# ChenyangLEI/All-In-One-Deflicker

Hardware: AMD Instinct MI355X
Metric: atlas-fit sampled points/sec (stage1, 10k iters) @1/2/4/8 GPU; PSNR vs ref (higher is better)
Workload: dtype f32 (MLP chains f16x3: operands split into 2 fp16 of their value scaled per row, 3 partial products; weight-gradient GEMM bf16x6; fp32 accumulate)

## Files before the change

all-in-one-deflicker_amd/csrc/elem.h:

```cpp
#pragma once
#include "af_dev.h"

struct PackArgs {
  const float* frames;
  const float* flow_f;
  const float* flow_b;
  const float* mask_f;
  const float* mask_b;
  const float* mask_fg;
  float* table;
  int resx, resy, F;
  unsigned long long* nvalid;
};

struct ResizeArgs {
  const void* src; int src_u8;
  int sh, sw, ch;
  float* dst; int dh, dw;
  long long pix_stride, ch_stride, offset;
  double scale0, scale1;
};
enum { AREA_GENERAL = 0, AREA_BLOCK = 1, AREA_2X2 = 2 };
struct AreaArgs {
  const unsigned char* src; int sh, sw, ch;
  unsigned char* dst; int dh, dw;
  int mode;
  int isx, isy; float inv_area;
  const int* xofs; const int* yofs;
  const int* xidx; const int* yidx;
  const float* xa; const float* ya;
};
struct LumaArgs {
  const unsigned char* src; int n, h, w;
  int gh, gw;
  int strip_rows, strips;
  unsigned long long* part;
};
enum { YUV_AXIS_FULL = 0, YUV_AXIS_CENTRED = 1, YUV_AXIS_COSITED = 2 };
struct YuvArgs {
  const unsigned char* src; unsigned char* dst;
  int h, w, ch, cw;
  int hmode, vmode, mono;
  int y0;
  int cy, crv, cgu, cgv, cbu;
  int ky[3], ku[3], kv[3];
};
struct ConsistencyArgs {
  const float* f12; const float* f21; int h, w;
  float* out; long long pix_stride, offset;
  float thresh;
};

struct PrepArgs {
  const float* table;
  const int64_t* inds;
  uint64_t seed; uint32_t iter;
  int N, resx, resy, F;
  float half_main, half_grad, half_frames;
  int d_local, d_global, nseg;
  float* coords;
  float* x0_tile;
  float* samples;
  int* counts;
  float* coords2;
  float* x0_tile2;
  float* coordsA;
  int d_global2;
  int* flow_rank;
  unsigned long long* scan;
  uint32_t epoch;
  unsigned long long* ticket;
  unsigned long long ticket_base;
  int* live;
};

struct LossArgs {
  const float* samples; const float* out_map; const float* out_atlas;
  float* dout_map; float* dout_atlas;
  const int* counts;
  const int* flow_rank; const int* live;
  float* loss_part;
  int N, nseg;
  float L, uv_scale; int d_local, d_global;
  float c_rgb, c_grad, c_rig, c_grig, c_flow;
};

struct LossSegArgs {
  const float* samples;
  const float* out_m1; const float* out_m2; const float* out_alpha; const float* out_atlas;
  float* dout_m1; float* dout_m2; float* dout_alpha; float* dout_atlas;
  const int* counts; float* loss_part;
  const int* flow_rank; const int* live;
  int N, nseg;
  float L, uv_scale; int d_local, d_global_fg, d_global_bg;
  float c_rgb, c_grad, c_rig, c_grig_fg, c_grig_bg, c_flow, c_boot, c_aflow, c_sparse;
};

struct PrePrepArgs {
  const int64_t* ys; const int64_t* xs;
  uint64_t seed; uint32_t iter;
  int N, resx, resy;
  float half_main, t;
  float* coords; float* x0_tile;
};
struct PreLossArgs { const float* coords; const float* out_map; float* dout_map; float* loss_part; int N; float uv_scale; };

struct CoordsAtArgs {
  float* coords;
  int resx, resy;
  int oh, ow;
  float half_main, t;
  long long r0; int n, n_pad;
};
struct FinishAtArgs {
  const float* out_atlas; const float* out_alpha; size_t row2;
  int n;
  float* rgb_out;
  unsigned char* u8_out;
  const unsigned char* ref;
  double* sse_part;
};

struct AdamJob {
  uint32_t part_off, part_blk, nslots, pld;
  uint32_t out_real, in_real, out_real_pad;
  uint32_t p_off;
  uint32_t p_ld;
  uint32_t col0;
  int32_t  b_off;
  uint32_t f_off;
  uint32_t f_mpad;
  int32_t  b_img_off;
  uint32_t b_mpad;
  uint32_t bias_img_off;
  uint32_t pe_kind;
  uint32_t hid_cols;
  int32_t  sf_off; uint32_t sf_kind, sf_mpad, sf_k0;
  int32_t  sb_off; uint32_t sb_kind, sb_mpad;
  int32_t  hf_off, hb_off;
};
struct AdamHyper { float step_size, bc2_sqrt, one_minus_b1, beta2, one_minus_b2, eps; };
struct AdamBufs { float* params; float* m; float* v; float* img_f; float* img_b; float* bias_img; char* sf; char* sb; char* hf; char* hb; };
struct AdamArgs {
  const AdamJob* jobs; const float* partial;
  AdamBufs bufs; AdamHyper hy;
  float* grad_out;
  const float* loss_part; float* loss_out; int* counts; int loss_nblk;
  int* nan_flag;
  int check_counts;
};

struct EditArgs {
  const float* uv1; const float* uv2; const float* out_alpha;
  int npix, res;
  int active[2]; float minx[2], miny[2], pixel_size[2];
  const float* tex[2];
  float* edit; float* edit_layer[2]; float* use[2];
  unsigned char* edit_u8;
};

struct LossMapArgs {
  float* coords; const float* table; size_t rec0;
  int resx, resy, rows_pad, frame, d;
  int seg_c, seg_ym, seg_xm, seg_t;
  float half_main, half_frames, t_centre;
  const float* out_m1; const float* out_m2;
  const float* out_alpha;
  const float* out_atlas;
  int flow_map;
  float L, uv_scale;
  float* rigidity1; float* rigidity2; float* flow1; float* flow2; float* flow_alpha; float* rgb_err; float* residual;
};

struct WarpErrArgs {
  const float* img1; const float* img2; const float* flow12; const float* flow21;
  size_t img_pair_stride, flow_pair_stride;
  int h, w, align_corners;
  float* noc; float* warped;
  double* part;
};
```

all-in-one-deflicker_amd/csrc/elem.hip:

```cpp
#include "af_dev.h"
#include "elem.h"

AF_DEV void philox4x32(uint32_t c0, uint32_t c1, uint32_t c2, uint32_t c3, uint32_t k0, uint32_t k1, uint32_t (&o)[4]) {
#pragma unroll
  for (int r = 0; r < 10; ++r) {
    const uint64_t p0 = (uint64_t)0xD2511F53u * c0, p1 = (uint64_t)0xCD9E8D57u * c2;
    const uint32_t n0 = (uint32_t)(p1 >> 32) ^ c1 ^ k0, n1 = (uint32_t)p1;
    const uint32_t n2 = (uint32_t)(p0 >> 32) ^ c3 ^ k1, n3 = (uint32_t)p0;
    c0 = n0; c1 = n1; c2 = n2; c3 = n3;
    k0 += 0x9E3779B9u; k1 += 0xBB67AE85u;
  }
  o[0] = c0; o[1] = c1; o[2] = c2; o[3] = c3;
}
AF_DEV uint64_t af_rand_below(uint64_t seed, uint32_t iter, uint32_t n, uint32_t stream, uint64_t bound) {
  uint32_t o[4];
  philox4x32(n, iter, stream, 0x41544c53u, (uint32_t)seed, (uint32_t)(seed >> 32), o);
  const uint64_t r = ((uint64_t)o[1] << 32) | o[0];
  return __umul64hi(r, bound);
}

__global__ void k_pack_table(PackArgs a) {
  const size_t P2 = (size_t)a.resx * a.resy;
  const size_t idx = (size_t)blockIdx.x * blockDim.x + threadIdx.x;
  const bool in_range = idx < P2 * a.F;
  const unsigned long long vf = __ballot(in_range && a.mask_f[idx] != 0.f), vb = __ballot(in_range && a.mask_b[idx] != 0.f);
  if (a.nvalid && (threadIdx.x & 63) == 0) {
    unsigned long long* c = a.nvalid + 2 * ((blockIdx.x * (blockDim.x >> 6) + (threadIdx.x >> 6)) & 63);
    if (vf) atomicAdd(c + 0, (unsigned long long)__popcll(vf));
    if (vb) atomicAdd(c + 1, (unsigned long long)__popcll(vb));
  }
  if (!in_range) return;
  const int f = (int)(idx % a.F);
  const size_t pix = idx / a.F;
  const int x = (int)(pix % a.resx), y = (int)(pix / a.resx);
  const int F = a.F;
  float rec[AF_REC_F];
#pragma unroll
  for (int c = 0; c < 3; ++c) {
    const float v = a.frames[(pix * 3 + c) * F + f];
    rec[REC_RGB + c] = v;
    rec[REC_DX + c] = (x + 1 < a.resx) ? a.frames[((pix + 1) * 3 + c) * F + f] - v : 0.f;
    rec[REC_DY + c] = (y + 1 < a.resy) ? a.frames[((pix + a.resx) * 3 + c) * F + f] - v : 0.f;
  }
#pragma unroll
  for (int c = 0; c < 2; ++c) {
    rec[REC_FF + c] = a.flow_f[(pix * 2 + c) * F + f];
    rec[REC_FB + c] = a.flow_b[(pix * 2 + c) * F + f];
  }
  rec[REC_MF] = a.mask_f[pix * F + f];
  rec[REC_MB] = a.mask_b[pix * F + f];
  rec[REC_FG] = a.mask_fg ? a.mask_fg[pix * F + f] : 0.f;
  f32x4* dst = (f32x4*)(a.table + ((size_t)f * P2 + pix) * AF_REC_F);
#pragma unroll
  for (int q = 0; q < 4; ++q) { f32x4 v = {rec[q * 4], rec[q * 4 + 1], rec[q * 4 + 2], rec[q * 4 + 3]}; dst[q] = v; }
}

template <class WT>
AF_DEV float resize_tap(const ResizeArgs& a, int y0, int y1, int x0, int x1, float a0, float a1, float b0, float b1, int c) {
#pragma clang fp contract(off)
  auto tap = [&](int yy, int xx) -> WT {
    const size_t i = ((size_t)yy * a.sw + xx) * a.ch + c;
    return a.src_u8 ? (WT)((double)((const unsigned char*)a.src)[i] / 255.0) : (WT)((const float*)a.src)[i];
  };
  const WT t0 = tap(y0, x0) * (WT)a0 + tap(y0, x1) * (WT)a1;
  const WT t1 = tap(y1, x0) * (WT)a0 + tap(y1, x1) * (WT)a1;
  return (float)(t0 * (WT)b0 + t1 * (WT)b1);
}
AF_DEV void resize_coeff(int d, int src, int dst, int& s0, int& s1, float& c0, float& c1) {
#pragma clang fp contract(off)
  const double scale = (double)src / (double)dst;
  float f = (float)(((double)d + 0.5) * scale - 0.5);
  int s = (int)floorf(f);
  f -= (float)s;
  if (s < 0) { s = 0; f = 0.f; }
  if (s >= src - 1) { s = src - 1; f = 0.f; }
  s0 = s; s1 = min(s + 1, src - 1); c0 = 1.f - f; c1 = f;
}
__global__ void k_resize_bilinear(ResizeArgs a) {
#pragma clang fp contract(off)
  const long long idx = (long long)blockIdx.x * blockDim.x + threadIdx.x;
  if (idx >= (long long)a.dh * a.dw) return;
  const int y = (int)(idx / a.dw), x = (int)(idx - (long long)y * a.dw);
  const bool same = a.sh == a.dh && a.sw == a.dw;
  int x0, x1, y0, y1; float a0, a1, b0, b1;
  resize_coeff(x, a.sw, a.dw, x0, x1, a0, a1);
  resize_coeff(y, a.sh, a.dh, y0, y1, b0, b1);
  for (int c = 0; c < a.ch; ++c) {
    float o;
    if (same) {
      const size_t i = ((size_t)y * a.sw + x) * a.ch + c;
      o = a.src_u8 ? (float)((double)((const unsigned char*)a.src)[i] / 255.0) : ((const float*)a.src)[i];
    } else {
      o = a.src_u8 ? resize_tap<double>(a, y0, y1, x0, x1, a0, a1, b0, b1, c) : resize_tap<float>(a, y0, y1, x0, x1, a0, a1, b0, b1, c);
    }
    if (c == 0) o = o * (float)a.scale0; else if (c == 1) o = o * (float)a.scale1;
    a.dst[idx * a.pix_stride + (long long)c * a.ch_stride + a.offset] = o;
  }
}

AF_DEV unsigned char area_u8(float v) { return (unsigned char)(int)fminf(fmaxf(rintf(v), 0.f), 255.f); }
__global__ __launch_bounds__(256) void k_resize_area(AreaArgs a) {
#pragma clang fp contract(off)
  const long long idx = (long long)blockIdx.x * blockDim.x + threadIdx.x;
  if (idx >= (long long)a.dh * a.dw) return;
  const int dy = (int)(idx / a.dw), dx = (int)(idx - (long long)dy * a.dw);
  unsigned char* o = a.dst + (size_t)idx * a.ch;
  if (a.mode != AREA_GENERAL) {
    unsigned long long s[4] = {0ull, 0ull, 0ull, 0ull};
    for (int ky = 0; ky < a.isy; ++ky) {
      const unsigned char* p = a.src + (((size_t)dy * a.isy + ky) * a.sw + (size_t)dx * a.isx) * a.ch;
      for (int kx = 0; kx < a.isx; ++kx, p += a.ch) {
#pragma unroll
        for (int c = 0; c < 4; ++c) if (c < a.ch) s[c] += p[c];
      }
    }
#pragma unroll
    for (int c = 0; c < 4; ++c) if (c < a.ch) o[c] = a.mode == AREA_2X2 ? (unsigned char)((s[c] + 2ull) >> 2) : area_u8((float)s[c] * a.inv_area);
    return;
  }
  const int x0 = a.xofs[dx], x1 = a.xofs[dx + 1], y0 = a.yofs[dy], y1 = a.yofs[dy + 1];
  float sum[4] = {0.f, 0.f, 0.f, 0.f};
  for (int j = y0; j < y1; ++j) {
    const unsigned char* row = a.src + (size_t)a.yidx[j] * a.sw * a.ch;
    const float beta = a.ya[j];
    float buf[4] = {0.f, 0.f, 0.f, 0.f};
    for (int i = x0; i < x1; ++i) {
      const unsigned char* p = row + (size_t)a.xidx[i] * a.ch;
      const float alpha = a.xa[i];
#pragma unroll
      for (int c = 0; c < 4; ++c) if (c < a.ch) buf[c] = buf[c] + (float)p[c] * alpha;
    }
#pragma unroll
    for (int c = 0; c < 4; ++c) sum[c] = j == y0 ? beta * buf[c] : sum[c] + beta * buf[c];
  }
#pragma unroll
  for (int c = 0; c < 4; ++c) if (c < a.ch) o[c] = area_u8(sum[c]);
}

__global__ void k_flow_consistency(ConsistencyArgs a) {
#pragma clang fp contract(off)
  const long long idx = (long long)blockIdx.x * blockDim.x + threadIdx.x;
  if (idx >= (long long)a.h * a.w) return;
  const int y = (int)(idx / a.w), x = (int)(idx - (long long)y * a.w);
  const float u = a.f12[idx * 2], v = a.f12[idx * 2 + 1];
  const float mx = u + (float)x, my = v + (float)y;
  const long long qx = (long long)rintf(mx * 32.f), qy = (long long)rintf(my * 32.f);
  const long long x0 = qx >> 5, y0 = qy >> 5;
  const float fx = (float)(qx & 31) / 32.f, fy = (float)(qy & 31) / 32.f;
  const float w0 = (1.f - fy) * (1.f - fx), w1 = (1.f - fy) * fx, w2 = fy * (1.f - fx), w3 = fy * fx;
  float acc[2];
  for (int c = 0; c < 2; ++c) {
    auto tap = [&](long long yy, long long xx) -> float {
      return (xx >= 0 && xx < a.w && yy >= 0 && yy < a.h) ? a.f21[(yy * a.w + xx) * 2 + c] : 0.f;
    };
    acc[c] = ((tap(y0, x0) * w0 + tap(y0, x0 + 1) * w1) + tap(y0 + 1, x0) * w2) + tap(y0 + 1, x0 + 1) * w3;
  }
  const float du = u + acc[0], dv = v + acc[1];
  const float nrm = sqrtf(du * du + dv * dv);
  a.out[idx * a.pix_stride + a.offset] = a.thresh > 0.f ? (nrm < a.thresh ? 1.f : 0.f) : nrm;
}

AF_DEV void put_row_to(float* coords, float* x0_tile, size_t r, float x, float y, float t) {
  f32x4 v = {x, y, t, 0.f};
  *(f32x4*)(coords + r * 4) = v;
  if (x0_tile) {
    float* tl = x0_tile + (r >> 5) * 1024 + (r & 31);
    tl[0] = x; tl[32] = y; tl[64] = t;
  }
}
AF_DEV void put_row_at(const PrepArgs& a, size_t r, long long arow, float x, float y, float t) {
  put_row_to(a.coords, a.x0_tile, r, x, y, t);
  if (a.coords2) {
    put_row_to(a.coords2, a.x0_tile2, r, x, y, t);
    if (arow >= 0) put_row_to(a.coordsA, nullptr, (size_t)arow, x, y, t);
  }
}
AF_DEV void put_row(const PrepArgs& a, int seg, int aseg, int n, float x, float y, float t) {
  put_row_at(a, (size_t)seg * a.N + n, aseg >= 0 ? (long long)aseg * a.N + n : -1, x, y, t);
}

__global__ __launch_bounds__(256) void k_prep(PrepArgs a) {
  __shared__ int wsum[4];
  __shared__ int red_i[4];
  if (threadIdx.x == 0) red_i[0] = (int)(atomicAdd(a.ticket, 1ull) - a.ticket_base);
  __syncthreads();
  const int vblk = red_i[0];
  __syncthreads();
  const int n = vblk * blockDim.x + threadIdx.x;
  const int lane = threadIdx.x & 63, wave = threadIdx.x >> 6;
  int vf = 0, vb = 0;
  int x = 0, y = 0, f = 0;
  float ffu = 0.f, ffv = 0.f, fbu = 0.f, fbv = 0.f;
  const float hm = a.half_main, hg = a.half_grad, hf = a.half_frames;
  if (n < a.N) {
    const uint64_t P2 = (uint64_t)a.resx * a.resy;
    const uint64_t k = a.inds ? (uint64_t)a.inds[n] : af_rand_below(a.seed, a.iter, (uint32_t)n, 0u, P2 * a.F);
    f = (int)(k / P2);
    const uint64_t rem = k - (uint64_t)f * P2;
    y = (int)(rem / a.resx); x = (int)(rem - (uint64_t)y * a.resx);
    const f32x4* rp = (const f32x4*)(a.table + k * AF_REC_F);
    f32x4 r0 = rp[0], r1 = rp[1], r2 = rp[2], r3 = rp[3];
    f32x4* sp = (f32x4*)(a.samples + (size_t)n * AF_REC_F);
    sp[0] = r0; sp[1] = r1; sp[2] = r2; sp[3] = r3;
    ffu = r2[1]; ffv = r2[2]; fbu = r2[3]; fbv = r3[0];
    const float mf = r3[1], mb = r3[2];
    const float xc = (float)x / hm - 1.f, yc = (float)y / hm - 1.f, tc = (float)f / hf - 1.f;
    put_row(a, 0, 0, n, xc, yc, tc);
    put_row(a, 1, 1, n, (float)x / hg - 1.f, (float)(y + 1) / hg - 1.f, tc);
    put_row(a, 2, 2, n, (float)(x + 1) / hg - 1.f, (float)y / hg - 1.f, tc);
    put_row(a, 3, -1, n, xc, (float)(y - a.d_local) / hm - 1.f, tc);
    put_row(a, 4, -1, n, (float)(x - a.d_local) / hm - 1.f, yc, tc);
    vf = mf != 0.f; vb = mb != 0.f;
    if (a.nseg > 7) {
      put_row_to(a.coords, a.x0_tile, (size_t)5 * a.N + n, xc, (float)(y - a.d_global) / hm - 1.f, tc);
      put_row_to(a.coords, a.x0_tile, (size_t)6 * a.N + n, (float)(x - a.d_global) / hm - 1.f, yc, tc);
      if (a.coords2) {
        put_row_to(a.coords2, a.x0_tile2, (size_t)5 * a.N + n, xc, (float)(y - a.d_global2) / hm - 1.f, tc);
        put_row_to(a.coords2, a.x0_tile2, (size_t)6 * a.N + n, (float)(x - a.d_global2) / hm - 1.f, yc, tc);
      }
    }
  }
  const unsigned long long bf = __ballot(vf), bb = __ballot(vb);
  const unsigned long long lt = (1ull << lane) - 1ull;
  const int in_wave = __popcll(bf & lt) + __popcll(bb & lt);
  if (lane == 0) {
    wsum[wave] = __popcll(bf) + __popcll(bb);
    if (bf) atomicAdd(a.counts + 0, __popcll(bf));
    if (bb) atomicAdd(a.counts + 1, __popcll(bb));
  }
  __syncthreads();
  int in_block = in_wave;
  for (int w = 0; w < wave; ++w) in_block += wsum[w];
  const int btot = (wsum[0] + wsum[1]) + (wsum[2] + wsum[3]);
  if (threadIdx.x == 0)
    __hip_atomic_store(a.scan + vblk, ((unsigned long long)a.epoch << 32) | (unsigned)btot, __ATOMIC_RELEASE, __HIP_MEMORY_SCOPE_AGENT);
  int pre = 0;
  if (wave == 0) {
    for (int b = lane; b < vblk; b += 64) {
      unsigned long long v;
      do { v = __hip_atomic_load(a.scan + b, __ATOMIC_ACQUIRE, __HIP_MEMORY_SCOPE_AGENT); } while ((uint32_t)(v >> 32) != a.epoch);
      pre += (int)(uint32_t)v;
    }
#pragma unroll
    for (int o = 32; o > 0; o >>= 1) pre += __shfl_xor(pre, o);
    if (lane == 0) red_i[0] = pre;
  }
  __syncthreads();
  pre = red_i[0];
  if (vblk == (int)gridDim.x - 1 && threadIdx.x == 0) *a.live = pre + btot;
  if (n < a.N) {
    const int rank_f = pre + in_block, rank_b = rank_f + vf;
    const size_t base = (size_t)(a.nseg - 2) * a.N, abase = (size_t)3 * a.N;
    a.flow_rank[2 * n] = vf ? rank_f : -1;
    a.flow_rank[2 * n + 1] = vb ? rank_b : -1;
    if (vf) put_row_at(a, base + rank_f, (long long)(abase + rank_f), ((float)x + ffu) / hm - 1.f, ((float)y + ffv) / hm - 1.f, (float)(f + 1) / hf - 1.f);
    if (vb) put_row_at(a, base + rank_b, (long long)(abase + rank_b), ((float)x + fbu) / hm - 1.f, ((float)y + fbv) / hm - 1.f, (float)(f - 1) / hf - 1.f);
  }
}

AF_DEV float block_sum(float v, float* red ) {
#pragma unroll
  for (int o = 32; o > 0; o >>= 1) v += __shfl_xor(v, o);
  __syncthreads();
  if ((threadIdx.x & 63) == 0) red[threadIdx.x >> 6] = v;
  __syncthreads();
  return (red[0] + red[1]) + (red[2] + red[3]);
}

struct Rig { float loss, du, dv, du_xm, du_ym, dv_xm, dv_ym; };
AF_DEV Rig rigidity(float u, float v, float u_ym, float v_ym, float u_xm, float v_xm, float L, float s, float d, float w) {
  const float j00 = ((u - u_xm) * L / 2.f) / s / d, j01 = ((u - u_ym) * L / 2.f) / s / d;
  const float j10 = ((v - v_xm) * L / 2.f) / s / d, j11 = ((v - v_ym) * L / 2.f) / s / d;
  const float g00 = j00 * j00 + j10 * j10, g01 = j00 * j01 + j10 * j11, g11 = j01 * j01 + j11 * j11;
  const float A = g00 + 0.001f, D = g11 + 0.001f, B = g01;
  const float det = A * D - B * B;
  const float i00 = D / det, i01 = -B / det, i11 = A / det;
  const float ng = sqrtf(g00 * g00 + 2.f * g01 * g01 + g11 * g11);
  const float ni = sqrtf(i00 * i00 + 2.f * i01 * i01 + i11 * i11);
  Rig r; r.loss = ng + ni;
  const float b2_00 = i00 * i00 + i01 * i01, b2_01 = i00 * i01 + i01 * i11, b2_11 = i01 * i01 + i11 * i11;
  const float b3_00 = b2_00 * i00 + b2_01 * i01, b3_01 = b2_00 * i01 + b2_01 * i11, b3_11 = b2_01 * i01 + b2_11 * i11;
  const float rg = ng > 0.f ? 1.f / ng : 0.f, ri = ni > 0.f ? 1.f / ni : 0.f;
  const float s00 = g00 * rg - b3_00 * ri, s01 = g01 * rg - b3_01 * ri, s11 = g11 * rg - b3_11 * ri;
  const float k = (L / 2.f) / s / d * w * 2.f;
  const float d00 = k * (j00 * s00 + j01 * s01), d01 = k * (j00 * s01 + j01 * s11);
  const float d10 = k * (j10 * s00 + j11 * s01), d11 = k * (j10 * s01 + j11 * s11);
  r.du = d00 + d01; r.dv = d10 + d11; r.du_xm = -d00; r.du_ym = -d01; r.dv_xm = -d10; r.dv_ym = -d11;
  return r;
}

AF_DEV void put_d2(float* dout, size_t row, float a, float b) { f32x4 v = {a, b, 0.f, 0.f}; *(f32x4*)(dout + row * 4) = v; }

__global__ __launch_bounds__(256) void k_loss_single(LossArgs a) {
  __shared__ float red[4];
  const int n = blockIdx.x * blockDim.x + threadIdx.x;
  float l_rgb = 0.f, l_grad = 0.f, l_rig = 0.f, l_grig = 0.f, l_ff = 0.f, l_fb = 0.f;
  if (n < a.N) {
    const size_t N = a.N;
    const float invN = 1.f / (float)a.N;
    const float* sp = a.samples + (size_t)n * AF_REC_F;
    const f32x4 uvc = *(const f32x4*)(a.out_map + (size_t)n * 4);
    const f32x4 uvy1 = *(const f32x4*)(a.out_map + (N + n) * 4);       (void)uvy1;
    float du = 0.f, dv = 0.f;
    const f32x4 tc = *(const f32x4*)(a.out_atlas + (size_t)n * 4);
    const f32x4 ty = *(const f32x4*)(a.out_atlas + (N + n) * 4);
    const f32x4 tx = *(const f32x4*)(a.out_atlas + (2 * N + n) * 4);
    float dtc[3], dty[3], dtx[3];
#pragma unroll
    for (int c = 0; c < 3; ++c) {
      const float rgb = (tc[c] + 1.f) * 0.5f, rgby = (ty[c] + 1.f) * 0.5f, rgbx = (tx[c] + 1.f) * 0.5f;
      const float e = rgb - sp[REC_RGB + c];
      const float rx = sp[REC_DX + c] - (rgbx - rgb), ry = sp[REC_DY + c] - (rgby - rgb);
      l_rgb += e * e;
      l_grad += rx * rx + ry * ry;
      dtc[c] = 0.5f * (a.c_rgb * 2.f * e + a.c_grad * 2.f * (rx + ry)) * invN;
      dtx[c] = 0.5f * (-a.c_grad * 2.f * rx) * invN;
      dty[c] = 0.5f * (-a.c_grad * 2.f * ry) * invN;
    }
    { f32x4 v = {dtc[0], dtc[1], dtc[2], 0.f}; *(f32x4*)(a.dout_atlas + (size_t)n * 4) = v; }
    { f32x4 v = {dty[0], dty[1], dty[2], 0.f}; *(f32x4*)(a.dout_atlas + (N + n) * 4) = v; }
    { f32x4 v = {dtx[0], dtx[1], dtx[2], 0.f}; *(f32x4*)(a.dout_atlas + (2 * N + n) * 4) = v; }
    put_d2(a.dout_map, N + n, 0.f, 0.f);
    put_d2(a.dout_map, 2 * N + n, 0.f, 0.f);
    {
      const f32x4 pym = *(const f32x4*)(a.out_map + (3 * N + n) * 4);
      const f32x4 pxm = *(const f32x4*)(a.out_map + (4 * N + n) * 4);
      const Rig r = rigidity(uvc[0], uvc[1], pym[0], pym[1], pxm[0], pxm[1], a.L, a.uv_scale, (float)a.d_local, a.c_rig * invN);
      l_rig = r.loss; du += r.du; dv += r.dv;
      put_d2(a.dout_map, 3 * N + n, r.du_ym, r.dv_ym);
      put_d2(a.dout_map, 4 * N + n, r.du_xm, r.dv_xm);
    }
    if (a.nseg > 7) {
      const f32x4 pym = *(const f32x4*)(a.out_map + (5 * N + n) * 4);
      const f32x4 pxm = *(const f32x4*)(a.out_map + (6 * N + n) * 4);
      const Rig r = rigidity(uvc[0], uvc[1], pym[0], pym[1], pxm[0], pxm[1], a.L, a.uv_scale, (float)a.d_global, a.c_grig * invN);
      l_grig = r.loss; du += r.du; dv += r.dv;
      put_d2(a.dout_map, 5 * N + n, r.du_ym, r.dv_ym);
      put_d2(a.dout_map, 6 * N + n, r.du_xm, r.dv_xm);
    }
    const float fscale = a.L / (2.f * a.uv_scale);
    const size_t flow_base = (size_t)(a.nseg - 2) * N;
#pragma unroll
    for (int dir = 0; dir < 2; ++dir) {
      const int rank = a.flow_rank[2 * n + dir];
      if (rank >= 0) {
        const size_t row = flow_base + rank;
        float gu = 0.f, gv = 0.f;
        const f32x4 m = *(const f32x4*)(a.out_map + row * 4);
        const float eu = m[0] - uvc[0], ev = m[1] - uvc[1];
        const float nrm = sqrtf(eu * eu + ev * ev);
        const float l = nrm * a.L / (2.f * a.uv_scale);
        if (dir) l_fb = l; else l_ff = l;
        const float cnt = (float)a.counts[dir];
        const float w = nrm > 0.f ? a.c_flow * 0.5f * fscale / (nrm * cnt) : 0.f;
        gu = w * eu; gv = w * ev;
        du -= gu; dv -= gv;
        put_d2(a.dout_map, row, gu, gv);
      }
    }
    put_d2(a.dout_map, (size_t)n, du, dv);
  }
  if (blockIdx.x == 0 && threadIdx.x < 32) {
    const size_t live_rows = (size_t)(a.nseg - 2) * a.N + *a.live, r = live_rows + threadIdx.x;
    if (r < ((live_rows + 31) & ~(size_t)31)) put_d2(a.dout_map, r, 0.f, 0.f);
  }
  float s[6] = {l_rgb, l_grad, l_rig, l_grig, l_ff, l_fb};
#pragma unroll
  for (int i = 0; i < 6; ++i) s[i] = block_sum(s[i], red);
  if (threadIdx.x == 0) {
    float* o = a.loss_part + (size_t)blockIdx.x * AF_LOSS_W;
#pragma unroll
    for (int i = 0; i < 6; ++i) o[i] = s[i];
#pragma unroll
    for (int i = 6; i < AF_LOSS_W; ++i) o[i] = 0.f;
  }
}

AF_DEV float alpha_of(float t) { float a = 0.5f * (t + 1.f); a = a * 0.99f; return a + 0.001f; }
#define AF_DALPHA 0.495f

__global__ __launch_bounds__(256) void k_loss_seg(LossSegArgs a) {
  __shared__ float red[4];
  const int n = blockIdx.x * blockDim.x + threadIdx.x;
  float ls[14];
#pragma unroll
  for (int i = 0; i < 14; ++i) ls[i] = 0.f;
  if (n < a.N) {
    const size_t N = a.N;
    const float invN = 1.f / (float)a.N;
    const float* sp = a.samples + (size_t)n * AF_REC_F;
    const float al = alpha_of(a.out_alpha[(size_t)n * 4]);
    const float aly = alpha_of(a.out_alpha[(N + n) * 4]);
    const float alx = alpha_of(a.out_alpha[(2 * N + n) * 4]);
    float dA = 0.f, dAy = 0.f, dAx = 0.f, dAf = 0.f, dAb = 0.f;
    const f32x4 t1c = *(const f32x4*)(a.out_atlas + (size_t)n * 4);
    const f32x4 t1y = *(const f32x4*)(a.out_atlas + (N + n) * 4);
    const f32x4 t1x = *(const f32x4*)(a.out_atlas + (2 * N + n) * 4);
    const f32x4 t2c = *(const f32x4*)(a.out_atlas + (3 * N + n) * 4);
    const f32x4 t2y = *(const f32x4*)(a.out_atlas + (4 * N + n) * 4);
    const f32x4 t2x = *(const f32x4*)(a.out_atlas + (5 * N + n) * 4);
    float d1c[3], d1y[3], d1x[3], d2c[3], d2y[3], d2x[3];
    float sq1 = 0.f;
#pragma unroll
    for (int c = 0; c < 3; ++c) {
      const float r1 = (t1c[c] + 1.f) * 0.5f, r2 = (t2c[c] + 1.f) * 0.5f;
      const float r1y = (t1y[c] + 1.f) * 0.5f, r2y = (t2y[c] + 1.f) * 0.5f;
      const float r1x = (t1x[c] + 1.f) * 0.5f, r2x = (t2x[c] + 1.f) * 0.5f;
      const float rgb = r1 * al + r2 * (1.f - al);
      const float rgby = r1y * aly + r2y * (1.f - aly);
      const float rgbx = r1x * alx + r2x * (1.f - alx);
      const float e = rgb - sp[REC_RGB + c];
      const float rx = sp[REC_DX + c] - (rgbx - rgb), ry = sp[REC_DY + c] - (rgby - rgb);
      const float nf = r1 * (1.f - al);
      ls[0] += e * e;
      ls[1] += rx * rx + ry * ry;
      ls[13] += nf * nf;
      sq1 += r1 * r1;
      const float g = (a.c_rgb * 2.f * e + a.c_grad * 2.f * (rx + ry)) * invN;
      const float gx = -a.c_grad * 2.f * rx * invN, gy = -a.c_grad * 2.f * ry * invN;
      d1c[c] = 0.5f * (al * g + a.c_sparse * 2.f * r1 * (1.f - al) * (1.f - al) * invN);
      d2c[c] = 0.5f * (1.f - al) * g;
      d1x[c] = 0.5f * alx * gx; d2x[c] = 0.5f * (1.f - alx) * gx;
      d1y[c] = 0.5f * aly * gy; d2y[c] = 0.5f * (1.f - aly) * gy;
      dA += (r1 - r2) * g;
      dAx += (r1x - r2x) * gx;
      dAy += (r1y - r2y) * gy;
    }
    dA -= a.c_sparse * 2.f * (1.f - al) * sq1 * invN;
    { f32x4 v = {d1c[0], d1c[1], d1c[2], 0.f}; *(f32x4*)(a.dout_atlas + (size_t)n * 4) = v; }
    { f32x4 v = {d1y[0], d1y[1], d1y[2], 0.f}; *(f32x4*)(a.dout_atlas + (N + n) * 4) = v; }
    { f32x4 v = {d1x[0], d1x[1], d1x[2], 0.f}; *(f32x4*)(a.dout_atlas + (2 * N + n) * 4) = v; }
    { f32x4 v = {d2c[0], d2c[1], d2c[2], 0.f}; *(f32x4*)(a.dout_atlas + (3 * N + n) * 4) = v; }
    { f32x4 v = {d2y[0], d2y[1], d2y[2], 0.f}; *(f32x4*)(a.dout_atlas + (4 * N + n) * 4) = v; }
    { f32x4 v = {d2x[0], d2x[1], d2x[2], 0.f}; *(f32x4*)(a.dout_atlas + (5 * N + n) * 4) = v; }
    {
      const float m = sp[REC_FG];
      ls[12] = -m * logf(al) - (1.f - m) * logf(1.f - al);
      dA += a.c_boot * (-m / al + (1.f - m) / (1.f - al)) * invN;
    }
    const float cntf = (float)a.counts[0], cntb = (float)a.counts[1];
    const bool vf = sp[REC_MF] != 0.f, vb = sp[REC_MB] != 0.f;
    const int rank_f = a.flow_rank[2 * n], rank_b = a.flow_rank[2 * n + 1];
    if (vf) {
      const float d = al - alpha_of(a.out_alpha[(3 * N + rank_f) * 4]);
      ls[10] = fabsf(d);
      const float g = a.c_aflow * 0.5f * (d > 0.f ? 1.f : (d < 0.f ? -1.f : 0.f)) / cntf;
      dA += g; dAf = -g;
    }
    if (vb) {
      const float d = alpha_of(a.out_alpha[(3 * N + rank_b) * 4]) - al;
      ls[11] = fabsf(d);
      const float g = a.c_aflow * 0.5f * (d > 0.f ? 1.f : (d < 0.f ? -1.f : 0.f)) / cntb;
      dAb = g; dA -= g;
    }
    const float fscale = a.L / (2.f * a.uv_scale);
#pragma unroll
    for (int net = 0; net < 2; ++net) {
      const float* om = net ? a.out_m2 : a.out_m1;
      float* dm = net ? a.dout_m2 : a.dout_m1;
      const f32x4 uvc = *(const f32x4*)(om + (size_t)n * 4);
      float du = 0.f, dv = 0.f;
      put_d2(dm, N + n, 0.f, 0.f);
      put_d2(dm, 2 * N + n, 0.f, 0.f);
      {
        const f32x4 pym = *(const f32x4*)(om + (3 * N + n) * 4);
        const f32x4 pxm = *(const f32x4*)(om + (4 * N + n) * 4);
        const Rig r = rigidity(uvc[0], uvc[1], pym[0], pym[1], pxm[0], pxm[1], a.L, a.uv_scale, (float)a.d_local, a.c_rig * invN);
        ls[2 + net] = r.loss; du += r.du; dv += r.dv;
        put_d2(dm, 3 * N + n, r.du_ym, r.dv_ym);
        put_d2(dm, 4 * N + n, r.du_xm, r.dv_xm);
      }
      if (a.nseg > 7) {
        const f32x4 pym = *(const f32x4*)(om + (5 * N + n) * 4);
        const f32x4 pxm = *(const f32x4*)(om + (6 * N + n) * 4);
        const Rig r = rigidity(uvc[0], uvc[1], pym[0], pym[1], pxm[0], pxm[1], a.L, a.uv_scale,
                               (float)(net ? a.d_global_bg : a.d_global_fg), (net ? a.c_grig_bg : a.c_grig_fg) * invN);
        ls[4 + net] = r.loss; du += r.du; dv += r.dv;
        put_d2(dm, 5 * N + n, r.du_ym, r.dv_ym);
        put_d2(dm, 6 * N + n, r.du_xm, r.dv_xm);
      }
      const float wrow = net ? 1.f - al : al;
      const float wsign = net ? -1.f : 1.f;
#pragma unroll
      for (int dir = 0; dir < 2; ++dir) {
        const bool valid = dir ? vb : vf;
        if (valid) {
          const size_t row = (size_t)(a.nseg - 2) * N + (dir ? rank_b : rank_f);
          float gu = 0.f, gv = 0.f;
          const f32x4 m = *(const f32x4*)(om + row * 4);
          const float eu = m[0] - uvc[0], ev = m[1] - uvc[1];
          const float nrm = sqrtf(eu * eu + ev * ev);
          const float l = nrm * a.L / (2.f * a.uv_scale);
          const float cnt = dir ? cntb : cntf;
          ls[6 + 2 * net + dir] = l * wrow;
          const float w = nrm > 0.f ? a.c_flow * 0.5f * fscale * wrow / (nrm * cnt) : 0.f;
          gu = w * eu; gv = w * ev;
          du -= gu; dv -= gv;
          dA += wsign * a.c_flow * 0.5f * l / cnt;
          put_d2(dm, row, gu, gv);
        }
      }
      put_d2(dm, (size_t)n, du, dv);
    }
    { f32x4 v = {AF_DALPHA * dA, 0.f, 0.f, 0.f};  *(f32x4*)(a.dout_alpha + (size_t)n * 4) = v; }
    { f32x4 v = {AF_DALPHA * dAy, 0.f, 0.f, 0.f}; *(f32x4*)(a.dout_alpha + (N + n) * 4) = v; }
    { f32x4 v = {AF_DALPHA * dAx, 0.f, 0.f, 0.f}; *(f32x4*)(a.dout_alpha + (2 * N + n) * 4) = v; }
    if (vf) { f32x4 v = {AF_DALPHA * dAf, 0.f, 0.f, 0.f}; *(f32x4*)(a.dout_alpha + (3 * N + rank_f) * 4) = v; }
    if (vb) { f32x4 v = {AF_DALPHA * dAb, 0.f, 0.f, 0.f}; *(f32x4*)(a.dout_alpha + (3 * N + rank_b) * 4) = v; }
  }
  if (blockIdx.x == 0 && threadIdx.x < 32) {
    const size_t live = (size_t)*a.live;
    const size_t rm = (size_t)(a.nseg - 2) * a.N + live, ra = (size_t)3 * a.N + live;
    if (rm + threadIdx.x < ((rm + 31) & ~(size_t)31)) { put_d2(a.dout_m1, rm + threadIdx.x, 0.f, 0.f); put_d2(a.dout_m2, rm + threadIdx.x, 0.f, 0.f); }
    if (ra + threadIdx.x < ((ra + 31) & ~(size_t)31)) { f32x4 v = {0.f, 0.f, 0.f, 0.f}; *(f32x4*)(a.dout_alpha + (ra + threadIdx.x) * 4) = v; }
  }
#pragma unroll
  for (int i = 0; i < 14; ++i) ls[i] = block_sum(ls[i], red);
  if (threadIdx.x == 0) {
    float* o = a.loss_part + (size_t)blockIdx.x * AF_LOSS_W;
#pragma unroll
    for (int i = 0; i < 14; ++i) o[i] = ls[i];
    o[14] = 0.f; o[15] = 0.f;
  }
}

__global__ void k_pre_prep(PrePrepArgs a) {
  const int n = blockIdx.x * blockDim.x + threadIdx.x;
  if (n >= a.N) return;
  const int y = a.ys ? (int)a.ys[n] : (int)af_rand_below(a.seed, a.iter, (uint32_t)n, 1u, (uint64_t)a.resy);
  const int x = a.xs ? (int)a.xs[n] : (int)af_rand_below(a.seed, a.iter, (uint32_t)n, 2u, (uint64_t)a.resx);
  const float xc = (float)x / a.half_main - 1.f, yc = (float)y / a.half_main - 1.f;
  f32x4 v = {xc, yc, a.t, 0.f};
  *(f32x4*)(a.coords + (size_t)n * 4) = v;
  if (a.x0_tile) {
    float* tl = a.x0_tile + ((size_t)n >> 5) * 1024 + (n & 31);
    tl[0] = xc; tl[32] = yc; tl[64] = a.t;
  }
}

__global__ __launch_bounds__(256) void k_pre_loss(PreLossArgs a) {
  __shared__ float red[4];
  const int n = blockIdx.x * blockDim.x + threadIdx.x;
  float l = 0.f;
  if (n < a.N) {
    const f32x4 c = *(const f32x4*)(a.coords + (size_t)n * 4);
    const f32x4 o = *(const f32x4*)(a.out_map + (size_t)n * 4);
    const float eu = c[0] * a.uv_scale - o[0], ev = c[1] * a.uv_scale - o[1];
    l = sqrtf(eu * eu + ev * ev);
    const float w = l > 0.f ? -1.f / (l * (float)a.N) : 0.f;
    put_d2(a.dout_map, (size_t)n, w * eu, w * ev);
  }
  l = block_sum(l, red);
  if (threadIdx.x == 0) { float* o = a.loss_part + (size_t)blockIdx.x * AF_LOSS_W; o[0] = l; for (int i = 1; i < AF_LOSS_W; ++i) o[i] = 0.f; }
}

AF_DEV uint16_t bf16_rne(float x) {
  const uint32_t u = __builtin_bit_cast(uint32_t, x);
  return (uint16_t)((u + 0x7fffu + ((u >> 16) & 1u)) >> 16);
}
AF_DEV void emit_bf3(char* block, uint32_t m, uint32_t k, float p) {
  const uint32_t T = k >> 5, q = (k >> 3) & 3, hh = (k >> 2) & 1, pp = k & 3;
  const uint32_t s = 2 * T + (q >> 1), i = 4 * (q & 1) + pp;
  const uint16_t h = bf16_rne(p);
  const float r1 = p - __builtin_bit_cast(float, (uint32_t)h << 16);
  const uint16_t mi = bf16_rne(r1);
  const float r2 = r1 - __builtin_bit_cast(float, (uint32_t)mi << 16);
  const uint16_t lo = bf16_rne(r2);
  const size_t base = ((size_t)((s * 8 + (m >> 5)) * 3) * 2 + hh) * 32 * 16 + (size_t)(m & 31) * 16 + i * 2;
  *(uint16_t*)(block + base) = h;
  *(uint16_t*)(block + base + 1024) = mi;
  *(uint16_t*)(block + base + 2048) = lo;
}

AF_DEV void emit_hf2(char* block, uint32_t m, uint32_t k, float p) {
  const uint32_t T = k >> 5, q = (k >> 3) & 3, hh = (k >> 2) & 1, pp = k & 3;
  const uint32_t s = 2 * T + (q >> 1), i = 4 * (q & 1) + pp;
  const float ps = p * 4096.f;
  const _Float16 h = (_Float16)ps;
  const _Float16 l = (_Float16)(ps - (float)h);
  const size_t base = ((size_t)((s * 8 + (m >> 5)) * 2) * 2 + hh) * 32 * 16 + (size_t)(m & 31) * 16 + i * 2;
  *(_Float16*)(block + base) = h;
  *(_Float16*)(block + base + 1024) = l;
}

AF_DEV void emit_weight(const AdamJob& j, const AdamBufs& b, uint32_t o, uint32_t i, float p) {
  const uint32_t col = j.col0 + i;
  uint32_t k = col;
  if (col >= j.hid_cols) k = j.hid_cols + (uint32_t)af_pe_slot_of_feature((int)j.pe_kind, (int)(col - j.hid_cols));
  b.img_f[j.f_off + af_img_index(j.f_mpad, o, k)] = p;
  if (j.b_img_off >= 0 && col < (j.hid_cols ? j.hid_cols : j.p_ld)) {
    const uint32_t mrow = j.hid_cols ? col : (uint32_t)af_pe_slot_of_feature((int)j.pe_kind, (int)col);
    b.img_b[(uint32_t)j.b_img_off + af_img_index(j.b_mpad, mrow, o)] = p;
    if (b.sb && j.sb_off >= 0) {
      if (j.sb_kind == 0) ((float*)(b.sb + j.sb_off))[af_img_index(j.sb_mpad, mrow, o)] = p;
      else                emit_bf3(b.sb + j.sb_off, mrow, o, p);
    }
    if (b.hb && j.hb_off >= 0) {
      if (j.sb_kind == 0) ((float*)(b.hb + j.hb_off))[af_img_index(j.sb_mpad, mrow, o)] = p;
      else                emit_hf2(b.hb + j.hb_off, mrow, o, p);
    }
  }
  if (b.sf && j.sf_off >= 0) {
    if (j.sf_kind == 0) ((float*)(b.sf + j.sf_off))[af_img_index(j.sf_mpad, o, k - j.sf_k0)] = p;
    else                emit_bf3(b.sf + j.sf_off, o, k, p);
  }
  if (b.hf && j.hf_off >= 0) {
    if (j.sf_kind == 0) ((float*)(b.hf + j.hf_off))[af_img_index(j.sf_mpad, o, k - j.sf_k0)] = p;
    else                emit_hf2(b.hf + j.hf_off, o, k, p);
  }
}

template <bool UPDATE>
__global__ __launch_bounds__(256) void k_adam(AdamArgs a) {
  const AdamJob j = a.jobs[blockIdx.y];
  const uint32_t e = blockIdx.x * blockDim.x + threadIdx.x;
  const uint32_t nw = j.out_real * j.in_real;
  const uint32_t nb = j.b_off >= 0 ? j.out_real : 0u;
  if (e < nw + nb) {
    const bool is_bias = e >= nw;
    const uint32_t o = is_bias ? e - nw : e / j.in_real;
    const uint32_t i = is_bias ? 0u : e - o * j.in_real;
    const uint32_t pidx = is_bias ? (uint32_t)j.b_off + o : j.p_off + o * j.p_ld + i;
    float p = a.bufs.params[pidx];
    if (UPDATE) {
      const float* pp = a.partial + j.part_off + (is_bias ? j.out_real_pad * j.pld + o : o * j.pld + i);
      float g = 0.f;
      uint32_t s = 0;
      for (; s + 8 <= j.nslots; s += 8) {
        float t[8];
#pragma unroll
        for (int q = 0; q < 8; ++q) t[q] = pp[(size_t)(s + q) * j.part_blk];
#pragma unroll
        for (int q = 0; q < 8; ++q) g += t[q];
      }
      if (s + 4 <= j.nslots) {
        float t[4];
#pragma unroll
        for (int q = 0; q < 4; ++q) t[q] = pp[(size_t)(s + q) * j.part_blk];
#pragma unroll
        for (int q = 0; q < 4; ++q) g += t[q];
        s += 4;
      }
      if (s + 2 <= j.nslots) {
        const float t0 = pp[(size_t)s * j.part_blk], t1 = pp[(size_t)(s + 1) * j.part_blk];
        g += t0; g += t1; s += 2;
      }
      if (s < j.nslots) g += pp[(size_t)s * j.part_blk];
      float m = a.bufs.m[pidx], v = a.bufs.v[pidx];
      m = m + (g - m) * a.hy.one_minus_b1;
      v = v * a.hy.beta2 + (a.hy.one_minus_b2 * g) * g;
      const float denom = sqrtf(v) / a.hy.bc2_sqrt + a.hy.eps;
      p = p - a.hy.step_size * (m / denom);
      a.bufs.m[pidx] = m; a.bufs.v[pidx] = v; a.bufs.params[pidx] = p;
      if (a.grad_out) a.grad_out[pidx] = g;
    }
    if (a.nan_flag && !(fabsf(p) <= 3.4028235e38f)) atomicOr(a.nan_flag, 1);
    if (a.nan_flag && a.bufs.hf && !is_bias && j.sf_kind == 1 && fabsf(p) >= 8.f) atomicOr(a.nan_flag, 2);
    if (is_bias) a.bufs.bias_img[j.bias_img_off + o] = p;
    else emit_weight(j, a.bufs, o, i, p);
  }
  if (UPDATE && blockIdx.x == 0 && blockIdx.y == 0 && a.loss_out) {
    if (threadIdx.x < AF_LOSS_W - 2) {
      float s = 0.f;
      for (int b = 0; b < a.loss_nblk; ++b) s += a.loss_part[b * AF_LOSS_W + threadIdx.x];
      a.loss_out[threadIdx.x] = s;
      if (a.nan_flag && !(s == s)) atomicOr(a.nan_flag, 1);
    } else if (threadIdx.x < AF_LOSS_W) {
      a.loss_out[threadIdx.x] = (float)a.counts[threadIdx.x - (AF_LOSS_W - 2)];
      if (a.nan_flag && a.check_counts && a.counts[threadIdx.x - (AF_LOSS_W - 2)] == 0) atomicOr(a.nan_flag, 1);
      a.counts[threadIdx.x - (AF_LOSS_W - 2)] = 0;
    }
  }
}

__global__ void k_frame_coords(float* coords, int resx, int resy, float half_main, float t, int npix_pad) {
  const int r = blockIdx.x * blockDim.x + threadIdx.x;
  if (r >= npix_pad) return;
  const int npix = resx * resy;
  f32x4 v = {0.f, 0.f, 0.f, 0.f};
  if (r < npix) { const int y = r / resx, x = r - y * resx; v[0] = (float)x / half_main - 1.f; v[1] = (float)y / half_main - 1.f; v[2] = t; }
  *(f32x4*)(coords + (size_t)r * 4) = v;
}

__global__ __launch_bounds__(256) void k_frame_finish(const float* out_atlas, const float* table, float* rgb_out, double* sse_part,
                                                     int npix, size_t rec0) {
  __shared__ double red[4];
  const int r = blockIdx.x * blockDim.x + threadIdx.x;
  double sse = 0.0;
  if (r < npix) {
    const f32x4 t = *(const f32x4*)(out_atlas + (size_t)r * 4);
    const float* rec = table + (rec0 + r) * AF_REC_F;
#pragma unroll
    for (int c = 0; c < 3; ++c) {
      const float v = (t[c] + 1.f) * 0.5f;
      rgb_out[(size_t)r * 3 + c] = v;
      const double d = (double)rec[REC_RGB + c] - (double)v;
      sse += d * d;
    }
  }
#pragma unroll
  for (int o = 32; o > 0; o >>= 1) sse += __shfl_xor(sse, o);
  if ((threadIdx.x & 63) == 0) red[threadIdx.x >> 6] = sse;
  __syncthreads();
  if (threadIdx.x == 0) sse_part[blockIdx.x] = (red[0] + red[1]) + (red[2] + red[3]);
}

__global__ __launch_bounds__(256) void k_frame_finish_seg(const float* out_atlas, const float* out_alpha, size_t row2, const float* table,
                                                         float* rgb_out, double* sse_part, int npix, size_t rec0) {
  __shared__ double red[4];
  const int r = blockIdx.x * blockDim.x + threadIdx.x;
  double sse = 0.0;
  if (r < npix) {
    const f32x4 t1 = *(const f32x4*)(out_atlas + (size_t)r * 4);
    const f32x4 t2 = *(const f32x4*)(out_atlas + (row2 + r) * 4);
    const float al = alpha_of(out_alpha[(size_t)r * 4]);
    const float* rec = table + (rec0 + r) * AF_REC_F;
#pragma unroll
    for (int c = 0; c < 3; ++c) {
      const float v = ((t1[c] + 1.f) * 0.5f) * al + ((t2[c] + 1.f) * 0.5f) * (1.f - al);
      rgb_out[(size_t)r * 3 + c] = v;
      const double d = (double)rec[REC_RGB + c] - (double)v;
      sse += d * d;
    }
  }
#pragma unroll
  for (int o = 32; o > 0; o >>= 1) sse += __shfl_xor(sse, o);
  if ((threadIdx.x & 63) == 0) red[threadIdx.x >> 6] = sse;
  __syncthreads();
  if (threadIdx.x == 0) sse_part[blockIdx.x] = (red[0] + red[1]) + (red[2] + red[3]);
}

__global__ __launch_bounds__(256) void k_frame_u8(const float* rgb, unsigned char* out, int npix) {
  const int r = blockIdx.x * blockDim.x + threadIdx.x;
  if (r >= npix) return;
#pragma unroll
  for (int c = 0; c < 3; ++c) out[(size_t)r * 3 + c] = (unsigned char)(int)((double)rgb[(size_t)r * 3 + c] * 255.0);
}

AF_DEV float coord_at(int d, int src, int dst, float half_main) {
#pragma clang fp contract(off)
  const double scale = (double)src / (double)dst;
  double s = ((double)d + 0.5) * scale - 0.5;
  s = s < 0.0 ? 0.0 : s;
  s = s > (double)(src - 1) ? (double)(src - 1) : s;
  return (float)s / half_main - 1.f;
}
__global__ __launch_bounds__(256) void k_frame_coords_at(CoordsAtArgs a) {
  const int r = blockIdx.x * blockDim.x + threadIdx.x;
  if (r >= a.n_pad) return;
  f32x4 v = {0.f, 0.f, 0.f, 0.f};
  if (r < a.n) {
    const long long g = a.r0 + r;
    const int Y = (int)(g / a.ow), X = (int)(g - (long long)Y * a.ow);
    v[0] = coord_at(X, a.resx, a.ow, a.half_main); v[1] = coord_at(Y, a.resy, a.oh, a.half_main); v[2] = a.t;
  }
  *(f32x4*)(a.coords + (size_t)r * 4) = v;
}

template <bool SEG>
__global__ __launch_bounds__(256) void k_frame_finish_at(FinishAtArgs a) {
#pragma clang fp contract(off)
  __shared__ double red[4];
  const int r = blockIdx.x * blockDim.x + threadIdx.x;
  double sse = 0.0;
  if (r < a.n) {
    const f32x4 t1 = *(const f32x4*)(a.out_atlas + (size_t)r * 4);
    f32x4 t2 = {0.f, 0.f, 0.f, 0.f};
    float al = 1.f;
    if (SEG) {
      t2 = *(const f32x4*)(a.out_atlas + (a.row2 + r) * 4);
      const float h = 0.5f * (a.out_alpha[(size_t)r * 4] + 1.f), q = h * 0.99f;
      al = q + 0.001f;
    }
#pragma unroll
    for (int c = 0; c < 3; ++c) {
      float v = (t1[c] + 1.f) * 0.5f;
      if (SEG) {
        const float bg = ((t2[c] + 1.f) * 0.5f) * (1.f - al);
        if (c == 1) { const float fg = v * al; v = fg + bg; } else v = __builtin_fmaf(al, v, bg);
      }
      if (a.rgb_out) a.rgb_out[(size_t)r * 3 + c] = v;
      if (a.u8_out) a.u8_out[(size_t)r * 3 + c] = (unsigned char)(int)((double)v * 255.0);
      if (a.ref) { const double d = (double)a.ref[(size_t)r * 3 + c] / 255.0 - (double)v; sse += d * d; }
    }
  }
  if (!a.sse_part) return;
#pragma unroll
  for (int o = 32; o > 0; o >>= 1) sse += __shfl_xor(sse, o);
  if ((threadIdx.x & 63) == 0) red[threadIdx.x >> 6] = sse;
  __syncthreads();
  if (threadIdx.x == 0) a.sse_part[blockIdx.x] = (red[0] + red[1]) + (red[2] + red[3]);
}

extern "C" {
int af_launch_frame_coords_at(const CoordsAtArgs* a, hipStream_t s) {
  hipLaunchKernelGGL(k_frame_coords_at, dim3((a->n_pad + 255) / 256), dim3(256), 0, s, *a);
  return (int)hipGetLastError();
}
int af_launch_frame_finish_at(const FinishAtArgs* a, hipStream_t s) {
  if (a->out_alpha) hipLaunchKernelGGL(k_frame_finish_at<true>, dim3((a->n + 255) / 256), dim3(256), 0, s, *a);
  else              hipLaunchKernelGGL(k_frame_finish_at<false>, dim3((a->n + 255) / 256), dim3(256), 0, s, *a);
  return (int)hipGetLastError();
}
int af_launch_frame_u8(const float* rgb, unsigned char* out, int npix, hipStream_t s) {
  hipLaunchKernelGGL(k_frame_u8, dim3((npix + 255) / 256), dim3(256), 0, s, rgb, out, npix);
  return (int)hipGetLastError();
}
int af_launch_resize(const ResizeArgs* a, hipStream_t s) {
  const long long n = (long long)a->dh * a->dw;
  hipLaunchKernelGGL(k_resize_bilinear, dim3((unsigned)((n + 255) / 256)), dim3(256), 0, s, *a);
  return (int)hipGetLastError();
}
int af_launch_resize_area(const AreaArgs* a, hipStream_t s) {
  const long long n = (long long)a->dh * a->dw;
  hipLaunchKernelGGL(k_resize_area, dim3((unsigned)((n + 255) / 256)), dim3(256), 0, s, *a);
  return (int)hipGetLastError();
}
int af_launch_consistency(const ConsistencyArgs* a, hipStream_t s) {
  const long long n = (long long)a->h * a->w;
  hipLaunchKernelGGL(k_flow_consistency, dim3((unsigned)((n + 255) / 256)), dim3(256), 0, s, *a);
  return (int)hipGetLastError();
}
int af_launch_loss_seg(const LossSegArgs* a, hipStream_t s) {
  hipLaunchKernelGGL(k_loss_seg, dim3((a->N + 255) / 256), dim3(256), 0, s, *a);
  return (int)hipGetLastError();
}
int af_launch_frame_finish_seg(const float* out_atlas, const float* out_alpha, size_t row2, const float* table, float* rgb_out, double* sse_part,
                               int npix, size_t rec0, hipStream_t s) {
  hipLaunchKernelGGL(k_frame_finish_seg, dim3((npix + 255) / 256), dim3(256), 0, s, out_atlas, out_alpha, row2, table, rgb_out, sse_part, npix, rec0);
  return (int)hipGetLastError();
}
int af_launch_pack(const PackArgs* a, hipStream_t s) {
  const size_t n = (size_t)a->resx * a->resy * a->F;
  hipLaunchKernelGGL(k_pack_table, dim3((unsigned)((n + 255) / 256)), dim3(256), 0, s, *a);
  return (int)hipGetLastError();
}
int af_launch_prep(const PrepArgs* a, hipStream_t s) {
  hipLaunchKernelGGL(k_prep, dim3((a->N + 255) / 256), dim3(256), 0, s, *a);
  return (int)hipGetLastError();
}
int af_launch_loss_single(const LossArgs* a, hipStream_t s) {
  hipLaunchKernelGGL(k_loss_single, dim3((a->N + 255) / 256), dim3(256), 0, s, *a);
  return (int)hipGetLastError();
}
int af_launch_pre_prep(const PrePrepArgs* a, hipStream_t s) {
  hipLaunchKernelGGL(k_pre_prep, dim3((a->N + 255) / 256), dim3(256), 0, s, *a);
  return (int)hipGetLastError();
}
int af_launch_pre_loss(const PreLossArgs* a, hipStream_t s) {
  hipLaunchKernelGGL(k_pre_loss, dim3((a->N + 255) / 256), dim3(256), 0, s, *a);
  return (int)hipGetLastError();
}
int af_launch_adam(const AdamArgs* a, int njobs, int update, hipStream_t s) {
  const dim3 grid((AF_HID * 320 + AF_HID + 255) / 256, njobs);
  if (update) hipLaunchKernelGGL(k_adam<true>, grid, dim3(256), 0, s, *a);
  else        hipLaunchKernelGGL(k_adam<false>, grid, dim3(256), 0, s, *a);
  return (int)hipGetLastError();
}
int af_launch_frame_coords(float* coords, int resx, int resy, float half_main, float t, int npix_pad, hipStream_t s) {
  hipLaunchKernelGGL(k_frame_coords, dim3((npix_pad + 255) / 256), dim3(256), 0, s, coords, resx, resy, half_main, t, npix_pad);
  return (int)hipGetLastError();
}
int af_launch_frame_finish(const float* out_atlas, const float* table, float* rgb_out, double* sse_part, int npix, size_t rec0, hipStream_t s) {
  hipLaunchKernelGGL(k_frame_finish, dim3((npix + 255) / 256), dim3(256), 0, s, out_atlas, table, rgb_out, sse_part, npix, rec0);
  return (int)hipGetLastError();
}
}
```

all-in-one-deflicker_amd/csrc/host.hip:

```cpp
#include <hip/hip_runtime.h>
#include <float.h>
#include <math.h>
#include <cmath>
#include <stdio.h>
#include <string.h>
#include <algorithm>
#include <string>
#include <vector>

#include "../../include/atlasfit.h"
#include "af_dev.h"
#include "elem.h"

extern "C" {
int af_launch_fwd_multi(MultiFwd* m, int train, hipStream_t s);
int af_launch_bwd_multi(MultiBwd* m, hipStream_t s);
int af_mlp_init();
int af_mlp_chunk_bytes(int net, int which, int nl);
int af_launch_fwd_multi_bf(MultiFwd* m, int train, hipStream_t s);
int af_launch_bwd_multi_bf(MultiBwd* m, hipStream_t s);
int af_mlp_bf_init();
int af_mlp_chunk_bytes_bf(int net, int which, int nl);
int af_launch_fwd_multi_hf(MultiFwd* m, int train, hipStream_t s);
int af_launch_bwd_multi_hf(MultiBwd* m, hipStream_t s);
int af_mlp_hf_init();
int af_mlp_chunk_bytes_hf(int net, int which, int nl);
int af_launch_fwd16(int net, const FwdArgs* a, hipStream_t s);
int af_launch_bwd16(int net, const BwdArgs* a, hipStream_t s);
int af_mlp16_init();
int af_launch_dw(const DwArgs* a, int nwg, int mode, hipStream_t s);
int af_dw_init();
int af_launch_pack(const PackArgs* a, hipStream_t s);
int af_launch_prep(const PrepArgs* a, hipStream_t s);
int af_launch_loss_single(const LossArgs* a, hipStream_t s);
int af_launch_loss_seg(const LossSegArgs* a, hipStream_t s);
int af_launch_resize(const ResizeArgs* a, hipStream_t s);
int af_launch_resize_area(const AreaArgs* a, hipStream_t s);
int af_launch_consistency(const ConsistencyArgs* a, hipStream_t s);
int af_launch_luma_grid(const LumaArgs* a, hipStream_t s);
int af_launch_yuv_to_rgb(const YuvArgs* a, hipStream_t s);
int af_launch_rgb_to_yuv(const YuvArgs* a, hipStream_t s);
int af_launch_frame_finish_seg(const float* out_atlas, const float* out_alpha, size_t row2, const float* table, float* rgb_out, double* sse_part,
                               int npix, size_t rec0, hipStream_t s);
int af_launch_pre_prep(const PrePrepArgs* a, hipStream_t s);
int af_launch_pre_loss(const PreLossArgs* a, hipStream_t s);
int af_launch_adam(const AdamArgs* a, int njobs, int update, hipStream_t s);
int af_launch_frame_coords(float* coords, int resx, int resy, float half_main, float t, int npix_pad, hipStream_t s);
int af_launch_frame_finish(const float* out_atlas, const float* table, float* rgb_out, double* sse_part, int npix, size_t rec0, hipStream_t s);
int af_launch_frame_u8(const float* rgb, unsigned char* out, int npix, hipStream_t s);
int af_launch_frame_coords_at(const CoordsAtArgs* a, hipStream_t s);
int af_launch_frame_finish_at(const FinishAtArgs* a, hipStream_t s);
int af_launch_layer_finish(const float* uv1s, const float* uv2s, const float* out_atlas, size_t row2, const float* out_alpha, int npix,
                           float* uv1, float* uv2, float* alpha, float* rgb1, float* rgb2, hipStream_t s);
int af_launch_area_reduce(const float* uv, const float* out_alpha, const float* table, size_t rec0, int npix, int which, float* part, hipStream_t s);
int af_launch_tex_coords(float* coords, int res, int row0, int nrows, float sx, float ex, float sy, float ey, int rows_pad, hipStream_t s);
int af_launch_tex_finish(const float* out_atlas, int rows, float* out, hipStream_t s);
int af_launch_edit(const EditArgs* a, hipStream_t s);
int af_launch_layer_finish_at(const float* uv1s, const float* uv2s, const float* out_atlas, size_t row2, const float* out_alpha, int npix,
                              float* uv1, float* uv2, float* alpha, float* rgb1, float* rgb2, unsigned char* alpha_u8, hipStream_t s);
int af_launch_edit_at(const EditArgs* a, hipStream_t s);
int af_launch_lossmap_rows(const LossMapArgs* a, hipStream_t s);
int af_launch_lossmap_finish(const LossMapArgs* a, hipStream_t s);
int af_launch_warp_error(const WarpErrArgs* a, int kind, int npairs, hipStream_t s);
}

namespace {

thread_local std::string g_create_error;

struct StreamPlan {
  size_t f_base = 0, b_base = 0;
  long long f_hid[AF_MAX_LAYERS], f_fp[AF_MAX_LAYERS], b_hid[AF_MAX_LAYERS], b_fp[AF_MAX_LAYERS];
};

struct NetDesc {
  int kern = -1;
  int id = -1, NL = 0, in_kind = 0, in_feat0 = 0, out = 0, pe_feats = 0, pe_kind = 0;
  unsigned skip = 0; bool dx0 = false; bool used = false;
  int in_feat[AF_MAX_LAYERS], out_feat[AF_MAX_LAYERS];
  size_t w_off[AF_MAX_LAYERS], b_off[AF_MAX_LAYERS];
  size_t nparams = 0, p_base = 0;
  int hid = AF_HID; size_t nlogical = 0; std::vector<uint32_t> lmap;
  size_t f_off[AF_MAX_LAYERS]; int f_mpad[AF_MAX_LAYERS], f_groups[AF_MAX_LAYERS];
  long long b_off_img[AF_MAX_LAYERS]; int b_mpad[AF_MAX_LAYERS];
  size_t f_base = 0, b_base = 0, bias_base = 0;
  std::vector<AfChunk> fchunks, bchunks;
  StreamPlan bf, hf;
  int nt_cap = 0;
  float *coords = nullptr, *x0_tile = nullptr;
  float *acts = nullptr, *dz = nullptr, *dz_last = nullptr, *pe_tile = nullptr, *out_buf = nullptr, *dout = nullptr;
  uint32_t* masks = nullptr;
};

struct Sched {
  std::vector<DwJob> jobs; std::vector<AdamJob> ajobs; std::vector<DwSeg> segs;
  int nwg = 0; size_t partial_floats = 0;
  DwJob* d_jobs = nullptr; AdamJob* d_ajobs = nullptr; DwSeg* d_segs = nullptr;
};

struct TimedEv { int cls; hipEvent_t a, b; };

}

struct af_edit {
  af_handle* h = nullptr;
  int res = 0; bool track = false;
  bool have_win[2] = {false, false}; float win[2][3] = {{0, 0, 0}, {0, 0, 0}};
  float* tex[2] = {nullptr, nullptr};
  float* use[2] = {nullptr, nullptr};
};

struct af_handle {
  af_config cfg;
  bool seg = false;
  int device = 0; hipStream_t stream = nullptr; int ncu = 256;
  std::string err;
  NetDesc nets[AF_MAX_NETS];
  size_t total_params = 0, img_f_floats = 0, img_b_floats = 0, bias_floats = 0, sf_bytes = 0, sb_bytes = 0;
  char *img_sf = nullptr, *img_sb = nullptr;
  char *img_hf = nullptr, *img_hb = nullptr; size_t hf_bytes = 0, hb_bytes = 0;
  int mlp_mode = 3;
  float *params = nullptr, *adam_m = nullptr, *adam_v = nullptr, *pre_m = nullptr, *pre_v = nullptr, *grads = nullptr;
  float *img_f = nullptr, *img_b = nullptr, *bias_img = nullptr;
  long long adam_step = 0;
  float* table = nullptr; bool have_video = false;
  int N = 0;
  float *samples = nullptr, *loss_part = nullptr, *loss_log = nullptr;
  int* counts = nullptr; int loss_nblk_cap = 0; size_t loss_log_cap = 0;
  int* nan_flag = nullptr;
  int cur_nseg = 0;
  int* flow_rank = nullptr; unsigned long long* scan = nullptr; int* live = nullptr; uint32_t prep_epoch = 0; unsigned long long prep_tickets = 0;
  unsigned long long* nvalid = nullptr; double p_valid[2] = {1.0, 1.0};
  int plan_flow_rows = 0;
  Sched sched[4]; float* partial = nullptr; size_t partial_cap = 0;
  unsigned long long* dw_clock = nullptr;
  unsigned long long* step_stamp = nullptr;
  int render_rows_cap = 0; float *r_coords = nullptr, *r_uv = nullptr, *r_uv2 = nullptr, *r_al = nullptr, *r_t = nullptr, *r_rgb = nullptr; double* r_sse = nullptr;
  unsigned char* r_u8 = nullptr;
  unsigned char* r_at = nullptr;
  std::vector<double> frame_sse; std::vector<char> frame_sse_valid;
  float* l_buf = nullptr; size_t l_cap = 0;
  std::vector<af_edit*> sessions;
  bool debug = false; unsigned timing = 0, timing_every = 1; bool timing_live = true;
  double flop_fwd[AF_MAX_NETS] = {0}, flop_dx[AF_MAX_NETS] = {0};
  bool dw_cost_set = false; double dw_cost[5] = {0}, dw_seg_cost = 0;
  int dw_mode = 1;
  std::vector<TimedEv> evs; double t_ms[16] = {0}, t_flops[16] = {0}; long long t_cnt[16] = {0};

  int fail(int code, const char* what, hipError_t e = hipSuccess) {
    char buf[512];
    if (e != hipSuccess) snprintf(buf, sizeof buf, "%s: %s", what, hipGetErrorString(e));
    else snprintf(buf, sizeof buf, "%s", what);
    err = buf;
    return code;
  }
};

#define HCHK(x) do { hipError_t e_ = (x); if (e_ != hipSuccess) return h->fail(AF_EHIP, #x, e_); } while (0)
#define AF_TEX_MAX 16384
#define LCHK(x) do { int r_ = (x); if (r_ != 0) return h->fail(AF_EHIP, #x, (hipError_t)r_); } while (0)

namespace {

enum { T_PREP = 0, T_FWD_1 = 1, T_FWD_2 = 2, T_LOSS = 3, T_BWD_1 = 4, T_BWD_2 = 5, T_DW = 6, T_ADAM = 7 };

template <class T> hipError_t dalloc(T** p, size_t n) { return hipMalloc((void**)p, std::max<size_t>(n, 1) * sizeof(T)); }

void describe_net(NetDesc& n, int id, int NL, int in_kind, int pe_freqs, int out, unsigned skip, bool dx0, int hid = AF_HID) {
  n.id = id; n.kern = (in_kind == AF_IN_PE3 && out == 2) ? AF_KIND_MAP_PE : id; n.NL = NL; n.in_kind = in_kind; n.out = out; n.skip = skip; n.dx0 = dx0; n.used = true;
  const int in_dim = in_kind == AF_IN_PE2 ? 2 : 3;
  n.pe_feats = in_kind == AF_IN_XYT ? 0 : 2 * in_dim * pe_freqs;
  n.pe_kind = in_kind == AF_IN_PE3 ? 2 : (in_kind == AF_IN_PE2 ? 1 : 0);
  n.in_feat0 = in_kind == AF_IN_XYT ? 3 : n.pe_feats;
  size_t off = 0;
  for (int l = 0; l < NL; ++l) {
    n.in_feat[l] = l == 0 ? n.in_feat0 : (AF_HID + (((skip >> l) & 1) ? n.pe_feats : 0));
    n.out_feat[l] = l == NL - 1 ? out : AF_HID;
    n.w_off[l] = off; off += (size_t)n.in_feat[l] * n.out_feat[l];
    n.b_off[l] = off; off += n.out_feat[l];
  }
  n.nparams = off;
  n.hid = hid; n.nlogical = off; n.lmap.clear();
  if (hid != AF_HID) {
    for (int l = 0; l < NL; ++l) {
      const int pin = n.in_feat[l], pout = n.out_feat[l];
      const int lout = l == NL - 1 ? out : hid;
      const int extra = l == 0 ? n.in_feat0 : (pin - AF_HID);
      const int lhid = l == 0 ? 0 : hid;
      for (int r = 0; r < lout; ++r) {
        for (int c = 0; c < lhid; ++c) n.lmap.push_back((uint32_t)(n.w_off[l] + (size_t)r * pin + c));
        for (int c = 0; c < extra; ++c) n.lmap.push_back((uint32_t)(n.w_off[l] + (size_t)r * pin + (l == 0 ? 0 : AF_HID) + c));
      }
      (void)pout;
      for (int r = 0; r < lout; ++r) n.lmap.push_back((uint32_t)(n.b_off[l] + r));
    }
    n.nlogical = n.lmap.size();
  }
}

size_t round_up(size_t v, size_t a) { return (v + a - 1) / a * a; }

void plan_images(NetDesc& n, size_t& f_cursor, size_t& b_cursor, size_t& bias_cursor) {
  n.f_base = f_cursor; n.b_base = b_cursor; n.bias_base = bias_cursor;
  bias_cursor += (size_t)n.NL * AF_HID;
  const int peg = n.in_kind == AF_IN_PE3 ? 4 : (n.in_kind == AF_IN_PE2 ? 5 : 0);
  size_t foff = 0;
  for (int l = 0; l < n.NL; ++l) {
    const bool last = l == n.NL - 1;
    const int mpad = last ? 4 : AF_HID;
    const int groups = (l == 0) ? (n.in_kind == AF_IN_XYT ? 1 : peg) : (32 + (((n.skip >> l) & 1) ? peg : 0));
    n.f_mpad[l] = mpad; n.f_groups[l] = groups;
    n.f_off[l] = n.f_base + foff / 4;
    const size_t gbytes = (size_t)2 * mpad * 16;
    if (l == 0 || last) {
      const size_t bytes = round_up(groups * gbytes, 4096);
      n.fchunks.push_back({(uint32_t)foff, (uint32_t)bytes});
      foff += bytes;
    } else {
      for (int c = 0; c < 4; ++c) { n.fchunks.push_back({(uint32_t)foff, (uint32_t)(8 * gbytes)}); foff += 8 * gbytes; }
      if ((n.skip >> l) & 1) { const size_t bytes = round_up(peg * gbytes, 4096); n.fchunks.push_back({(uint32_t)foff, (uint32_t)bytes}); foff += bytes; }
    }
  }
  f_cursor += foff / 4;
  size_t boff = 0;
  for (int l = 0; l < n.NL; ++l) { n.b_off_img[l] = -1; n.b_mpad[l] = 0; }
  for (int l = n.NL - 1; l >= (n.dx0 ? 0 : 1); --l) {
    const int mpad = l == 0 ? 64 : AF_HID;
    const int groups = l == n.NL - 1 ? 1 : 32;
    n.b_mpad[l] = mpad; n.b_off_img[l] = (long long)(n.b_base + boff / 4);
    const size_t gbytes = (size_t)2 * mpad * 16;
    if (groups * gbytes <= AF_CHUNK_MAX) { n.bchunks.push_back({(uint32_t)boff, (uint32_t)(groups * gbytes)}); boff += groups * gbytes; }
    else for (int c = 0; c < 4; ++c) { n.bchunks.push_back({(uint32_t)boff, (uint32_t)(8 * gbytes)}); boff += 8 * gbytes; }
  }
  b_cursor += boff / 4;
}

struct ChainFamily {
  int cls;
  int (*fwd)(MultiFwd*, int, hipStream_t);
  int (*bwd)(MultiBwd*, hipStream_t);
  int (*chunk_bytes)(int net, int which, int nl);
  int hid_chunks, wbytes;
};
const ChainFamily k_fp32 = {0, af_launch_fwd_multi, af_launch_bwd_multi, af_mlp_chunk_bytes, 4, 4};
const ChainFamily k_bf16x6 = {1, af_launch_fwd_multi_bf, af_launch_bwd_multi_bf, af_mlp_chunk_bytes_bf, 8, 6};
const ChainFamily k_f16x3 = {2, af_launch_fwd_multi_hf, af_launch_bwd_multi_hf, af_mlp_chunk_bytes_hf, 4, 4};
const ChainFamily& chain_family(int mlp_mode) { return mlp_mode == 3 ? k_f16x3 : (mlp_mode ? k_bf16x6 : k_fp32); }

bool plan_stream(NetDesc& n, StreamPlan& sp, const ChainFamily& fam, size_t& f_cursor, size_t& b_cursor) {
  const auto chunk_bytes = fam.chunk_bytes; const int hid_chunks = fam.hid_chunks;
  const int peg = n.in_kind == AF_IN_PE3 ? 4 : (n.in_kind == AF_IN_PE2 ? 5 : 0);
  const int cb_l0 = chunk_bytes(n.kern, 0, n.NL), cb_hid = chunk_bytes(n.kern, 1, n.NL), cb_skip = chunk_bytes(n.kern, 2, n.NL);
  const int cb_last = chunk_bytes(n.kern, 3, n.NL), cb_blast = chunk_bytes(n.kern, 4, n.NL), cb_bl0h = chunk_bytes(n.kern, 5, n.NL);
  for (int l = 0; l < AF_MAX_LAYERS; ++l) sp.f_hid[l] = sp.f_fp[l] = sp.b_hid[l] = sp.b_fp[l] = -1;
  sp.f_base = f_cursor; sp.b_base = b_cursor;
  size_t off = 0;
  sp.f_fp[0] = (long long)off; off += cb_l0;
  if ((size_t)cb_l0 < round_up((size_t)(n.in_kind == AF_IN_XYT ? 1 : peg) * 2 * AF_HID * 16, 4096)) return false;
  for (int l = 1; l < n.NL - 1; ++l) {
    sp.f_hid[l] = (long long)off; off += (size_t)hid_chunks * cb_hid;
    if ((n.skip >> l) & 1) { sp.f_fp[l] = (long long)off; off += cb_skip; }
  }
  sp.f_fp[n.NL - 1] = (long long)off; off += cb_last;
  f_cursor += off;
  off = 0;
  sp.b_fp[n.NL - 1] = (long long)off; off += cb_blast;
  for (int l = n.NL - 2; l >= 1; --l) { sp.b_hid[l] = (long long)off; off += (size_t)hid_chunks * cb_hid; }
  if (n.dx0) { sp.b_fp[0] = (long long)off; off += (size_t)2 * cb_bl0h; }
  b_cursor += off;
  return hid_chunks * cb_hid == AF_HID * AF_HID * fam.wbytes && cb_blast == 2 * AF_HID * 16 && 2 * cb_bl0h == 32 * 2 * 64 * 16;
}

bool check_chunk_plan(const NetDesc& n) {
  std::vector<int> f, b;
  f.push_back(af_mlp_chunk_bytes(n.kern, 0, n.NL));
  for (int l = 1; l < n.NL - 1; ++l) { for (int c = 0; c < 4; ++c) f.push_back(af_mlp_chunk_bytes(n.kern, 1, n.NL)); if ((n.skip >> l) & 1) f.push_back(af_mlp_chunk_bytes(n.kern, 2, n.NL)); }
  f.push_back(af_mlp_chunk_bytes(n.kern, 3, n.NL));
  b.push_back(af_mlp_chunk_bytes(n.kern, 4, n.NL));
  for (int l = n.NL - 2; l >= 1; --l) for (int c = 0; c < 4; ++c) b.push_back(af_mlp_chunk_bytes(n.kern, 1, n.NL));
  if (n.dx0) b.push_back(af_mlp_chunk_bytes(n.kern, 5, n.NL));
  auto same = [](const std::vector<AfChunk>& plan, const std::vector<int>& want) {
    if (plan.size() != want.size()) return false;
    uint32_t off = 0;
    for (size_t i = 0; i < plan.size(); ++i) { if (plan[i].off != off || (int)plan[i].bytes != want[i]) return false; off += plan[i].bytes; }
    return true;
  };
  return same(n.fchunks, f) && same(n.bchunks, b);
}

int shape_tiles(int shape, int& To, int& Ti) {
  switch (shape) {
    case DW_8x8: To = 8; Ti = 8; return 256;
    case DW_8x2: To = 8; Ti = 2; return 64;
    case DW_8x1: To = 8; Ti = 1; return 32;
    case DW_1x8: To = 1; Ti = 8; return 32;
    default:     To = 1; Ti = 2; return 16;
  }
}

struct NetUse { NetDesc* n; int NT; int live_base = -1; int NT_plan = -1; };

bool build_sched(af_handle* h, Sched& sc, const std::vector<NetUse>& uses) {
  sc.jobs.clear(); sc.ajobs.clear(); sc.segs.clear();
  std::vector<int> job_nt, job_cap;
  int cur_live_base = -1, cur_cap = 0;
  auto add = [&](NetDesc& n, int NT, int l, int shape, const float* A, uint32_t as, const float* B, uint32_t bs,
                 int col0, int in_real, bool owns_bias) {
    int To, Ti; shape_tiles(shape, To, Ti);
    DwJob j{}; j.A = A; j.B = B; j.a_stride = as; j.b_stride = bs; j.shape = shape;
    if (cur_live_base >= 0) { j.live_base = cur_live_base; j.live_rows = h->live; }
    j.part_blk = (uint32_t)(To * 32 * Ti * 32 + To * 32);
    sc.jobs.push_back(j); job_nt.push_back(NT); job_cap.push_back(cur_cap);
    AdamJob a{};
    a.part_blk = j.part_blk; a.pld = Ti * 32; a.out_real = n.out_feat[l]; a.in_real = in_real; a.out_real_pad = To * 32;
    a.p_off = (uint32_t)(n.p_base + n.w_off[l] + col0); a.p_ld = n.in_feat[l]; a.col0 = col0;
    a.b_off = owns_bias ? (int32_t)(n.p_base + n.b_off[l]) : -1;
    a.f_off = (uint32_t)n.f_off[l]; a.f_mpad = n.f_mpad[l];
    a.b_img_off = (int32_t)n.b_off_img[l]; a.b_mpad = n.b_mpad[l];
    a.bias_img_off = (uint32_t)(n.bias_base + (size_t)l * AF_HID);
    a.pe_kind = n.pe_kind;
    a.hid_cols = l == 0 ? (n.in_kind == AF_IN_XYT ? n.in_feat[l] : 0) : AF_HID;
    const bool last_l = l == n.NL - 1;
    a.sf_k0 = 0; a.sf_mpad = last_l ? 4 : AF_HID; a.sb_mpad = l == 0 ? 64 : AF_HID;
    if (l == 0 || last_l)  { a.sf_kind = 0; a.sf_off = (int32_t)(n.bf.f_base + n.bf.f_fp[l]); }
    else if (col0 == 0)    { a.sf_kind = 1; a.sf_off = (int32_t)(n.bf.f_base + n.bf.f_hid[l]); }
    else                   { a.sf_kind = 0; a.sf_off = (int32_t)(n.bf.f_base + n.bf.f_fp[l]); a.sf_k0 = AF_HID; }
    if (n.b_off_img[l] < 0)      { a.sb_kind = 0; a.sb_off = -1; }
    else if (last_l || l == 0)   { a.sb_kind = 0; a.sb_off = (int32_t)(n.bf.b_base + n.bf.b_fp[l]); }
    else                         { a.sb_kind = 1; a.sb_off = (int32_t)(n.bf.b_base + n.bf.b_hid[l]); }
    a.hf_off = (int32_t)(n.hf.f_base + (a.sf_kind == 1 ? n.hf.f_hid[l] : n.hf.f_fp[l]));
    a.hb_off = a.sb_off < 0 ? -1 : (int32_t)(n.hf.b_base + (a.sb_kind == 1 ? n.hf.b_hid[l] : n.hf.b_fp[l]));
    sc.ajobs.push_back(a);
  };
  for (const NetUse& u : uses) {
    NetDesc& n = *u.n;
    const int NT = u.NT_plan >= 0 ? std::min(u.NT_plan, u.NT) : u.NT;
    cur_live_base = u.live_base; cur_cap = u.NT;
    const size_t ts = (size_t)u.NT * AF_TILE_F;
    for (int l = 0; l < n.NL; ++l) {
      const bool last = l == n.NL - 1, sk = (n.skip >> l) & 1;
      if (l == 0) {
        if (n.in_kind == AF_IN_XYT) add(n, NT, 0, DW_8x1, n.dz, AF_TILE_F, n.x0_tile, 1024, 0, 3, true);
        else                        add(n, NT, 0, DW_8x2, n.dz, AF_TILE_F, n.pe_tile, 2048, 0, n.pe_feats, true);
      } else if (!last) {
        add(n, NT, l, DW_8x8, n.dz + l * ts, AF_TILE_F, n.acts + (l - 1) * ts, AF_TILE_F, 0, AF_HID, true);
        if (sk) add(n, NT, l, DW_8x2, n.dz + l * ts, AF_TILE_F, n.pe_tile, 2048, AF_HID, n.pe_feats, false);
      } else {
        add(n, NT, l, DW_1x8, n.dz_last, 1024, n.acts + (l - 1) * ts, AF_TILE_F, 0, AF_HID, true);
        if (sk) add(n, NT, l, DW_1x2, n.dz_last, 1024, n.pe_tile, 2048, AF_HID, n.pe_feats, false);
      }
    }
  }
  const int nj = (int)sc.jobs.size();
  static const double kTileCost[3][5] = {{306.0, 94.0, 62.0, 62.0, 46.0}, {306.0, 166.0, 140.0, 143.0, 97.0}, {306.0, 168.0, 157.0, 150.0, 95.0}};
  double seg_cost = 60.0;
  double cost_row[5];
  for (int i = 0; i < 5; ++i) cost_row[i] = kTileCost[h->dw_mode][i];
  if (h->dw_cost_set) {
    for (int i = 0; i < 5; ++i) cost_row[i] = h->dw_cost[i];
    if (h->dw_seg_cost > 0) seg_cost = h->dw_seg_cost;
  }
  auto tile_cost = [&](int j) { return cost_row[sc.jobs[j].shape]; };
  double work = 0;
  for (int j = 0; j < nj; ++j) work += tile_cost(j) * job_nt[j];
  int nwg = (int)std::min<double>(h->ncu, std::max(1.0, work / (4.0 * 276.0)));
  std::vector<int> order(nj);
  for (int j = 0; j < nj; ++j) order[j] = j;
  std::stable_sort(order.begin(), order.end(), [&](int a, int b) { return tile_cost(a) * job_nt[a] > tile_cost(b) * job_nt[b]; });
  std::vector<int> nslots(nj, 0);
  std::vector<std::vector<DwSeg>> wg(nwg);
  const double total = work + seg_cost * (nj + nwg);
  const double target = total / nwg;
  int w = 0; double cum = 0;
  for (int oi = 0; oi < nj; ++oi) {
    const int j = order[oi]; int t = 0; const double tc = tile_cost(j);
    while (t < job_nt[j]) {
      const double bound = (w + 1) * target;
      int take;
      if (w == nwg - 1) take = job_nt[j] - t;
      else {
        take = (int)floor((bound - cum - seg_cost) / tc + 0.5);
        if (take <= 0 || (int)wg[w].size() >= DW_MAXSEG) { ++w; continue; }
        take = std::min(take, job_nt[j] - t);
      }
      wg[w].push_back({j, t, t + take, nslots[j]++});
      cum += seg_cost + tc * take; t += take;
      if (t == job_nt[j]) wg[w].back().t1 = job_cap[j];
      if (w < nwg - 1 && cum >= bound - 0.5 * tc) ++w;
    }
  }
  sc.nwg = nwg;
  for (int i = 0; i < nwg; ++i) if (wg[i].size() > DW_MAXSEG) return false;
  sc.segs.assign((size_t)nwg * DW_MAXSEG, DwSeg{-1, 0, 0, 0});
  for (int i = 0; i < nwg; ++i)
    for (size_t s = 0; s < wg[i].size() && s < DW_MAXSEG; ++s) sc.segs[(size_t)i * DW_MAXSEG + s] = wg[i][s];
  size_t off = 0;
  for (int j = 0; j < nj; ++j) {
    sc.jobs[j].part_off = (uint32_t)off; sc.ajobs[j].part_off = (uint32_t)off; sc.ajobs[j].nslots = nslots[j];
    off += (size_t)nslots[j] * sc.jobs[j].part_blk;
  }
  sc.partial_floats = off;
  return true;
}

hipError_t upload_sched(Sched& sc) {
  hipError_t e;
  if (sc.d_jobs) { (void)hipFree(sc.d_jobs); (void)hipFree(sc.d_ajobs); (void)hipFree(sc.d_segs); sc.d_jobs = nullptr; }
  if ((e = dalloc(&sc.d_jobs, sc.jobs.size())) != hipSuccess) return e;
  if ((e = dalloc(&sc.d_ajobs, sc.ajobs.size())) != hipSuccess) return e;
  if ((e = dalloc(&sc.d_segs, sc.segs.size())) != hipSuccess) return e;
  if ((e = hipMemcpy(sc.d_jobs, sc.jobs.data(), sc.jobs.size() * sizeof(DwJob), hipMemcpyHostToDevice)) != hipSuccess) return e;
  if ((e = hipMemcpy(sc.d_ajobs, sc.ajobs.data(), sc.ajobs.size() * sizeof(AdamJob), hipMemcpyHostToDevice)) != hipSuccess) return e;
  return hipMemcpy(sc.d_segs, sc.segs.data(), sc.segs.size() * sizeof(DwSeg), hipMemcpyHostToDevice);
}

int tiles_of(int rows) { return (rows + 31) / 32; }

int planned_flow_rows(const af_handle* h) {
  const double N = h->N, pf = h->p_valid[0], pb = h->p_valid[1];
  const double e = N * (pf + pb), sd = sqrt(std::max(0.0, N * (pf * (1.0 - pf) + pb * (1.0 - pb))));
  return (int)std::min(2.0 * N, ceil(e + 4.0 * sd) + 32.0);
}

bool build_main_scheds(af_handle* h) {
  NetDesc& M = h->nets[AF_NET_MAP1]; NetDesc& A = h->nets[AF_NET_ATLAS]; NetDesc& M2 = h->nets[AF_NET_MAP2]; NetDesc& AL = h->nets[AF_NET_ALPHA];
  const int N = h->N; const bool seg = h->seg;
  h->plan_flow_rows = planned_flow_rows(h);
  for (int v = 0; v < 2; ++v) {
    const int nseg = v == 0 ? 9 : 7, fb = (nseg - 2) * N;
    std::vector<NetUse> uses = {{&M, tiles_of(nseg * N), fb, tiles_of(fb + h->plan_flow_rows)}};
    if (seg) { uses.push_back({&M2, tiles_of(nseg * N), fb, tiles_of(fb + h->plan_flow_rows)}); uses.push_back({&AL, tiles_of(5 * N), 3 * N, tiles_of(3 * N + h->plan_flow_rows)}); }
    uses.push_back({&A, tiles_of((seg ? 6 : 3) * N)});
    if (!build_sched(h, h->sched[v], uses)) return false;
  }
  return true;
}

hipError_t alloc_net_buffers(NetDesc& n, int rows_cap, bool own_coords) {
  n.nt_cap = tiles_of(rows_cap);
  const size_t nt = n.nt_cap, rp = nt * 32;
  hipError_t e;
  if ((e = dalloc(&n.acts, (size_t)(n.NL - 1) * nt * AF_TILE_F)) != hipSuccess) return e;
  if ((e = dalloc(&n.dz, (size_t)(n.NL - 1) * nt * AF_TILE_F)) != hipSuccess) return e;
  if ((e = dalloc(&n.masks, (size_t)(n.NL - 1) * nt * 64 * 4)) != hipSuccess) return e;
  if ((e = dalloc(&n.dz_last, nt * 1024)) != hipSuccess) return e;
  if ((e = dalloc(&n.pe_tile, n.pe_feats ? nt * 2048 : 1)) != hipSuccess) return e;
  if ((e = dalloc(&n.out_buf, rp * 4)) != hipSuccess) return e;
  if ((e = dalloc(&n.dout, rp * 4)) != hipSuccess) return e;
  if ((e = hipMemset(n.dz_last, 0, nt * 1024 * 4)) != hipSuccess) return e;
  if (n.pe_feats && (e = hipMemset(n.pe_tile, 0, nt * 2048 * 4)) != hipSuccess) return e;
  if ((e = hipMemset(n.out_buf, 0, rp * 16)) != hipSuccess) return e;
  if ((e = hipMemset(n.dout, 0, rp * 16)) != hipSuccess) return e;
  if (own_coords) {
    if ((e = dalloc(&n.coords, rp * 4)) != hipSuccess) return e;
    if ((e = hipMemset(n.coords, 0, rp * 16)) != hipSuccess) return e;
    if (n.in_kind == AF_IN_XYT) {
      if ((e = dalloc(&n.x0_tile, nt * 1024)) != hipSuccess) return e;
      if ((e = hipMemset(n.x0_tile, 0, nt * 4096)) != hipSuccess) return e;
    }
  }
  return hipSuccess;
}

void free_net(NetDesc& n) {
  (void)hipFree(n.acts); (void)hipFree(n.dz); (void)hipFree(n.masks); (void)hipFree(n.dz_last); (void)hipFree(n.pe_tile); (void)hipFree(n.out_buf); (void)hipFree(n.dout);
  (void)hipFree(n.coords); (void)hipFree(n.x0_tile);
}

const float* chain_wimg(const af_handle* h, const NetDesc& n, bool fwd) {
  switch (chain_family(h->mlp_mode).cls) {
    case 0:  return fwd ? h->img_f + n.f_base : h->img_b + n.b_base;
    case 1:  return (const float*)(fwd ? h->img_sf + n.bf.f_base : h->img_sb + n.bf.b_base);
    default: return (const float*)(fwd ? h->img_hf + n.hf.f_base : h->img_hb + n.hf.b_base);
  }
}

FwdArgs fwd_args(af_handle* h, NetDesc& n, const float* in, float* out, int NT, bool train) {
  FwdArgs a{};
  a.wimg = chain_wimg(h, n, true); a.bias = h->bias_img + n.bias_base;
  a.in = in; a.in1 = nullptr; a.out = out; a.acts = train ? n.acts : nullptr; a.masks = train ? n.masks : nullptr; a.pe_tile = train ? n.pe_tile : nullptr;
  a.in_scale = 0.5f; a.in_shift0 = 0.5f; a.in_shift1 = -0.5f; a.split_row = 0x7fffffff;
  a.NT = NT; a.nt_stride = NT; a.nl = n.NL;
  return a;
}

BwdArgs bwd_args(af_handle* h, NetDesc& n, int NT) {
  BwdArgs a{};
  a.wimg = chain_wimg(h, n, false); a.out = n.out_buf; a.dout = n.dout; a.masks = n.masks;
  a.dz = n.dz; a.dz_last = n.dz_last; a.pe_tile = n.pe_tile; a.din0 = nullptr; a.din1 = nullptr; a.din_scale = 0.5f;
  a.split_row = 0x7fffffff; a.nrows = 0; a.NT = NT; a.nt_stride = NT; a.nl = n.NL;
  return a;
}
FwdArgs fp32_images(FwdArgs a, const af_handle* h, const NetDesc& n) { a.wimg = h->img_f + n.f_base; return a; }
BwdArgs fp32_images(BwdArgs a, const af_handle* h, const NetDesc& n) { a.wimg = h->img_b + n.b_base; return a; }

struct Timer {
  af_handle* h; int cls; hipEvent_t a = nullptr, b = nullptr;
  Timer(af_handle* h_, int c, double flops = 0.0) : h(h_), cls(c) {
    if (on()) { (void)hipEventCreate(&a); (void)hipEventCreate(&b); (void)hipEventRecord(a, h->stream); h->t_flops[cls] += flops; }
  }
  ~Timer() { if (on()) { (void)hipEventRecord(b, h->stream); h->evs.push_back({cls, a, b}); } }
  bool on() const { return h->timing_live && ((h->timing >> cls) & 1u); }
};

void drain_timers(af_handle* h) {
  for (TimedEv& e : h->evs) {
    float ms = 0; (void)hipEventSynchronize(e.b); (void)hipEventElapsedTime(&ms, e.a, e.b);
    h->t_ms[e.cls] += ms; h->t_cnt[e.cls] += 1;
    (void)hipEventDestroy(e.a); (void)hipEventDestroy(e.b);
  }
  h->evs.clear();
}

AdamHyper adam_hyper(double lr, long long step) {
  const double b1 = 0.9, b2 = 0.999, eps = 1e-8;
  const double bc1 = 1.0 - pow(b1, (double)step), bc2 = 1.0 - pow(b2, (double)step);
  AdamHyper hy;
  hy.step_size = (float)(lr / bc1); hy.bc2_sqrt = (float)sqrt(bc2);
  hy.one_minus_b1 = (float)(1.0 - b1); hy.beta2 = (float)b2; hy.one_minus_b2 = (float)(1.0 - b2); hy.eps = (float)eps;
  return hy;
}

AdamBufs adam_bufs(af_handle* h, float* m, float* v) {
  const int cls = chain_family(h->mlp_mode).cls;
  const bool bf = cls == 1, hf = cls == 2;
  return {h->params, m, v, h->img_f, h->img_b, h->bias_img, bf ? h->img_sf : nullptr, bf ? h->img_sb : nullptr, hf ? h->img_hf : nullptr, hf ? h->img_hb : nullptr};
}

int repack(af_handle* h, Sched& sc) {
  AdamArgs a{};
  a.jobs = sc.d_ajobs; a.partial = h->partial;
  a.bufs = adam_bufs(h, h->adam_m, h->adam_v);
  a.nan_flag = h->nan_flag;
  LCHK(af_launch_adam(&a, (int)sc.ajobs.size(), 0, h->stream));
  return 0;
}

bool glob_on(const af_config& c, int iter) { return c.include_global_rigidity_loss && iter <= c.stop_global_rigidity; }

double part_rows(int tile0, int NT, int rows_total) { return (double)std::max(0, std::min(NT * 32, rows_total) - tile0 * 32); }

struct FwdPart { int net; FwdArgs a; int rows_total; };
struct BwdPart { int net; BwdArgs a; int rows_total; };

int launch_fwd(af_handle* h, int cls, std::initializer_list<FwdPart> parts, bool train) {
  MultiFwd m{}; double fl = 0;
  for (const FwdPart& p : parts) {
    if (p.a.NT <= p.a.tile0) continue;
    m.net[m.n] = h->nets[p.net].kern; m.a[m.n] = p.a; ++m.n;
    fl += part_rows(p.a.tile0, p.a.NT, p.rows_total) * h->flop_fwd[p.net];
  }
  if (m.n == 0) return 0;
  if (h->step_stamp && train && (cls == T_FWD_1 || cls == T_FWD_2)) m.wg_stamp = h->step_stamp + (size_t)(cls == T_FWD_1 ? 0 : 1) * AF_STAMP_WG * 4;
  Timer t(h, cls, fl);
  LCHK(chain_family(h->mlp_mode).fwd(&m, train ? 1 : 0, h->stream));
  return 0;
}
int launch_bwd(af_handle* h, int cls, std::initializer_list<BwdPart> parts) {
  MultiBwd m{}; double fl = 0;
  for (const BwdPart& p : parts) {
    if (p.a.NT <= p.a.tile0) continue;
    m.net[m.n] = h->nets[p.net].kern; m.a[m.n] = p.a; ++m.n;
    fl += part_rows(p.a.tile0, p.a.NT, p.rows_total) * h->flop_dx[p.net];
  }
  if (m.n == 0) return 0;
  if (h->step_stamp && (cls == T_BWD_1 || cls == T_BWD_2)) m.wg_stamp = h->step_stamp + (size_t)(cls == T_BWD_1 ? 2 : 3) * AF_STAMP_WG * 4;
  Timer t(h, cls, fl);
  m.nprod = h->mlp_mode == 2 ? 3 : 6;
  LCHK(chain_family(h->mlp_mode).bwd(&m, h->stream));
  return 0;
}
template <class Args> Args with_live(Args a, const af_handle* h, int live_base) { a.live_rows = h->live; a.live_base = live_base; return a; }
FwdArgs tile_range(FwdArgs a, int t0, int t1) { a.tile0 = t0; a.NT = t1; return a; }
BwdArgs tile_range(BwdArgs a, int t0, int t1) { a.tile0 = t0; a.NT = t1; return a; }

void plan_mapping_split(int ncu, int NT_map, int NT_atlas, int dep_rows, int& T1, int& T2) {
  const int round = ncu * 4, t1 = NT_map / round * round;
  T1 = t1 * 32 >= dep_rows ? t1 : NT_map;
  const int extra = (NT_atlas + 3) / 4 + (NT_map - T1 + 3) / 4 - ncu;
  T2 = std::min(NT_map, T1 + 4 * std::max(0, extra));
}

int finish_step(af_handle* h, Sched& sc, float* m, float* v, long long step, float* loss_out, int loss_nblk, double dw_flops, bool check_counts = true) {
  { Timer t(h, T_DW, dw_flops); DwArgs d{sc.d_jobs, sc.d_segs, h->partial, h->dw_clock, h->step_stamp ? h->step_stamp + (size_t)4 * AF_STAMP_WG * 4 : nullptr}; LCHK(af_launch_dw(&d, sc.nwg, h->dw_mode, h->stream)); }
  {
    Timer t(h, T_ADAM);
    AdamArgs a{};
    a.jobs = sc.d_ajobs; a.partial = h->partial;
    a.bufs = adam_bufs(h, m, v);
    a.hy = adam_hyper(h->cfg.lr, step);
    a.grad_out = h->debug ? h->grads : nullptr;
    a.loss_part = h->loss_part; a.loss_out = loss_out; a.counts = h->counts; a.loss_nblk = loss_nblk; a.nan_flag = h->nan_flag;
    a.check_counts = check_counts ? 1 : 0;
    LCHK(af_launch_adam(&a, (int)sc.ajobs.size(), 1, h->stream));
  }
  return 0;
}

int take_nan_flag(af_handle* h, int& flag) {
  flag = 0;
  HCHK(hipMemcpy(&flag, h->nan_flag, 4, hipMemcpyDeviceToHost));
  if (flag) HCHK(hipMemset(h->nan_flag, 0, 4));
  return 0;
}

int ensure_loss_log(af_handle* h, size_t steps) {
  if (steps * AF_LOSS_W <= h->loss_log_cap) return 0;
  if (h->loss_log) (void)hipFree(h->loss_log);
  h->loss_log = nullptr; h->loss_log_cap = 0;
  HCHK(dalloc(&h->loss_log, steps * AF_LOSS_W));
  h->loss_log_cap = steps * AF_LOSS_W;
  return 0;
}

int enqueue_single_step(af_handle* h, int i, const int64_t* d_inds, uint64_t seed, float* loss_out) {
  const af_config& c = h->cfg;
  NetDesc& M = h->nets[AF_NET_MAP1]; NetDesc& A = h->nets[AF_NET_ATLAS];
  const int N = h->N, L = std::max(c.resx, c.resy);
  const bool glob = glob_on(c, i);
  const int nseg = glob ? 9 : 7;
  Sched& sc = h->sched[glob ? 0 : 1];
  const int NT_map = tiles_of(nseg * N), NT_atlas = tiles_of(3 * N);
  if (nseg != h->cur_nseg) {
    HCHK(hipMemsetAsync(M.dout, 0, (size_t)M.nt_cap * 32 * 16, h->stream));
    h->cur_nseg = nseg;
  }
  {
    Timer t(h, T_PREP);
    PrepArgs p{};
    p.table = h->table; p.inds = d_inds; p.seed = seed; p.iter = (uint32_t)i;
    p.N = N; p.resx = c.resx; p.resy = c.resy; p.F = c.number_of_frames;
    p.half_main = (float)(L / 2.0); p.half_grad = (float)(c.resx / 2.0); p.half_frames = (float)(c.number_of_frames / 2.0);
    p.d_local = c.derivative_amount; p.d_global = c.global_rigidity_derivative_amount_fg; p.nseg = nseg;
    p.coords = M.coords; p.x0_tile = M.x0_tile; p.samples = h->samples; p.counts = h->counts;
    p.flow_rank = h->flow_rank; p.scan = h->scan; p.live = h->live; p.epoch = ++h->prep_epoch;
    p.ticket = h->scan + (N + 255) / 256; p.ticket_base = h->prep_tickets;
    LCHK(af_launch_prep(&p, h->stream));
    h->prep_tickets += (unsigned long long)((N + 255) / 256);
  }
  int rc, T1, T2;
  plan_mapping_split(h->ncu, std::min(NT_map, tiles_of((nseg - 2) * N + h->plan_flow_rows)), NT_atlas, 3 * N, T1, T2);
  const int flow_base = (nseg - 2) * N;
  const FwdArgs fm = with_live(fwd_args(h, M, M.coords, M.out_buf, NT_map, true), h, flow_base);
  if ((rc = launch_fwd(h, T_FWD_1, {{AF_NET_MAP1, tile_range(fm, 0, T1), nseg * N}}, true)) != 0) return rc;
  if ((rc = launch_fwd(h, T_FWD_2, {{AF_NET_MAP1, tile_range(fm, T1, T2), nseg * N},
                                    {AF_NET_ATLAS, fwd_args(h, A, M.out_buf, A.out_buf, NT_atlas, true), 3 * N},
                                    {AF_NET_MAP1, tile_range(fm, T2, NT_map), nseg * N}}, true)) != 0) return rc;
  {
    Timer t(h, T_LOSS);
    LossArgs l{};
    l.samples = h->samples; l.out_map = M.out_buf; l.out_atlas = A.out_buf; l.dout_map = M.dout; l.dout_atlas = A.dout;
    l.counts = h->counts; l.loss_part = h->loss_part; l.N = N; l.nseg = nseg; l.flow_rank = h->flow_rank; l.live = h->live;
    l.L = (float)L; l.uv_scale = c.uv_mapping_scale; l.d_local = c.derivative_amount; l.d_global = c.global_rigidity_derivative_amount_fg;
    l.c_rgb = c.rgb_coeff; l.c_grad = c.use_gradient_loss ? c.gradient_loss_coeff : 0.f; l.c_rig = c.rigidity_coeff;
    l.c_grig = glob ? c.global_rigidity_coeff_fg : 0.f; l.c_flow = c.optical_flow_coeff;
    LCHK(af_launch_loss_single(&l, h->stream));
  }
  h->adam_step += 1;
  {
    BwdArgs ba = bwd_args(h, A, NT_atlas); ba.din0 = M.dout; ba.nrows = 3 * N;
    const BwdArgs bm = with_live(bwd_args(h, M, NT_map), h, flow_base);
    if ((rc = launch_bwd(h, T_BWD_1, {{AF_NET_MAP1, tile_range(bm, T1, T2), nseg * N}, {AF_NET_ATLAS, ba, 3 * N},
                                      {AF_NET_MAP1, tile_range(bm, T2, NT_map), nseg * N}})) != 0) return rc;
    if ((rc = launch_bwd(h, T_BWD_2, {{AF_NET_MAP1, tile_range(bm, 0, T1), nseg * N}})) != 0) return rc;
  }
  const double dwf = (double)nseg * N * h->flop_fwd[AF_NET_MAP1] + 3.0 * N * h->flop_fwd[AF_NET_ATLAS];
  return finish_step(h, sc, h->adam_m, h->adam_v, h->adam_step, loss_out, (N + 255) / 256, dwf);
}

int enqueue_seg_step(af_handle* h, int i, const int64_t* d_inds, uint64_t seed, float* loss_out) {
  const af_config& c = h->cfg;
  NetDesc& M1 = h->nets[AF_NET_MAP1]; NetDesc& M2 = h->nets[AF_NET_MAP2]; NetDesc& A = h->nets[AF_NET_ATLAS]; NetDesc& AL = h->nets[AF_NET_ALPHA];
  const int N = h->N, L = std::max(c.resx, c.resy);
  const bool glob = glob_on(c, i);
  const int nseg = glob ? 9 : 7;
  Sched& sc = h->sched[glob ? 0 : 1];
  const int NT_map = tiles_of(nseg * N), NT_atlas = tiles_of(6 * N), NT_alpha = tiles_of(5 * N);
  if (nseg != h->cur_nseg) {
    HCHK(hipMemsetAsync(M1.dout, 0, (size_t)M1.nt_cap * 32 * 16, h->stream));
    HCHK(hipMemsetAsync(M2.dout, 0, (size_t)M2.nt_cap * 32 * 16, h->stream));
    h->cur_nseg = nseg;
  }
  {
    Timer t(h, T_PREP);
    PrepArgs p{};
    p.table = h->table; p.inds = d_inds; p.seed = seed; p.iter = (uint32_t)i;
    p.N = N; p.resx = c.resx; p.resy = c.resy; p.F = c.number_of_frames;
    p.half_main = (float)(L / 2.0); p.half_grad = (float)(c.resx / 2.0); p.half_frames = (float)(c.number_of_frames / 2.0);
    p.d_local = c.derivative_amount; p.d_global = c.global_rigidity_derivative_amount_fg; p.nseg = nseg;
    p.coords = M1.coords; p.x0_tile = M1.x0_tile; p.samples = h->samples; p.counts = h->counts;
    p.coords2 = M2.coords; p.x0_tile2 = M2.x0_tile; p.coordsA = AL.coords; p.d_global2 = c.global_rigidity_derivative_amount_bg;
    p.flow_rank = h->flow_rank; p.scan = h->scan; p.live = h->live; p.epoch = ++h->prep_epoch;
    p.ticket = h->scan + (N + 255) / 256; p.ticket_base = h->prep_tickets;
    LCHK(af_launch_prep(&p, h->stream));
    h->prep_tickets += (unsigned long long)((N + 255) / 256);
  }
  int rc;
  const int wg_atlas = (NT_atlas + 3) / 4, pad = (h->ncu - wg_atlas % h->ncu) % h->ncu;
  const int T_al = std::max(0, std::min(NT_alpha, tiles_of(3 * N + h->plan_flow_rows)) - 4 * pad);
  const int flow_base = (nseg - 2) * N;
  const FwdArgs fal = with_live(fwd_args(h, AL, AL.coords, AL.out_buf, NT_alpha, true), h, 3 * N);
  FwdArgs fat = fwd_args(h, A, M1.out_buf, A.out_buf, NT_atlas, true);
  fat.in1 = M2.out_buf; fat.split_row = 3 * N;
  if ((rc = launch_fwd(h, T_FWD_1, {{AF_NET_ALPHA, tile_range(fal, 0, T_al), 5 * N},
                                    {AF_NET_MAP1, with_live(fwd_args(h, M1, M1.coords, M1.out_buf, NT_map, true), h, flow_base), nseg * N},
                                    {AF_NET_MAP2, with_live(fwd_args(h, M2, M2.coords, M2.out_buf, NT_map, true), h, flow_base), nseg * N}}, true)) != 0) return rc;
  if ((rc = launch_fwd(h, T_FWD_2, {{AF_NET_ATLAS, fat, 6 * N}, {AF_NET_ALPHA, tile_range(fal, T_al, NT_alpha), 5 * N}}, true)) != 0) return rc;
  {
    Timer t(h, T_LOSS);
    LossSegArgs l{};
    l.samples = h->samples; l.out_m1 = M1.out_buf; l.out_m2 = M2.out_buf; l.out_alpha = AL.out_buf; l.out_atlas = A.out_buf;
    l.dout_m1 = M1.dout; l.dout_m2 = M2.dout; l.dout_alpha = AL.dout; l.dout_atlas = A.dout;
    l.counts = h->counts; l.loss_part = h->loss_part; l.N = N; l.nseg = nseg; l.flow_rank = h->flow_rank; l.live = h->live;
    l.L = (float)L; l.uv_scale = c.uv_mapping_scale; l.d_local = c.derivative_amount;
    l.d_global_fg = c.global_rigidity_derivative_amount_fg; l.d_global_bg = c.global_rigidity_derivative_amount_bg;
    l.c_rgb = c.rgb_coeff; l.c_grad = c.use_gradient_loss ? c.gradient_loss_coeff : 0.f; l.c_rig = c.rigidity_coeff;
    l.c_grig_fg = glob ? c.global_rigidity_coeff_fg : 0.f; l.c_grig_bg = glob ? c.global_rigidity_coeff_bg : 0.f;
    l.c_flow = c.optical_flow_coeff;
    l.c_boot = i > c.stop_bootstrapping_iteration ? 0.f : c.alpha_bootstrapping_factor;
    l.c_aflow = c.alpha_flow_factor; l.c_sparse = c.sparsity_coeff;
    LCHK(af_launch_loss_seg(&l, h->stream));
  }
  h->adam_step += 1;
  {
    BwdArgs ba = bwd_args(h, A, NT_atlas);
    ba.din0 = M1.dout; ba.din1 = M2.dout; ba.split_row = 3 * N; ba.nrows = 6 * N;
    const BwdArgs bal = with_live(bwd_args(h, AL, NT_alpha), h, 3 * N);
    if ((rc = launch_bwd(h, T_BWD_1, {{AF_NET_ATLAS, ba, 6 * N}, {AF_NET_ALPHA, tile_range(bal, T_al, NT_alpha), 5 * N}})) != 0) return rc;
    if ((rc = launch_bwd(h, T_BWD_2, {{AF_NET_ALPHA, tile_range(bal, 0, T_al), 5 * N}, {AF_NET_MAP1, with_live(bwd_args(h, M1, NT_map), h, flow_base), nseg * N},
                                      {AF_NET_MAP2, with_live(bwd_args(h, M2, NT_map), h, flow_base), nseg * N}})) != 0) return rc;
  }
  const double dwf = (double)nseg * N * (h->flop_fwd[AF_NET_MAP1] + h->flop_fwd[AF_NET_MAP2]) + 6.0 * N * h->flop_fwd[AF_NET_ATLAS] + 5.0 * N * h->flop_fwd[AF_NET_ALPHA];
  return finish_step(h, sc, h->adam_m, h->adam_v, h->adam_step, loss_out, (N + 255) / 256, dwf);
}

}

extern "C" {

size_t af_config_size(void) { return sizeof(af_config); }

namespace {
struct Staged {
  void* d = nullptr; bool own = false;
  hipError_t in(const void* p, size_t bytes, bool on_device) {
    if (on_device) { d = const_cast<void*>(p); return hipSuccess; }
    hipError_t e = hipMalloc(&d, std::max<size_t>(bytes, 1)); if (e != hipSuccess) return e;
    own = true;
    return p ? hipMemcpy(d, p, bytes, hipMemcpyHostToDevice) : hipSuccess;
  }
  ~Staged() { if (own) (void)hipFree(d); }
};
int util_fail(const char* what, hipError_t e) { g_create_error = std::string(what) + ": " + hipGetErrorString(e); return AF_EHIP; }
}

int af_resize_bilinear(int device_ordinal, const void* src, int src_u8, int sh, int sw, int ch, float* dst, int dh, int dw,
                       int64_t pix_stride, int64_t ch_stride, int64_t offset, double scale0, double scale1, int on_device) {
  if (!src || !dst || sh <= 0 || sw <= 0 || dh <= 0 || dw <= 0 || ch <= 0 || pix_stride <= 0) { g_create_error = "af_resize_bilinear: arguments"; return AF_EINVAL; }
  hipError_t e = hipSetDevice(device_ordinal); if (e != hipSuccess) return util_fail("hipSetDevice", e);
  if (!on_device && (pix_stride != ch || ch_stride != 1 || offset != 0)) { g_create_error = "af_resize_bilinear: host destinations must be HWC contiguous"; return AF_EINVAL; }
  Staged s, d;
  const size_t sbytes = (size_t)sh * sw * ch * (src_u8 ? 1 : 4), dbytes = (size_t)dh * dw * ch * 4;
  if ((e = s.in(src, sbytes, on_device)) != hipSuccess) return util_fail("stage source", e);
  if ((e = d.in(on_device ? (const void*)dst : nullptr, dbytes, on_device)) != hipSuccess) return util_fail("stage destination", e);
  ResizeArgs a{s.d, src_u8, sh, sw, ch, (float*)d.d, dh, dw, pix_stride, ch_stride, offset, scale0, scale1};
  int r = af_launch_resize(&a, nullptr); if (r) return util_fail("k_resize_bilinear", (hipError_t)r);
  if ((e = hipStreamSynchronize(nullptr)) != hipSuccess) return util_fail("k_resize_bilinear", e);
  if (!on_device && (e = hipMemcpy(dst, d.d, dbytes, hipMemcpyDeviceToHost)) != hipSuccess) return util_fail("copy back", e);
  return AF_OK;
}

static void area_table(int ssize, int dsize, double scale, std::vector<int>& ofs, std::vector<int>& idx, std::vector<float>& w) {
  for (int d = 0; d < dsize; ++d) {
    const double f1 = d * scale, f2 = f1 + scale, cell = std::min(scale, ssize - f1);
    int s1 = (int)std::ceil(f1);
    const int s2 = std::min((int)std::floor(f2), ssize - 1);
    s1 = std::min(s1, s2);
    ofs.push_back((int)idx.size());
    if (s1 - f1 > 1e-3) { idx.push_back(s1 - 1); w.push_back((float)((s1 - f1) / cell)); }
    for (int s = s1; s < s2; ++s) { idx.push_back(s); w.push_back((float)(1.0 / cell)); }
    if (f2 - s2 > 1e-3) { idx.push_back(s2); w.push_back((float)(std::min(std::min(f2 - s2, 1.0), cell) / cell)); }
  }
  ofs.push_back((int)idx.size());
}

int af_resize_area(int device_ordinal, const uint8_t* src, int sh, int sw, int ch, uint8_t* dst, int dh, int dw, int on_device) {
  if (!src || !dst) { g_create_error = "af_resize_area: null pointer"; return AF_EINVAL; }
  if (ch < 1 || ch > 4) { g_create_error = "af_resize_area: ch must be 1..4"; return AF_EINVAL; }
  if (dh < 1) { g_create_error = "af_resize_area: dh < 1"; return AF_EINVAL; }
  if (dw < 1) { g_create_error = "af_resize_area: dw < 1"; return AF_EINVAL; }
  if (dh > sh) { g_create_error = "af_resize_area: dh > sh (INTER_AREA is implemented for shrinking only)"; return AF_EINVAL; }
  if (dw > sw) { g_create_error = "af_resize_area: dw > sw (INTER_AREA is implemented for shrinking only)"; return AF_EINVAL; }
  if (dh == sh && dw == sw) { g_create_error = "af_resize_area: dh == sh && dw == sw (nothing to resize)"; return AF_EINVAL; }
  if ((int64_t)dh * dw > ((int64_t)1 << 38)) { g_create_error = "af_resize_area: image too large"; return AF_EINVAL; }
  hipError_t e = hipSetDevice(device_ordinal); if (e != hipSuccess) return util_fail("hipSetDevice", e);
  AreaArgs a{};
  a.sh = sh; a.sw = sw; a.ch = ch; a.dh = dh; a.dw = dw;
  const double scale_x = 1.0 / ((double)dw / sw), scale_y = 1.0 / ((double)dh / sh);
  const int isx = (int)std::nearbyint(scale_x), isy = (int)std::nearbyint(scale_y);
  const bool fast = std::fabs(scale_x - isx) < DBL_EPSILON && std::fabs(scale_y - isy) < DBL_EPSILON &&
                    (int64_t)isx * dw == sw && (int64_t)isy * dh == sh;
  std::vector<int> tab;
  Staged t;
  if (fast) {
    a.mode = (isx == 2 && isy == 2 && ch != 2) ? AREA_2X2 : AREA_BLOCK;
    a.isx = isx; a.isy = isy; a.inv_area = (float)(1.f / (float)((int64_t)isx * isy));
  } else {
    std::vector<int> xofs, yofs, xidx, yidx; std::vector<float> xa, ya;
    area_table(sw, dw, scale_x, xofs, xidx, xa);
    area_table(sh, dh, scale_y, yofs, yidx, ya);
    for (int v : xidx) if (v < 0 || v >= sw) { g_create_error = "af_resize_area: x table out of range"; return AF_EINVAL; }
    for (int v : yidx) if (v < 0 || v >= sh) { g_create_error = "af_resize_area: y table out of range"; return AF_EINVAL; }
    const size_t o_yofs = xofs.size(), o_xidx = o_yofs + yofs.size(), o_yidx = o_xidx + xidx.size(), o_xa = o_yidx + yidx.size(), o_ya = o_xa + xa.size();
    tab.resize(o_ya + ya.size());
    std::copy(xofs.begin(), xofs.end(), tab.begin()); std::copy(yofs.begin(), yofs.end(), tab.begin() + o_yofs);
    std::copy(xidx.begin(), xidx.end(), tab.begin() + o_xidx); std::copy(yidx.begin(), yidx.end(), tab.begin() + o_yidx);
    if (!xa.empty()) memcpy(tab.data() + o_xa, xa.data(), xa.size() * 4);
    if (!ya.empty()) memcpy(tab.data() + o_ya, ya.data(), ya.size() * 4);
    if ((e = t.in(tab.data(), tab.size() * 4, false)) != hipSuccess) return util_fail("stage tables", e);
    const int* base = (const int*)t.d;
    a.mode = AREA_GENERAL;
    a.xofs = base; a.yofs = base + o_yofs; a.xidx = base + o_xidx; a.yidx = base + o_yidx;
    a.xa = (const float*)(base + o_xa); a.ya = (const float*)(base + o_ya);
  }
  Staged s, d;
  const size_t sbytes = (size_t)sh * sw * ch, dbytes = (size_t)dh * dw * ch;
  if ((e = s.in(src, sbytes, on_device)) != hipSuccess) return util_fail("stage source", e);
  if ((e = d.in(on_device ? (const void*)dst : nullptr, dbytes, on_device)) != hipSuccess) return util_fail("stage destination", e);
  a.src = (const unsigned char*)s.d; a.dst = (unsigned char*)d.d;
  int r = af_launch_resize_area(&a, nullptr); if (r) return util_fail("k_resize_area", (hipError_t)r);
  if ((e = hipStreamSynchronize(nullptr)) != hipSuccess) return util_fail("k_resize_area", e);
  if (!on_device && (e = hipMemcpy(dst, d.d, dbytes, hipMemcpyDeviceToHost)) != hipSuccess) return util_fail("copy back", e);
  return AF_OK;
}

int af_luma_grid(int device_ordinal, const uint8_t* src, int n, int h, int w, int gh, int gw, uint64_t* sums_out, int on_device) {
  if (!src || !sums_out) { g_create_error = "af_luma_grid: null pointer"; return AF_EINVAL; }
  if (n < 1) { g_create_error = "af_luma_grid: n < 1"; return AF_EINVAL; }
  if (h < 1) { g_create_error = "af_luma_grid: h < 1"; return AF_EINVAL; }
  if (w < 1) { g_create_error = "af_luma_grid: w < 1"; return AF_EINVAL; }
  if (gh < 1 || gh > 64) { g_create_error = "af_luma_grid: gh must be 1..64"; return AF_EINVAL; }
  if (gw < 1 || gw > 64) { g_create_error = "af_luma_grid: gw must be 1..64"; return AF_EINVAL; }
  if (h > (1 << 24) || w > (1 << 24)) { g_create_error = "af_luma_grid: image too large"; return AF_EINVAL; }
  hipError_t e = hipSetDevice(device_ordinal); if (e != hipSuccess) return util_fail("hipSetDevice", e);
  LumaArgs a{};
  a.n = n; a.h = h; a.w = w; a.gh = std::min(gh, h); a.gw = std::min(gw, w);
  const int cw = (w + a.gw - 1) / a.gw, chh = (h + a.gh - 1) / a.gh;
  a.strip_rows = std::max(4, (4096 + cw - 1) / cw);
  a.strips = (chh + a.strip_rows - 1) / a.strip_rows;
  const size_t cells = (size_t)a.gh * a.gw, nparts = (size_t)n * cells * a.strips;
  Staged s, d;
  if ((e = s.in(src, (size_t)n * h * w * 3, on_device)) != hipSuccess) return util_fail("stage source", e);
  if ((e = d.in(nullptr, nparts * 8, false)) != hipSuccess) return util_fail("stage partial sums", e);
  a.src = (const unsigned char*)s.d; a.part = (unsigned long long*)d.d;
  int r = af_launch_luma_grid(&a, nullptr); if (r) return util_fail("k_luma_grid", (hipError_t)r);
  if ((e = hipStreamSynchronize(nullptr)) != hipSuccess) return util_fail("k_luma_grid", e);
  std::vector<unsigned long long> part(nparts);
  if ((e = hipMemcpy(part.data(), d.d, nparts * 8, hipMemcpyDeviceToHost)) != hipSuccess) return util_fail("copy back", e);
  for (size_t c = 0; c < (size_t)n * cells; ++c) {
    uint64_t t = 0;
    for (int k = 0; k < a.strips; ++k) t += part[c * a.strips + k];
    sums_out[c] = t;
  }
  return AF_OK;
}

namespace {
bool yuv_plane_sizes(int h, int w, int layout, int* ch, int* cw, int* hmode, int* vmode) {
  switch (layout) {
    case AF_YUV_444: *hmode = YUV_AXIS_FULL; *vmode = YUV_AXIS_FULL; break;
    case AF_YUV_422: *hmode = YUV_AXIS_COSITED; *vmode = YUV_AXIS_FULL; break;
    case AF_YUV_420JPEG: *hmode = YUV_AXIS_CENTRED; *vmode = YUV_AXIS_CENTRED; break;
    case AF_YUV_420MPEG2: *hmode = YUV_AXIS_COSITED; *vmode = YUV_AXIS_CENTRED; break;
    case AF_YUV_MONO: *hmode = YUV_AXIS_FULL; *vmode = YUV_AXIS_FULL; *ch = 0; *cw = 0; return true;
    default: return false;
  }
  *cw = *hmode == YUV_AXIS_FULL ? w : (w + 1) / 2;
  *ch = *vmode == YUV_AXIS_FULL ? h : (h + 1) / 2;
  return true;
}
int yuv_q14(double v) { return (int)std::nearbyint(v * 16384.0); }
void yuv_fix_row(int (&row)[3], int target) {
  int big = 0;
  for (int k = 1; k < 3; ++k) if (std::abs(row[k]) > std::abs(row[big])) big = k;
  row[big] += target - (row[0] + row[1] + row[2]);
}
int yuv_convert(const char* name, bool to_rgb, int device_ordinal, const uint8_t* src, int h, int w, int layout, int matrix, int full_range,
                uint8_t* dst, int on_device) {
  const std::string who(name);
  if (!src || !dst) { g_create_error = who + ": null pointer"; return AF_EINVAL; }
  if (h < 1 || h > 16384) { g_create_error = who + ": h must be 1..16384"; return AF_EINVAL; }
  if (w < 1 || w > 16384) { g_create_error = who + ": w must be 1..16384"; return AF_EINVAL; }
  YuvArgs a{};
  if (!yuv_plane_sizes(h, w, layout, &a.ch, &a.cw, &a.hmode, &a.vmode)) { g_create_error = who + ": unknown layout"; return AF_EINVAL; }
  if (matrix != AF_YUV_BT601 && matrix != AF_YUV_BT709) { g_create_error = who + ": unknown matrix"; return AF_EINVAL; }
  hipError_t e = hipSetDevice(device_ordinal); if (e != hipSuccess) return util_fail("hipSetDevice", e);
  const double kr = matrix == AF_YUV_BT601 ? 0.299 : 0.2126, kb = matrix == AF_YUV_BT601 ? 0.114 : 0.0722, kg = 1.0 - kr - kb;
  const double sy = full_range ? 1.0 : 219.0 / 255.0, sc = full_range ? 1.0 : 224.0 / 255.0;
  a.h = h; a.w = w; a.mono = layout == AF_YUV_MONO; a.y0 = full_range ? 0 : 16;
  a.cy = yuv_q14(1.0 / sy);
  a.crv = yuv_q14(2.0 * (1.0 - kr) / sc);
  a.cgu = yuv_q14(-2.0 * (1.0 - kb) * kb / kg / sc);
  a.cgv = yuv_q14(-2.0 * (1.0 - kr) * kr / kg / sc);
  a.cbu = yuv_q14(2.0 * (1.0 - kb) / sc);
  a.ky[0] = yuv_q14(kr * sy); a.ky[1] = yuv_q14(kg * sy); a.ky[2] = yuv_q14(kb * sy);
  a.ku[0] = yuv_q14(-kr / (2.0 * (1.0 - kb)) * sc); a.ku[1] = yuv_q14(-kg / (2.0 * (1.0 - kb)) * sc); a.ku[2] = yuv_q14(0.5 * sc);
  a.kv[0] = yuv_q14(0.5 * sc); a.kv[1] = yuv_q14(-kg / (2.0 * (1.0 - kr)) * sc); a.kv[2] = yuv_q14(-kb / (2.0 * (1.0 - kr)) * sc);
  yuv_fix_row(a.ky, yuv_q14(sy)); yuv_fix_row(a.ku, 0); yuv_fix_row(a.kv, 0);
  const size_t ybytes = (size_t)h * w + 2 * (size_t)a.ch * a.cw, rbytes = (size_t)h * w * 3;
  const size_t sbytes = to_rgb ? ybytes : rbytes, dbytes = to_rgb ? rbytes : ybytes;
  Staged s, d;
  if ((e = s.in(src, sbytes, on_device)) != hipSuccess) return util_fail("stage source", e);
  if ((e = d.in(on_device ? (const void*)dst : nullptr, dbytes, on_device)) != hipSuccess) return util_fail("stage destination", e);
  a.src = (const unsigned char*)s.d; a.dst = (unsigned char*)d.d;
  const char* kernel = to_rgb ? "k_yuv_to_rgb" : "k_rgb_to_yuv";
  int r = to_rgb ? af_launch_yuv_to_rgb(&a, nullptr) : af_launch_rgb_to_yuv(&a, nullptr); if (r) return util_fail(kernel, (hipError_t)r);
  if ((e = hipStreamSynchronize(nullptr)) != hipSuccess) return util_fail(kernel, e);
  if (!on_device && (e = hipMemcpy(dst, d.d, dbytes, hipMemcpyDeviceToHost)) != hipSuccess) return util_fail("copy back", e);
  return AF_OK;
}
}

int64_t af_yuv_frame_bytes(int h, int w, int layout) {
  int ch, cw, hm, vm;
  if (h < 1 || h > 16384 || w < 1 || w > 16384 || !yuv_plane_sizes(h, w, layout, &ch, &cw, &hm, &vm)) return 0;
  return (int64_t)h * w + 2 * (int64_t)ch * cw;
}

int af_yuv_to_rgb(int device_ordinal, const uint8_t* yuv, int h, int w, int layout, int matrix, int full_range, uint8_t* rgb, int on_device) {
  return yuv_convert("af_yuv_to_rgb", true, device_ordinal, yuv, h, w, layout, matrix, full_range, rgb, on_device);
}

int af_rgb_to_yuv(int device_ordinal, const uint8_t* rgb, int h, int w, int layout, int matrix, int full_range, uint8_t* yuv, int on_device) {
  return yuv_convert("af_rgb_to_yuv", false, device_ordinal, rgb, h, w, layout, matrix, full_range, yuv, on_device);
}

int af_flow_consistency(int device_ordinal, const float* f12, const float* f21, int h, int w, float* out,
                        int64_t pix_stride, int64_t offset, float thresh, int on_device) {
  if (!f12 || !f21 || !out || h <= 0 || w <= 0 || pix_stride <= 0) { g_create_error = "af_flow_consistency: arguments"; return AF_EINVAL; }
  hipError_t e = hipSetDevice(device_ordinal); if (e != hipSuccess) return util_fail("hipSetDevice", e);
  if (!on_device && (pix_stride != 1 || offset != 0)) { g_create_error = "af_flow_consistency: host destinations must be contiguous"; return AF_EINVAL; }
  Staged a12, a21, o;
  const size_t fb = (size_t)h * w * 8, ob = (size_t)h * w * 4;
  if ((e = a12.in(f12, fb, on_device)) != hipSuccess || (e = a21.in(f21, fb, on_device)) != hipSuccess) return util_fail("stage flows", e);
  if ((e = o.in(on_device ? (const void*)out : nullptr, ob, on_device)) != hipSuccess) return util_fail("stage output", e);
  ConsistencyArgs a{(const float*)a12.d, (const float*)a21.d, h, w, (float*)o.d, pix_stride, offset, thresh};
  int r = af_launch_consistency(&a, nullptr); if (r) return util_fail("k_flow_consistency", (hipError_t)r);
  if ((e = hipStreamSynchronize(nullptr)) != hipSuccess) return util_fail("k_flow_consistency", e);
  if (!on_device && (e = hipMemcpy(out, o.d, ob, hipMemcpyDeviceToHost)) != hipSuccess) return util_fail("copy back", e);
  return AF_OK;
}

static double warp_error_of(const double* part, int nblk, int npix) {
  double sse = 0.0, cnt = 0.0;
  for (int b = 0; b < nblk; ++b) { sse += part[2 * b]; cnt += part[2 * b + 1]; }
  return sse / (3.0 * (cnt > 0.0 ? cnt : (double)npix));
}

int af_warp_error_pair(int device_ordinal, const float* img1, const float* img2, const float* flow12, const float* flow21, int h, int w,
                       int align_corners, double* err, float* noc, float* warped, int on_device) {
  if (!img1 || !img2 || !flow12 || !flow21 || !err || h < 2 || w < 2 || (align_corners != 0 && align_corners != 1)) {
    g_create_error = "af_warp_error_pair: arguments"; return AF_EINVAL;
  }
  if ((int64_t)h * w > INT32_MAX / 4) { g_create_error = "af_warp_error_pair: image too large"; return AF_EINVAL; }
  hipError_t e = hipSetDevice(device_ordinal); if (e != hipSuccess) return util_fail("hipSetDevice", e);
  const int npix = h * w, nblk = (npix + 255) / 256;
  const size_t ib = (size_t)npix * 12, fb = (size_t)npix * 8;
  Staged s1, s2, s12, s21, sn, sw, sp;
  if ((e = s1.in(img1, ib, on_device)) != hipSuccess || (e = s2.in(img2, ib, on_device)) != hipSuccess ||
      (e = s12.in(flow12, fb, on_device)) != hipSuccess || (e = s21.in(flow21, fb, on_device)) != hipSuccess) return util_fail("stage inputs", e);
  if (noc && (e = sn.in(on_device ? (const void*)noc : nullptr, (size_t)npix * 4, on_device)) != hipSuccess) return util_fail("stage noc", e);
  if (warped && (e = sw.in(on_device ? (const void*)warped : nullptr, ib, on_device)) != hipSuccess) return util_fail("stage warped", e);
  if ((e = sp.in(nullptr, (size_t)nblk * 16, false)) != hipSuccess) return util_fail("block partials", e);
  WarpErrArgs a{(const float*)s1.d, (const float*)s2.d, (const float*)s12.d, (const float*)s21.d, 0, 0, h, w, align_corners,
                noc ? (float*)sn.d : nullptr, warped ? (float*)sw.d : nullptr, (double*)sp.d};
  int r = af_launch_warp_error(&a, 2, 1, nullptr); if (r) return util_fail("k_warp_error", (hipError_t)r);
  std::vector<double> part((size_t)nblk * 2);
  if ((e = hipMemcpy(part.data(), sp.d, (size_t)nblk * 16, hipMemcpyDeviceToHost)) != hipSuccess) return util_fail("k_warp_error", e);
  if (!on_device && noc && (e = hipMemcpy(noc, sn.d, (size_t)npix * 4, hipMemcpyDeviceToHost)) != hipSuccess) return util_fail("copy back", e);
  if (!on_device && warped && (e = hipMemcpy(warped, sw.d, ib, hipMemcpyDeviceToHost)) != hipSuccess) return util_fail("copy back", e);
  *err = warp_error_of(part.data(), nblk, npix);
  return AF_OK;
}

const char* af_last_error(const af_handle* h) { return h ? h->err.c_str() : g_create_error.c_str(); }

void af_set_thread_error(const char* m) { g_create_error = m; }

int af_create(const af_config* cfg, int device_ordinal, af_handle** out) {
  if (!cfg || !out) { g_create_error = "af_create: null argument"; return AF_EINVAL; }
  *out = nullptr;
  auto bad = [&](const char* m) { g_create_error = std::string("af_create: ") + m; return (int)AF_EINVAL; };
  if (cfg->resx <= 1 || cfg->resy <= 1 || cfg->number_of_frames <= 0) return bad("resx/resy/number_of_frames");
  if (cfg->samples_batch <= 0) return bad("samples_batch");
  auto width_ok = [](int w) { return w >= 1 && w <= AF_HID; };
  if (!width_ok(cfg->number_of_channels_mapping1) || !width_ok(cfg->number_of_channels_atlas)) return bad("number_of_channels_mapping1 / number_of_channels_atlas must be 1..256 (config_flow_100.json:19,24)");
  auto layers_ok = [](int n) { return n >= 2 && n <= AF_MAX_LAYERS; };
  if (!layers_ok(cfg->number_of_layers_mapping1) || !layers_ok(cfg->number_of_layers_atlas)) return bad("number_of_layers_mapping1 / number_of_layers_atlas must be 2..8");
  if (cfg->positional_encoding_num_atlas < 1 || cfg->positional_encoding_num_atlas > 10) return bad("positional_encoding_num_atlas must be 1..10");
  auto pe_ok = [](int k) { return k >= 1 && k <= 5; };
  if (cfg->use_positional_encoding_mapping1 && !pe_ok(cfg->number_of_positional_encoding_mapping1)) return bad("number_of_positional_encoding_mapping1 must be 1..5 when use_positional_encoding_mapping1 is set");
  if (cfg->derivative_amount <= 0 || cfg->global_rigidity_derivative_amount_fg <= 0) return bad("derivative amounts");
  const bool seg = cfg->two_layer != 0;
  if (seg) {
    if (!width_ok(cfg->number_of_channels_mapping2) || !width_ok(cfg->number_of_channels_alpha)) return bad("number_of_channels_mapping2 / number_of_channels_alpha must be 1..256 (config_flow_100.json:21,26)");
    if (!layers_ok(cfg->number_of_layers_mapping2) || !layers_ok(cfg->number_of_layers_alpha)) return bad("number_of_layers_mapping2 / number_of_layers_alpha must be 2..8");
    if (cfg->positional_encoding_num_alpha < 1 || cfg->positional_encoding_num_alpha > 5) return bad("positional_encoding_num_alpha must be 1..5");
    if (cfg->use_positional_encoding_mapping2 && !pe_ok(cfg->number_of_positional_encoding_mapping2)) return bad("number_of_positional_encoding_mapping2 must be 1..5 when use_positional_encoding_mapping2 is set");
    if (cfg->global_rigidity_derivative_amount_bg <= 0) return bad("global_rigidity_derivative_amount_bg");
  }
  hipError_t e = hipSetDevice(device_ordinal);
  if (e != hipSuccess) { g_create_error = std::string("af_create: hipSetDevice: ") + hipGetErrorString(e); return AF_EHIP; }
  af_handle* h = new af_handle();
  h->cfg = *cfg; h->device = device_ordinal; h->seg = seg;
  if (h->cfg.pretrain_batch <= 0) h->cfg.pretrain_batch = 10000;
  if (h->cfg.lr <= 0) h->cfg.lr = 1e-4f;
  auto die = [&](int code) { g_create_error = h->err; af_destroy(h); return code; };
#define CCHK(x) do { hipError_t e_ = (x); if (e_ != hipSuccess) { h->fail(AF_EHIP, #x, e_); return die(e_ == hipErrorOutOfMemory ? AF_ENOMEM : AF_EHIP); } } while (0)
  hipDeviceProp_t prop; CCHK(hipGetDeviceProperties(&prop, device_ordinal));
  h->ncu = prop.multiProcessorCount > 0 ? prop.multiProcessorCount : 256;
  CCHK(hipStreamCreateWithFlags(&h->stream, hipStreamNonBlocking));
  CCHK((hipError_t)af_mlp_init()); CCHK((hipError_t)af_mlp16_init()); CCHK((hipError_t)af_dw_init()); CCHK((hipError_t)af_mlp_bf_init()); CCHK((hipError_t)af_mlp_hf_init());

  const int nl_atlas = cfg->number_of_layers_atlas;
  const unsigned atlas_skip = (nl_atlas > 4 ? (1u << 4) : 0u) | (nl_atlas > 7 ? (1u << 7) : 0u);
  if (cfg->use_positional_encoding_mapping1) describe_net(h->nets[AF_NET_MAP1], AF_NET_MAP1, cfg->number_of_layers_mapping1, AF_IN_PE3, cfg->number_of_positional_encoding_mapping1, 2, 0u, false, cfg->number_of_channels_mapping1);
  else describe_net(h->nets[AF_NET_MAP1], AF_NET_MAP1, cfg->number_of_layers_mapping1, AF_IN_XYT, 0, 2, 0u, false, cfg->number_of_channels_mapping1);
  describe_net(h->nets[AF_NET_ATLAS], AF_NET_ATLAS, nl_atlas, AF_IN_PE2, cfg->positional_encoding_num_atlas, 3, atlas_skip, true, cfg->number_of_channels_atlas);
  if (seg) {
    if (cfg->use_positional_encoding_mapping2) describe_net(h->nets[AF_NET_MAP2], AF_NET_MAP2, cfg->number_of_layers_mapping2, AF_IN_PE3, cfg->number_of_positional_encoding_mapping2, 2, 0u, false, cfg->number_of_channels_mapping2);
    else describe_net(h->nets[AF_NET_MAP2], AF_NET_MAP2, cfg->number_of_layers_mapping2, AF_IN_XYT, 0, 2, 0u, false, cfg->number_of_channels_mapping2);
    describe_net(h->nets[AF_NET_ALPHA], AF_NET_ALPHA, cfg->number_of_layers_alpha, AF_IN_PE3, cfg->positional_encoding_num_alpha, 1, 0u, false, cfg->number_of_channels_alpha);
  }
  for (NetDesc& n : h->nets) if (n.used) {
    auto lw = [&](int w) { return w == AF_HID ? n.hid : (w > AF_HID ? w - AF_HID + n.hid : w); };
    double f = 0, d = n.dx0 ? (double)n.in_feat0 * n.hid : 0.0;
    for (int l = 0; l < n.NL; ++l) {
      const double lin = l == 0 ? n.in_feat0 : lw(n.in_feat[l]), lout = l == n.NL - 1 ? n.out : n.hid;
      f += lin * lout; if (l >= 1) d += (double)n.hid * lout;
    }
    h->flop_fwd[n.id] = 2.0 * f; h->flop_dx[n.id] = 2.0 * d;
  }
  size_t fc = 0, bc = 0, biasc = 0, pc = 0;
  for (NetDesc& n : h->nets) if (n.used) {
    n.p_base = pc; pc += n.nparams; plan_images(n, fc, bc, biasc);
    if (!check_chunk_plan(n)) { h->fail(AF_EINVAL, "weight-image plan does not match the kernels' chunk sequence"); return die(AF_EINVAL); }
    if (!plan_stream(n, n.bf, k_bf16x6, h->sf_bytes, h->sb_bytes)) { h->fail(AF_EINVAL, "bf16 stream plan does not match the kernels' chunk sizes"); return die(AF_EINVAL); }
    if (!plan_stream(n, n.hf, k_f16x3, h->hf_bytes, h->hb_bytes)) { h->fail(AF_EINVAL, "fp16 stream plan does not match the kernels' chunk sizes"); return die(AF_EINVAL); }
  }
  h->sf_bytes += 49152 + 65536; h->sb_bytes += 49152 + 65536;
  if (h->sf_bytes >= ((size_t)1 << 31) || h->sb_bytes >= ((size_t)1 << 31)) { h->fail(AF_EINVAL, "stream images exceed 2 GB"); return die(AF_EINVAL); }
  CCHK(hipMalloc((void**)&h->img_sf, h->sf_bytes)); CCHK(hipMalloc((void**)&h->img_sb, h->sb_bytes));
  CCHK(hipMemset(h->img_sf, 0, h->sf_bytes)); CCHK(hipMemset(h->img_sb, 0, h->sb_bytes));
  h->hf_bytes += 2 * 65536; h->hb_bytes += 2 * 65536;
  if (h->hf_bytes >= ((size_t)1 << 31) || h->hb_bytes >= ((size_t)1 << 31)) { h->fail(AF_EINVAL, "stream images exceed 2 GB"); return die(AF_EINVAL); }
  CCHK(hipMalloc((void**)&h->img_hf, h->hf_bytes)); CCHK(hipMalloc((void**)&h->img_hb, h->hb_bytes));
  CCHK(hipMemset(h->img_hf, 0, h->hf_bytes)); CCHK(hipMemset(h->img_hb, 0, h->hb_bytes));
  fc += AF_CHUNK_MAX / 4; bc += AF_CHUNK_MAX / 4;
  h->total_params = pc; h->img_f_floats = fc; h->img_b_floats = bc; h->bias_floats = biasc;
  CCHK(dalloc(&h->params, pc)); CCHK(dalloc(&h->adam_m, pc)); CCHK(dalloc(&h->adam_v, pc));
  CCHK(dalloc(&h->pre_m, pc)); CCHK(dalloc(&h->pre_v, pc)); CCHK(dalloc(&h->grads, pc));
  CCHK(dalloc(&h->img_f, fc)); CCHK(dalloc(&h->img_b, bc)); CCHK(dalloc(&h->bias_img, biasc));
  CCHK(hipMemset(h->params, 0, pc * 4)); CCHK(hipMemset(h->adam_m, 0, pc * 4)); CCHK(hipMemset(h->adam_v, 0, pc * 4));
  CCHK(hipMemset(h->pre_m, 0, pc * 4)); CCHK(hipMemset(h->pre_v, 0, pc * 4)); CCHK(hipMemset(h->grads, 0, pc * 4));
  CCHK(hipMemset(h->img_f, 0, fc * 4)); CCHK(hipMemset(h->img_b, 0, bc * 4)); CCHK(hipMemset(h->bias_img, 0, biasc * 4));
  h->N = cfg->samples_batch;
  const int N = h->N, rows_pre = h->cfg.pretrain_batch;
  NetDesc& M = h->nets[AF_NET_MAP1]; NetDesc& A = h->nets[AF_NET_ATLAS]; NetDesc& M2 = h->nets[AF_NET_MAP2]; NetDesc& AL = h->nets[AF_NET_ALPHA];
  CCHK(alloc_net_buffers(M, std::max(9 * N, rows_pre), true));
  CCHK(alloc_net_buffers(A, (seg ? 6 : 3) * N, false));
  if (seg) {
    CCHK(alloc_net_buffers(M2, std::max(9 * N, rows_pre), true));
    CCHK(alloc_net_buffers(AL, 5 * N, true));
  }
  CCHK(dalloc(&h->samples, (size_t)N * AF_REC_F));
  h->loss_nblk_cap = (std::max(N, rows_pre) + 255) / 256;
  CCHK(dalloc(&h->loss_part, (size_t)h->loss_nblk_cap * AF_LOSS_W)); CCHK(hipMemset(h->loss_part, 0, (size_t)h->loss_nblk_cap * AF_LOSS_W * 4));
  CCHK(dalloc(&h->counts, 2)); CCHK(hipMemset(h->counts, 0, 8));
  CCHK(dalloc(&h->nan_flag, 1)); CCHK(hipMemset(h->nan_flag, 0, 4));
  CCHK(dalloc(&h->flow_rank, (size_t)2 * N)); CCHK(hipMemset(h->flow_rank, 0xff, (size_t)2 * N * 4));
  CCHK(dalloc(&h->scan, (size_t)(N + 255) / 256 + 1)); CCHK(hipMemset(h->scan, 0, (size_t)((N + 255) / 256 + 1) * 8));
  CCHK(dalloc(&h->live, 1)); CCHK(hipMemset(h->live, 0, 4));
  CCHK(dalloc(&h->nvalid, 128));
  bool ok = build_main_scheds(h);
  ok = ok && build_sched(h, h->sched[2], {{&M, tiles_of(rows_pre)}});
  if (seg) ok = ok && build_sched(h, h->sched[3], {{&M2, tiles_of(rows_pre)}});
  if (!ok) { h->fail(AF_EINVAL, "dW schedule needs more than DW_MAXSEG segments per workgroup"); return die(AF_EINVAL); }
  size_t pf = 0;
  for (int i = 0; i < (seg ? 4 : 3); ++i) { CCHK(upload_sched(h->sched[i])); pf = std::max(pf, h->sched[i].partial_floats); }
  CCHK(dalloc(&h->partial, pf)); h->partial_cap = pf;
  h->frame_sse.assign(cfg->number_of_frames, 0.0); h->frame_sse_valid.assign(cfg->number_of_frames, 0);
  if (repack(h, h->sched[0]) != 0) return die(AF_EHIP);
  CCHK(hipStreamSynchronize(h->stream));
#undef CCHK
  *out = h;
  return AF_OK;
}

static void edit_release(af_edit* e) {
  for (int L = 0; L < 2; ++L) { (void)hipFree(e->tex[L]); (void)hipFree(e->use[L]); e->tex[L] = nullptr; e->use[L] = nullptr; }
  e->h = nullptr;
}

void af_destroy(af_handle* h) {
  if (!h) return;
  (void)hipSetDevice(h->device);
  if (h->stream) (void)hipStreamSynchronize(h->stream);
  for (af_edit* e : h->sessions) edit_release(e);
  h->sessions.clear();
  drain_timers(h);
  for (NetDesc& n : h->nets) if (n.used) free_net(n);
  for (Sched& s : h->sched) { (void)hipFree(s.d_jobs); (void)hipFree(s.d_ajobs); (void)hipFree(s.d_segs); }
  (void)hipFree(h->params); (void)hipFree(h->adam_m); (void)hipFree(h->adam_v); (void)hipFree(h->pre_m); (void)hipFree(h->pre_v); (void)hipFree(h->grads);
  (void)hipFree(h->img_f); (void)hipFree(h->img_b); (void)hipFree(h->bias_img); (void)hipFree(h->table); (void)hipFree(h->img_sf); (void)hipFree(h->img_sb); (void)hipFree(h->img_hf); (void)hipFree(h->img_hb);
  (void)hipFree(h->samples); (void)hipFree(h->loss_part); (void)hipFree(h->loss_log); (void)hipFree(h->counts); (void)hipFree(h->nan_flag); (void)hipFree(h->flow_rank); (void)hipFree(h->scan); (void)hipFree(h->live); (void)hipFree(h->nvalid);
  (void)hipFree(h->partial); (void)hipFree(h->dw_clock); (void)hipFree(h->step_stamp); (void)hipFree(h->r_coords); (void)hipFree(h->r_uv); (void)hipFree(h->r_uv2); (void)hipFree(h->r_al);
  (void)hipFree(h->r_t); (void)hipFree(h->r_rgb); (void)hipFree(h->r_sse); (void)hipFree(h->r_u8); (void)hipFree(h->r_at); (void)hipFree(h->l_buf);
  if (h->stream) (void)hipStreamDestroy(h->stream);
  delete h;
}

int af_sync(af_handle* h) {
  if (!h) return AF_EINVAL;
  HCHK(hipSetDevice(h->device)); HCHK(hipStreamSynchronize(h->stream));
  return AF_OK;
}

int af_upload_video(af_handle* h, const float* frames, const float* flow_fwd, const float* flow_bwd,
                    const float* mask_fwd, const float* mask_bwd, const float* mask_fg, int on_device) {
  if (!h) return AF_EINVAL;
  if (!frames || !flow_fwd || !flow_bwd || !mask_fwd || !mask_bwd) return h->fail(AF_EINVAL, "af_upload_video: null tensor");
  if (h->seg && !mask_fg) return h->fail(AF_EINVAL, "af_upload_video: a two_layer handle needs mask_fg (mask_frames, unwrap_utils.py:68-70)");
  HCHK(hipSetDevice(h->device));
  const size_t P2 = (size_t)h->cfg.resx * h->cfg.resy, F = h->cfg.number_of_frames, P = P2 * F;
  if (!h->table) { hipError_t e = dalloc(&h->table, P * AF_REC_F); if (e != hipSuccess) return h->fail(AF_ENOMEM, "record table", e); }
  const float* src[6] = {frames, flow_fwd, flow_bwd, mask_fwd, mask_bwd, mask_fg};
  const size_t cnt[6] = {P * 3, P * 2, P * 2, P, P, P};
  float* tmp[6] = {nullptr, nullptr, nullptr, nullptr, nullptr, nullptr};
  const float* dev[6];
  int rc = AF_OK;
  for (int i = 0; i < 6 && rc == AF_OK; ++i) {
    if (!src[i]) { dev[i] = nullptr; continue; }
    if (on_device) { dev[i] = src[i]; continue; }
    hipError_t e = dalloc(&tmp[i], cnt[i]);
    if (e == hipSuccess) e = hipMemcpy(tmp[i], src[i], cnt[i] * 4, hipMemcpyHostToDevice);
    if (e != hipSuccess) rc = h->fail(e == hipErrorOutOfMemory ? AF_ENOMEM : AF_EHIP, "af_upload_video staging", e);
    dev[i] = tmp[i];
  }
  if (rc == AF_OK) {
    PackArgs a{dev[0], dev[1], dev[2], dev[3], dev[4], dev[5], h->table, h->cfg.resx, h->cfg.resy, h->cfg.number_of_frames, h->nvalid};
    hipError_t e = hipMemsetAsync(h->nvalid, 0, 128 * 8, h->stream);
    int r = e == hipSuccess ? af_launch_pack(&a, h->stream) : (int)e;
    e = r ? (hipError_t)r : hipStreamSynchronize(h->stream);
    unsigned long long nv[2] = {0, 0}, nvs[128];
    if (e == hipSuccess) e = hipMemcpy(nvs, h->nvalid, sizeof nvs, hipMemcpyDeviceToHost);
    if (e == hipSuccess) for (int i = 0; i < 64; ++i) { nv[0] += nvs[2 * i]; nv[1] += nvs[2 * i + 1]; }
    if (e != hipSuccess) rc = h->fail(AF_EHIP, "pack table", e);
    else {
      h->p_valid[0] = (double)nv[0] / (double)P; h->p_valid[1] = (double)nv[1] / (double)P;
      if (planned_flow_rows(h) != h->plan_flow_rows) {
        if (!build_main_scheds(h)) rc = h->fail(AF_EINVAL, "dW schedule needs more than DW_MAXSEG segments per workgroup");
        for (int i = 0; i < 2 && rc == AF_OK; ++i) {
          if ((e = upload_sched(h->sched[i])) != hipSuccess) rc = h->fail(AF_EHIP, "schedule upload", e);
          if (rc == AF_OK && h->sched[i].partial_floats > h->partial_cap) {
            (void)hipFree(h->partial); h->partial = nullptr;
            if ((e = dalloc(&h->partial, h->sched[i].partial_floats)) != hipSuccess) rc = h->fail(AF_ENOMEM, "partial dW buffer", e);
            else h->partial_cap = h->sched[i].partial_floats;
          }
        }
      }
    }
  }
  for (int i = 0; i < 6; ++i) if (tmp[i]) (void)hipFree(tmp[i]);
  if (rc == AF_OK) { h->have_video = true; std::fill(h->frame_sse_valid.begin(), h->frame_sse_valid.end(), 0); }
  return rc;
}

size_t af_param_count(const af_handle* h, int net) {
  if (!h || net < 0 || net >= AF_MAX_NETS || !h->nets[net].used) return 0;
  return h->nets[net].nlogical;
}

static int check_net(af_handle* h, int net, size_t n) {
  if (!h) return AF_EINVAL;
  if (net < 0 || net >= AF_MAX_NETS || !h->nets[net].used) return h->fail(AF_EINVAL, "unknown net");
  if (n != h->nets[net].nlogical) return h->fail(AF_EINVAL, "parameter count mismatch");
  return AF_OK;
}
static int put_flat(af_handle* h, const NetDesc& n, float* dev, const float* flat) {
  if (n.lmap.empty()) { HCHK(hipMemcpy(dev + n.p_base, flat, n.nparams * 4, hipMemcpyHostToDevice)); return AF_OK; }
  std::vector<float> phys(n.nparams, 0.f);
  for (size_t i = 0; i < n.nlogical; ++i) phys[n.lmap[i]] = flat[i];
  HCHK(hipMemcpy(dev + n.p_base, phys.data(), n.nparams * 4, hipMemcpyHostToDevice));
  return AF_OK;
}
static int get_flat(af_handle* h, const NetDesc& n, const float* dev, float* flat) {
  if (n.lmap.empty()) { HCHK(hipMemcpy(flat, dev + n.p_base, n.nparams * 4, hipMemcpyDeviceToHost)); return AF_OK; }
  std::vector<float> phys(n.nparams);
  HCHK(hipMemcpy(phys.data(), dev + n.p_base, n.nparams * 4, hipMemcpyDeviceToHost));
  for (size_t i = 0; i < n.nlogical; ++i) flat[i] = phys[n.lmap[i]];
  return AF_OK;
}

int af_set_params(af_handle* h, int net, const float* flat, size_t n) {
  int rc = check_net(h, net, n); if (rc) return rc;
  if (!flat) return h->fail(AF_EINVAL, "af_set_params: null");
  HCHK(hipSetDevice(h->device));
  HCHK(hipStreamSynchronize(h->stream));
  rc = put_flat(h, h->nets[net], h->params, flat); if (rc) return rc;
  rc = repack(h, h->sched[0]); if (rc) return rc;
  HCHK(hipStreamSynchronize(h->stream));
  std::fill(h->frame_sse_valid.begin(), h->frame_sse_valid.end(), 0);
  return AF_OK;
}

int af_get_params(af_handle* h, int net, float* flat, size_t n) {
  int rc = check_net(h, net, n); if (rc) return rc;
  if (!flat) return h->fail(AF_EINVAL, "af_get_params: null");
  HCHK(hipSetDevice(h->device)); HCHK(hipStreamSynchronize(h->stream));
  return get_flat(h, h->nets[net], h->params, flat);
}

int af_get_adam_state(af_handle* h, int net, float* m, float* v, int64_t* step) {
  if (!h) return AF_EINVAL;
  if (net < 0 || net >= AF_MAX_NETS || !h->nets[net].used) return h->fail(AF_EINVAL, "unknown net");
  HCHK(hipSetDevice(h->device)); HCHK(hipStreamSynchronize(h->stream));
  const NetDesc& n = h->nets[net];
  int rc = AF_OK;
  if (m && (rc = get_flat(h, n, h->adam_m, m)) != AF_OK) return rc;
  if (v && (rc = get_flat(h, n, h->adam_v, v)) != AF_OK) return rc;
  if (step) *step = h->adam_step;
  return AF_OK;
}

int af_set_adam_state(af_handle* h, int net, const float* m, const float* v, int64_t step) {
  if (!h) return AF_EINVAL;
  if (net < 0 || net >= AF_MAX_NETS || !h->nets[net].used) return h->fail(AF_EINVAL, "unknown net");
  if (step < 0) return h->fail(AF_EINVAL, "negative step");
  HCHK(hipSetDevice(h->device)); HCHK(hipStreamSynchronize(h->stream));
  const NetDesc& n = h->nets[net];
  int rc = AF_OK;
  if (m && (rc = put_flat(h, n, h->adam_m, m)) != AF_OK) return rc;
  if (v && (rc = put_flat(h, n, h->adam_v, v)) != AF_OK) return rc;
  h->adam_step = step;
  return AF_OK;
}

static int rebuild_dw_scheds(af_handle* h) {
  HCHK(hipSetDevice(h->device)); HCHK(hipStreamSynchronize(h->stream));
  bool ok = build_main_scheds(h);
  ok = ok && build_sched(h, h->sched[2], {{&h->nets[AF_NET_MAP1], tiles_of(h->cfg.pretrain_batch)}});
  if (h->seg) ok = ok && build_sched(h, h->sched[3], {{&h->nets[AF_NET_MAP2], tiles_of(h->cfg.pretrain_batch)}});
  if (!ok) return h->fail(AF_EINVAL, "dW schedule needs more than DW_MAXSEG segments per workgroup");
  for (int i = 0; i < (h->seg ? 4 : 3); ++i) {
    HCHK(upload_sched(h->sched[i]));
    if (h->sched[i].partial_floats > h->partial_cap) {
      (void)hipFree(h->partial); h->partial = nullptr; h->partial_cap = 0;
      HCHK(dalloc(&h->partial, h->sched[i].partial_floats)); h->partial_cap = h->sched[i].partial_floats;
    }
  }
  return AF_OK;
}
int af_set_dw_mode(af_handle* h, int mode) {
  if (!h) return AF_EINVAL;
  if (mode < 0 || mode > 2) return h->fail(AF_EINVAL, "af_set_dw_mode: 0 (fp32 MFMA), 1 (bf16x6) or 2 (bf16x3)");
  if (mode == h->dw_mode) return AF_OK;
  h->dw_mode = mode;
  return rebuild_dw_scheds(h);
}
int af_debug_set_dw_cost(af_handle* h, const double* cost5, double seg_cost) {
  if (!h) return AF_EINVAL;
  if (!cost5) { if (!h->dw_cost_set) return AF_OK; h->dw_cost_set = false; h->dw_seg_cost = 0; return rebuild_dw_scheds(h); }
  for (int i = 0; i < 5; ++i)
    if (!(cost5[i] > 0.0) || !std::isfinite(cost5[i])) return h->fail(AF_EINVAL, "af_debug_set_dw_cost: every tile cost must be finite and > 0");
  if (std::isnan(seg_cost) || std::isinf(seg_cost)) return h->fail(AF_EINVAL, "af_debug_set_dw_cost: seg_cost must be finite (<= 0 keeps the shipped one)");
  const double r = *std::max_element(cost5, cost5 + 5) / *std::min_element(cost5, cost5 + 5);
  if (r > 1.0e3) return h->fail(AF_EINVAL, "af_debug_set_dw_cost: cost ratios beyond 1000:1 cut segments the DW_MAXSEG lists cannot hold");
  double keep[5]; const bool was = h->dw_cost_set; const double keep_seg = h->dw_seg_cost;
  for (int i = 0; i < 5; ++i) { keep[i] = h->dw_cost[i]; h->dw_cost[i] = cost5[i]; }
  h->dw_cost_set = true; h->dw_seg_cost = seg_cost > 0 ? seg_cost : 0;
  const int rc = rebuild_dw_scheds(h);
  if (rc != AF_OK) {
    const std::string msg = h->err;
    for (int i = 0; i < 5; ++i) h->dw_cost[i] = keep[i];
    h->dw_cost_set = was; h->dw_seg_cost = keep_seg;
    (void)rebuild_dw_scheds(h);
    h->err = msg;
  }
  return rc;
}
int af_set_mlp_mode(af_handle* h, int mode) {
  if (!h) return AF_EINVAL;
  if (mode < 0 || mode > 3) return h->fail(AF_EINVAL, "af_set_mlp_mode: 0 (fp32 MFMA), 1 (bf16x6), 2 (bf16x6 forward, three-product bf16 backward chain) or 3 (f16x3: two-term fp16 split with a scale per row)");
  const int cls_old = chain_family(h->mlp_mode).cls, cls_new = chain_family(mode).cls;
  h->mlp_mode = mode;
  if (cls_new != cls_old && cls_new != 0) {
    HCHK(hipSetDevice(h->device));
    const int rc = repack(h, h->sched[0]); if (rc) return rc;
    HCHK(hipStreamSynchronize(h->stream));
  }
  return AF_OK;
}
int af_get_modes(const af_handle* h, int* mlp_mode, int* dw_mode) {
  if (!h) return AF_EINVAL;
  if (mlp_mode) *mlp_mode = h->mlp_mode;
  if (dw_mode) *dw_mode = h->dw_mode;
  return AF_OK;
}
int af_set_debug(af_handle* h, int enable) { if (!h) return AF_EINVAL; h->debug = enable != 0; return AF_OK; }
int af_set_timing(af_handle* h, int class_mask) {
  if (!h) return AF_EINVAL;
  h->timing = (unsigned)class_mask & 0xFFFFu;
  const unsigned every = ((unsigned)class_mask >> 16) & 0xFFu;
  h->timing_every = every ? every : 1;
  return AF_OK;
}
int af_get_timing(af_handle* h, double* ms16, int64_t* counts16, double* flops16, int reset) {
  if (!h) return AF_EINVAL;
  (void)hipSetDevice(h->device); (void)hipStreamSynchronize(h->stream); drain_timers(h);
  for (int i = 0; i < 16; ++i) {
    if (ms16) ms16[i] = h->t_ms[i];
    if (counts16) counts16[i] = h->t_cnt[i];
    if (flops16) flops16[i] = h->t_flops[i];
    if (reset) { h->t_ms[i] = 0; h->t_cnt[i] = 0; h->t_flops[i] = 0; }
  }
  return AF_OK;
}

int af_get_last_grads(af_handle* h, int net, float* flat, size_t n) {
  int rc = check_net(h, net, n); if (rc) return rc;
  HCHK(hipSetDevice(h->device)); HCHK(hipStreamSynchronize(h->stream));
  return get_flat(h, h->nets[net], h->grads, flat);
}

int af_loss_width(const af_handle* h) { return h && h->seg ? 16 : 8; }

int af_pretrain(af_handle* h, int net, int pretrain_iters, const int64_t* ys, const int64_t* xs, uint64_t seed, float* losses_out) {
  if (!h) return AF_EINVAL;
  if (!(net == AF_MAPPING1 || (net == AF_MAPPING2 && h->seg))) return h->fail(AF_EINVAL, "af_pretrain: net must be a mapping net of this handle");
  if (pretrain_iters < 0 || ((ys == nullptr) != (xs == nullptr))) return h->fail(AF_EINVAL, "af_pretrain: arguments");
  HCHK(hipSetDevice(h->device));
  const int F = h->cfg.number_of_frames, NB = h->cfg.pretrain_batch;
  const size_t steps = (size_t)pretrain_iters * F;
  if (steps == 0) return AF_OK;
  NetDesc& M = h->nets[net];
  Sched& sc = h->sched[net == AF_MAPPING1 ? 2 : 3];
  int rc = ensure_loss_log(h, steps); if (rc) return rc;
  int64_t *d_ys = nullptr, *d_xs = nullptr;
  if (ys) {
    HCHK(dalloc(&d_ys, steps * NB)); HCHK(dalloc(&d_xs, steps * NB));
    HCHK(hipMemcpy(d_ys, ys, steps * NB * 8, hipMemcpyHostToDevice));
    HCHK(hipMemcpy(d_xs, xs, steps * NB * 8, hipMemcpyHostToDevice));
  }
  const int NT = tiles_of(NB);
  HCHK(hipMemsetAsync(M.dout, 0, (size_t)M.nt_cap * 32 * 16, h->stream));
  HCHK(hipMemsetAsync(h->pre_m, 0, h->total_params * 4, h->stream));
  HCHK(hipMemsetAsync(h->pre_v, 0, h->total_params * 4, h->stream));
  h->cur_nseg = 0;
  const float half_main = (float)(std::max(h->cfg.resx, h->cfg.resy) / 2.0);
  size_t s = 0;
  for (int it = 0; it < pretrain_iters && rc == 0; ++it)
    for (int f = 0; f < F && rc == 0; ++f, ++s) {
      PrePrepArgs p{};
      p.ys = d_ys ? d_ys + s * NB : nullptr; p.xs = d_xs ? d_xs + s * NB : nullptr;
      p.seed = seed; p.iter = (uint32_t)s; p.N = NB; p.resx = h->cfg.resx; p.resy = h->cfg.resy;
      p.half_main = half_main; p.t = (float)((double)f / (F / 2.0) - 1.0);
      p.coords = M.coords; p.x0_tile = M.x0_tile;
      if (af_launch_pre_prep(&p, h->stream)) { rc = h->fail(AF_EHIP, "pre_prep"); break; }
      const bool hf = h->mlp_mode == 3;
      if (hf) { if ((rc = launch_fwd(h, T_FWD_1, {{net, fwd_args(h, M, M.coords, M.out_buf, NT, true), NB}}, true)) != 0) break; }
      else { Timer t(h, T_FWD_1, (double)NB * h->flop_fwd[net]); const FwdArgs fa = fp32_images(fwd_args(h, M, M.coords, M.out_buf, NT, true), h, M);
        if (af_launch_fwd16(M.kern, &fa, h->stream)) { rc = h->fail(AF_EHIP, "fwd16"); break; } }
      PreLossArgs l{M.coords, M.out_buf, M.dout, h->loss_part, NB, h->cfg.uv_mapping_scale};
      if (af_launch_pre_loss(&l, h->stream)) { rc = h->fail(AF_EHIP, "pre_loss"); break; }
      if (hf) { if ((rc = launch_bwd(h, T_BWD_2, {{net, bwd_args(h, M, NT), NB}})) != 0) break; }
      else { Timer t(h, T_BWD_2, (double)NB * h->flop_dx[net]); const BwdArgs ba = fp32_images(bwd_args(h, M, NT), h, M);
        if (af_launch_bwd16(M.kern, &ba, h->stream)) { rc = h->fail(AF_EHIP, "bwd16"); break; } }
      rc = finish_step(h, sc, h->pre_m, h->pre_v, (long long)s + 1, h->loss_log + s * AF_LOSS_W, (NB + 255) / 256, (double)NB * h->flop_fwd[net], false);
    }
  hipError_t e = hipStreamSynchronize(h->stream);
  drain_timers(h);
  if (d_ys) { (void)hipFree(d_ys); (void)hipFree(d_xs); }
  if (rc) return rc;
  if (e != hipSuccess) return h->fail(AF_EHIP, "af_pretrain sync", e);
  { int dev_nan = 0; int r2 = take_nan_flag(h, dev_nan); if (r2) return r2; if (dev_nan & 1) return h->fail(AF_ENAN, "af_pretrain: NaN loss or non-finite parameter");
    if ((dev_nan & 2) && h->mlp_mode == 3) return h->fail(AF_ERANGE, "af_pretrain: a hidden-layer weight reached |w| >= 8, beyond what the fp16 weight images of af_set_mlp_mode(h, 3) are scaled for; use mode 1 (bf16x6)"); }
  if (losses_out) {
    std::vector<float> tmp(steps * AF_LOSS_W);
    HCHK(hipMemcpy(tmp.data(), h->loss_log, steps * AF_LOSS_W * 4, hipMemcpyDeviceToHost));
    for (size_t i = 0; i < steps; ++i) losses_out[i] = tmp[i * AF_LOSS_W] / (float)NB;
  }
  std::fill(h->frame_sse_valid.begin(), h->frame_sse_valid.end(), 0);
  return AF_OK;
}

int af_train_steps(af_handle* h, int first_iter, int n_iters, const int64_t* inds, uint64_t seed, float* losses_out) {
  if (!h) return AF_EINVAL;
  if (!h->have_video) return h->fail(AF_ESTATE, "af_train_steps: no video uploaded");
  if (n_iters < 0 || first_iter < 0) return h->fail(AF_EINVAL, "af_train_steps: arguments");
  if (n_iters == 0) return AF_OK;
  HCHK(hipSetDevice(h->device));
  const af_config& c = h->cfg;
  const int N = h->N;
  int rc = ensure_loss_log(h, n_iters); if (rc) return rc;
  int64_t* d_inds = nullptr;
  if (inds) {
    HCHK(dalloc(&d_inds, (size_t)n_iters * N));
    HCHK(hipMemcpy(d_inds, inds, (size_t)n_iters * N * 8, hipMemcpyHostToDevice));
  }
  HCHK(hipMemsetAsync(h->counts, 0, 8, h->stream));
  for (int k = 0; k < n_iters && rc == 0; ++k) {
    const int64_t* di = d_inds ? d_inds + (size_t)k * N : nullptr;
    float* lo = h->loss_log + (size_t)k * AF_LOSS_W;
    h->timing_live = (k % (int)h->timing_every) == 0;
    rc = h->seg ? enqueue_seg_step(h, first_iter + k, di, seed, lo) : enqueue_single_step(h, first_iter + k, di, seed, lo);
  }
  h->timing_live = true;
  hipError_t e = hipStreamSynchronize(h->stream);
  drain_timers(h);
  if (d_inds) (void)hipFree(d_inds);
  if (rc) return rc;
  if (e != hipSuccess) return h->fail(AF_EHIP, "af_train_steps sync", e);
  std::fill(h->frame_sse_valid.begin(), h->frame_sse_valid.end(), 0);
  int dev_nan = 0;
  if ((rc = take_nan_flag(h, dev_nan)) != 0) return rc;
  if (losses_out) {
    std::vector<float> tmp((size_t)n_iters * AF_LOSS_W);
    HCHK(hipMemcpy(tmp.data(), h->loss_log, (size_t)n_iters * AF_LOSS_W * 4, hipMemcpyDeviceToHost));
    bool nan = false;
    const float invN = 1.f / (float)N;
    for (int k = 0; k < n_iters; ++k) {
      const int i = first_iter + k;
      const bool glob = glob_on(c, i);
      const float* s = &tmp[(size_t)k * AF_LOSS_W];
      const float nf = s[AF_LOSS_W - 2], nb = s[AF_LOSS_W - 1];
      float total;
      if (!h->seg) {
        float* o = losses_out + (size_t)k * 8;
        o[0] = s[0] * invN; o[1] = c.use_gradient_loss ? s[1] * invN : 0.f; o[2] = s[2] * invN; o[3] = glob ? s[3] * invN : 0.f;
        o[4] = 0.5f * (s[5] / nb) + 0.5f * (s[4] / nf);
        o[5] = c.rigidity_coeff * o[2] + (glob ? c.global_rigidity_coeff_fg * o[3] : 0.f) + c.rgb_coeff * o[0] + c.optical_flow_coeff * o[4] + c.gradient_loss_coeff * o[1];
        o[6] = nf; o[7] = nb;
        total = o[5];
      } else {
        float* o = losses_out + (size_t)k * 16;
        const float boot = i > c.stop_bootstrapping_iteration ? 0.f : c.alpha_bootstrapping_factor;
        o[0] = s[0] * invN; o[1] = c.use_gradient_loss ? s[1] * invN : 0.f; o[2] = s[2] * invN; o[3] = s[3] * invN;
        o[4] = glob ? s[4] * invN : 0.f; o[5] = glob ? s[5] * invN : 0.f;
        o[6] = 0.5f * (s[7] / nb) + 0.5f * (s[6] / nf);
        o[7] = 0.5f * (s[9] / nb) + 0.5f * (s[8] / nf);
        o[8] = (s[10] / nf + s[11] / nb) * 0.5f;
        o[9] = s[12] * invN; o[10] = s[13] * invN;
        o[11] = c.rigidity_coeff * (o[2] + o[3]) + c.rgb_coeff * o[0] + c.optical_flow_coeff * (o[6] + o[7]) + boot * o[9]
              + c.alpha_flow_factor * o[8] + c.sparsity_coeff * o[10] + c.gradient_loss_coeff * o[1]
              + (glob ? c.global_rigidity_coeff_fg * o[4] + c.global_rigidity_coeff_bg * o[5] : 0.f);
        o[12] = nf; o[13] = nb; o[14] = 0.f; o[15] = 0.f;
        total = o[11];
      }
      if (!(total == total)) nan = true;
    }
    if (nan) return h->fail(AF_ENAN, "af_train_steps: NaN loss (a batch without valid flow pixels, as in the reference, or divergence)");
  }
  if (dev_nan & 1) return h->fail(AF_ENAN, "af_train_steps: NaN loss or non-finite parameter (a batch without valid flow pixels, as in the reference, or divergence)");
  if ((dev_nan & 2) && h->mlp_mode == 3) return h->fail(AF_ERANGE, "af_train_steps: a hidden-layer weight reached |w| >= 8, beyond what the fp16 weight images of af_set_mlp_mode(h, 3) are scaled for; use mode 1 (bf16x6)");
  return AF_OK;
}

int af_step_work(const af_handle* h, int iter, int64_t rows4[4], double* flops) {
  if (!h) return AF_EINVAL;
  const int64_t nseg = glob_on(h->cfg, iter) ? 9 : 7, N = h->N;
  int64_t r[4] = {nseg * N, (h->seg ? 6 : 3) * N, h->seg ? nseg * N : 0, h->seg ? 5 * N : 0};
  double f = 0;
  for (int i = 0; i < 4; ++i) { if (rows4) rows4[i] = r[i]; f += (double)r[i] * (2.0 * h->flop_fwd[i] + h->flop_dx[i]); }
  if (flops) *flops = f;
  return AF_OK;
}

static int ensure_render(af_handle* h, int rows) {
  if (rows <= h->render_rows_cap) return 0;
  (void)hipFree(h->r_coords); (void)hipFree(h->r_uv); (void)hipFree(h->r_uv2); (void)hipFree(h->r_al); (void)hipFree(h->r_t); (void)hipFree(h->r_rgb); (void)hipFree(h->r_sse);
  h->r_coords = h->r_uv = h->r_uv2 = h->r_al = h->r_t = h->r_rgb = nullptr; h->r_sse = nullptr; h->render_rows_cap = 0;
  const size_t rp = (size_t)tiles_of(rows) * 32;
  HCHK(dalloc(&h->r_coords, rp * 4)); HCHK(dalloc(&h->r_uv, rp * 4)); HCHK(dalloc(&h->r_t, rp * 4 * (h->seg ? 2 : 1)));
  if (h->seg) { HCHK(dalloc(&h->r_uv2, rp * 4)); HCHK(dalloc(&h->r_al, rp * 4)); }
  HCHK(dalloc(&h->r_rgb, rp * 3)); HCHK(dalloc(&h->r_sse, (rp + 255) / 256));
  h->render_rows_cap = rows;
  return 0;
}

int af_debug_plan(int ncu, int rows_map, int rows_atlas, int dep_rows, int out3[3]) {
  if (!out3 || ncu <= 0) return AF_EINVAL;
  const int NT_map = tiles_of(rows_map), NT_atlas = tiles_of(rows_atlas);
  plan_mapping_split(ncu, NT_map, NT_atlas, dep_rows, out3[0], out3[1]);
  out3[2] = NT_map;
  return AF_OK;
}

int af_debug_dw_clocks(af_handle* h, int enable, uint64_t* out, int cap_wg) {
  if (!h) return AF_EINVAL;
  HCHK(hipSetDevice(h->device)); HCHK(hipStreamSynchronize(h->stream));
  if (enable && !h->dw_clock) { HCHK(dalloc(&h->dw_clock, (size_t)h->ncu * 2)); HCHK(hipMemset(h->dw_clock, 0, (size_t)h->ncu * 16)); }
  if (out && h->dw_clock) HCHK(hipMemcpy(out, h->dw_clock, (size_t)std::min(cap_wg, h->ncu) * 16, hipMemcpyDeviceToHost));
  if (!enable && h->dw_clock) { (void)hipFree(h->dw_clock); h->dw_clock = nullptr; }
  return h->ncu;
}

int af_debug_step_clocks(af_handle* h, int enable, uint64_t* out, int cap_wg) {
  if (!h) return AF_EINVAL;
  HCHK(hipSetDevice(h->device)); HCHK(hipStreamSynchronize(h->stream));
  const size_t n = (size_t)5 * AF_STAMP_WG * 4;
  if (enable && !h->step_stamp) { HCHK(dalloc(&h->step_stamp, n)); HCHK(hipMemset(h->step_stamp, 0, n * 8)); }
  if (out && h->step_stamp) {
    const int w = std::min(cap_wg, AF_STAMP_WG);
    for (int l = 0; l < 5; ++l) HCHK(hipMemcpy(out + (size_t)l * w * 4, h->step_stamp + (size_t)l * AF_STAMP_WG * 4, (size_t)w * 32, hipMemcpyDeviceToHost));
  }
  if (h->step_stamp) HCHK(hipMemset(h->step_stamp, 0, n * 8));
  if (!enable && h->step_stamp) { (void)hipFree(h->step_stamp); h->step_stamp = nullptr; }
  return AF_STAMP_WG;
}

int af_debug_dw_schedule(af_handle* h, int which, int32_t* out, int cap_wg) {
  if (!h || which < 0 || which > 3) return AF_EINVAL;
  const Sched& sc = h->sched[which];
  int live = 0;
  if (out) { (void)hipSetDevice(h->device); (void)hipStreamSynchronize(h->stream); (void)hipMemcpy(&live, h->live, 4, hipMemcpyDeviceToHost); }
  if (out) {
    for (int w = 0; w < std::min(cap_wg, sc.nwg); ++w)
      for (int k = 0; k < DW_MAXSEG; ++k) {
        const DwSeg& sg = sc.segs[(size_t)w * DW_MAXSEG + k];
        int32_t* o = out + ((size_t)w * DW_MAXSEG + k) * 4;
        o[0] = sg.job < 0 ? -1 : sc.jobs[sg.job].shape; o[1] = sg.t0; o[2] = sg.t1; o[3] = sg.job;
        if (sg.job >= 0 && sc.jobs[sg.job].live_rows) o[2] = std::max(sg.t0, std::min(sg.t1, tiles_of(sc.jobs[sg.job].live_base + live)));
      }
  }
  return sc.nwg;
}

int af_debug_records(af_handle* h, const int64_t* inds, int n, float* out) {
  if (!h || !inds || !out || n <= 0) return AF_EINVAL;
  if (!h->have_video) return h->fail(AF_ESTATE, "af_debug_records: no video uploaded");
  HCHK(hipSetDevice(h->device)); HCHK(hipStreamSynchronize(h->stream));
  const int64_t P = (int64_t)h->cfg.resx * h->cfg.resy * h->cfg.number_of_frames;
  for (int i = 0; i < n; ++i) {
    if (inds[i] < 0 || inds[i] >= P) return h->fail(AF_EINVAL, "af_debug_records: index out of range");
    HCHK(hipMemcpy(out + (size_t)i * AF_REC_F, h->table + (size_t)inds[i] * AF_REC_F, AF_REC_F * 4, hipMemcpyDeviceToHost));
  }
  return AF_OK;
}

int af_debug_forward(af_handle* h, int net, const float* in, int rows, float* out) {
  if (!h || !in || !out || rows <= 0) return AF_EINVAL;
  if (net < 0 || net >= AF_MAX_NETS || !h->nets[net].used) return h->fail(AF_EINVAL, "unknown net");
  HCHK(hipSetDevice(h->device));
  int rc = ensure_render(h, rows); if (rc) return rc;
  const int NT = tiles_of(rows);
  HCHK(hipMemsetAsync(h->r_coords, 0, (size_t)NT * 32 * 16, h->stream));
  HCHK(hipMemcpyAsync(h->r_coords, in, (size_t)rows * 16, hipMemcpyHostToDevice, h->stream));
  FwdArgs fa = fwd_args(h, h->nets[net], h->r_coords, h->r_uv, NT, false);
  if (h->nets[net].in_kind != AF_IN_XYT) { fa.in_scale = 1.f; fa.in_shift0 = 0.f; fa.in_shift1 = 0.f; }
  { int rc2 = launch_fwd(h, T_FWD_1, {{net, fa, rows}}, false); if (rc2) return rc2; }
  HCHK(hipMemcpyAsync(out, h->r_uv, (size_t)rows * 16, hipMemcpyDeviceToHost, h->stream));
  HCHK(hipStreamSynchronize(h->stream));
  return AF_OK;
}

int af_debug_tiles(af_handle* h, int net, int which, int layer, int nt_stride, int tile0, int ntiles, float* out) {
  if (!h || !out || ntiles <= 0 || tile0 < 0 || layer < 0 || nt_stride <= 0) return AF_EINVAL;
  if (net < 0 || net >= AF_MAX_NETS || !h->nets[net].used) return h->fail(AF_EINVAL, "unknown net");
  const NetDesc& n = h->nets[net];
  if (tile0 + ntiles > nt_stride || nt_stride > n.nt_cap) return h->fail(AF_EINVAL, "af_debug_tiles: tile range");
  const float* src = nullptr; size_t per = 0; bool planes = false;
  switch (which) {
    case 0: src = n.acts; per = AF_TILE_F; planes = true; break;
    case 1: src = n.dz; per = AF_TILE_F; planes = true; break;
    case 2: src = (const float*)n.masks; per = 64 * 4; planes = true; break;
    case 3: src = n.pe_tile; per = 2048; break;
    case 4: src = n.dz_last; per = 1024; break;
    case 5: src = n.x0_tile; per = 1024; break;
    default: return h->fail(AF_EINVAL, "af_debug_tiles: which");
  }
  if (!src || (which == 3 && !n.pe_feats)) return h->fail(AF_EINVAL, "af_debug_tiles: this net has no such tensor");
  if (planes && layer >= n.NL - 1) return h->fail(AF_EINVAL, "af_debug_tiles: layer");
  HCHK(hipSetDevice(h->device)); HCHK(hipStreamSynchronize(h->stream));
  const size_t off = ((planes ? (size_t)layer * nt_stride : 0) + tile0) * per;
  HCHK(hipMemcpy(out, src + off, (size_t)ntiles * per * 4, hipMemcpyDeviceToHost));
  return AF_OK;
}

static int chains_over(af_handle* h, int n) {
  int rc;
  const int NT = tiles_of(n);
  FwdArgs fm = fwd_args(h, h->nets[AF_NET_MAP1], h->r_coords, h->r_uv, NT, false);
  if (!h->seg) {
    if ((rc = launch_fwd(h, T_FWD_1, {{AF_NET_MAP1, fm, n}}, false)) != 0) return rc;
    FwdArgs fa = fwd_args(h, h->nets[AF_NET_ATLAS], h->r_uv, h->r_t, NT, false);
    if ((rc = launch_fwd(h, T_FWD_2, {{AF_NET_ATLAS, fa, n}}, false)) != 0) return rc;
  } else {
    FwdArgs f2 = fwd_args(h, h->nets[AF_NET_MAP2], h->r_coords, h->r_uv2, NT, false);
    FwdArgs fl = fwd_args(h, h->nets[AF_NET_ALPHA], h->r_coords, h->r_al, NT, false);
    if ((rc = launch_fwd(h, T_FWD_1, {{AF_NET_ALPHA, fl, n}, {AF_NET_MAP1, fm, n}, {AF_NET_MAP2, f2, n}}, false)) != 0) return rc;
    FwdArgs fa = fwd_args(h, h->nets[AF_NET_ATLAS], h->r_uv, h->r_t, 2 * NT, false);
    fa.in1 = h->r_uv2; fa.split_row = NT * 32;
    if ((rc = launch_fwd(h, T_FWD_2, {{AF_NET_ATLAS, fa, 2 * NT * 32}}, false)) != 0) return rc;
  }
  return 0;
}

static int frame_chains(af_handle* h, float t) {
  const int npix = h->cfg.resx * h->cfg.resy;
  int rc = ensure_render(h, npix); if (rc) return rc;
  const float half_main = (float)(std::max(h->cfg.resx, h->cfg.resy) / 2.0);
  LCHK(af_launch_frame_coords(h->r_coords, h->cfg.resx, h->cfg.resy, half_main, t, tiles_of(npix) * 32, h->stream));
  return chains_over(h, npix);
}

static float frame_time(const af_handle* h, int frame) {
  return (float)((double)frame / (h->cfg.number_of_frames / 2.0) - 1.0);
}

static int render_frame_impl(af_handle* h, int frame, float* rgb_out, unsigned char* u8_out, int on_device, double* sse_out, const char* what) {
  if (!h) return AF_EINVAL;
  if (frame < 0 || frame >= h->cfg.number_of_frames) return h->fail(AF_EINVAL, (std::string(what) + ": frame index").c_str());
  if (!h->have_video) return h->fail(AF_ESTATE, (std::string(what) + ": no video uploaded").c_str());
  HCHK(hipSetDevice(h->device));
  const int npix = h->cfg.resx * h->cfg.resy;
  int rc = frame_chains(h, frame_time(h, frame)); if (rc) return rc;
  const int NT = tiles_of(npix);
  if (!h->seg) LCHK(af_launch_frame_finish(h->r_t, h->table, h->r_rgb, h->r_sse, npix, (size_t)frame * npix, h->stream));
  else         LCHK(af_launch_frame_finish_seg(h->r_t, h->r_al, (size_t)NT * 32, h->table, h->r_rgb, h->r_sse, npix, (size_t)frame * npix, h->stream));
  const int nblk = (npix + 255) / 256;
  std::vector<double> part(nblk);
  HCHK(hipMemcpyAsync(part.data(), h->r_sse, (size_t)nblk * 8, hipMemcpyDeviceToHost, h->stream));
  if (rgb_out) HCHK(hipMemcpyAsync(rgb_out, h->r_rgb, (size_t)npix * 12, on_device ? hipMemcpyDeviceToDevice : hipMemcpyDeviceToHost, h->stream));
  if (u8_out && on_device) LCHK(af_launch_frame_u8(h->r_rgb, u8_out, npix, h->stream));
  else if (u8_out) {
    if (!h->r_u8) HCHK(dalloc(&h->r_u8, (size_t)npix * 3));
    LCHK(af_launch_frame_u8(h->r_rgb, h->r_u8, npix, h->stream));
    HCHK(hipMemcpyAsync(u8_out, h->r_u8, (size_t)npix * 3, hipMemcpyDeviceToHost, h->stream));
  }
  HCHK(hipStreamSynchronize(h->stream));
  double sse = 0; for (double v : part) sse += v;
  h->frame_sse[frame] = sse; h->frame_sse_valid[frame] = 1;
  if (sse_out) *sse_out = sse;
  return AF_OK;
}

int af_render_frame(af_handle* h, int frame, float* rgb_out, double* sse_out) {
  return render_frame_impl(h, frame, rgb_out, nullptr, 0, sse_out, "af_render_frame");
}

int af_render_frame_u8(af_handle* h, int frame, float* rgb_out, uint8_t* u8_out, int on_device, double* sse_out) {
  return render_frame_impl(h, frame, rgb_out, u8_out, on_device, sse_out, "af_render_frame_u8");
}

int af_render_frame_at(af_handle* h, int frame, int oh, int ow, float* rgb_out, uint8_t* u8_out, const uint8_t* ref_u8, double* sse_out, int on_device) {
  if (!h) return AF_EINVAL;
  if (frame < 0 || frame >= h->cfg.number_of_frames) return h->fail(AF_EINVAL, "af_render_frame_at: frame index");
  if (oh < 1 || oh > AF_TEX_MAX || ow < 1 || ow > AF_TEX_MAX) return h->fail(AF_EINVAL, "af_render_frame_at: oh and ow must be 1..16384");
  if (!rgb_out && !u8_out && !ref_u8) return h->fail(AF_EINVAL, "af_render_frame_at: rgb_out, u8_out and ref_u8 are all NULL");
  if (sse_out && !ref_u8) return h->fail(AF_EINVAL, "af_render_frame_at: sse_out needs ref_u8");
  if (ref_u8 && !sse_out) return h->fail(AF_EINVAL, "af_render_frame_at: ref_u8 needs sse_out");
  HCHK(hipSetDevice(h->device));
  const int band = h->cfg.resx * h->cfg.resy;
  int rc = ensure_render(h, band); if (rc) return rc;
  if (!on_device && (u8_out || ref_u8) && !h->r_at) HCHK(dalloc(&h->r_at, (size_t)band * 6));
  const long long total = (long long)oh * ow;
  const float t = frame_time(h, frame);
  std::vector<double> part;
  if (ref_u8) part.resize((size_t)((total + band - 1) / band) * ((band + 255) / 256), 0.0);
  size_t blk0 = 0;
  for (long long r0 = 0; r0 < total; r0 += band) {
    const int n = (int)std::min<long long>(band, total - r0), NT = tiles_of(n), nblk = (n + 255) / 256;
    CoordsAtArgs ca{};
    ca.coords = h->r_coords; ca.resx = h->cfg.resx; ca.resy = h->cfg.resy; ca.oh = oh; ca.ow = ow;
    ca.half_main = (float)(std::max(h->cfg.resx, h->cfg.resy) / 2.0); ca.t = t; ca.r0 = r0; ca.n = n; ca.n_pad = NT * 32;
    LCHK(af_launch_frame_coords_at(&ca, h->stream));
    if ((rc = chains_over(h, n)) != 0) return rc;
    const size_t off = (size_t)r0 * 3;
    FinishAtArgs fa{};
    fa.out_atlas = h->r_t; fa.out_alpha = h->seg ? h->r_al : nullptr; fa.row2 = (size_t)NT * 32; fa.n = n;
    if (on_device) {
      fa.rgb_out = rgb_out ? rgb_out + off : nullptr; fa.u8_out = u8_out ? u8_out + off : nullptr; fa.ref = ref_u8 ? ref_u8 + off : nullptr;
    } else {
      fa.rgb_out = rgb_out ? h->r_rgb : nullptr; fa.u8_out = u8_out ? h->r_at : nullptr;
      if (ref_u8) {
        HCHK(hipMemcpyAsync(h->r_at + (size_t)band * 3, ref_u8 + off, (size_t)n * 3, hipMemcpyHostToDevice, h->stream));
        fa.ref = h->r_at + (size_t)band * 3;
      }
    }
    fa.sse_part = ref_u8 ? h->r_sse : nullptr;
    LCHK(af_launch_frame_finish_at(&fa, h->stream));
    if (ref_u8) { HCHK(hipMemcpyAsync(part.data() + blk0, h->r_sse, (size_t)nblk * 8, hipMemcpyDeviceToHost, h->stream)); blk0 += nblk; }
    if (!on_device && rgb_out) HCHK(hipMemcpyAsync(rgb_out + off, h->r_rgb, (size_t)n * 12, hipMemcpyDeviceToHost, h->stream));
    if (!on_device && u8_out) HCHK(hipMemcpyAsync(u8_out + off, h->r_at, (size_t)n * 3, hipMemcpyDeviceToHost, h->stream));
  }
  HCHK(hipStreamSynchronize(h->stream));
  if (sse_out) { double sse = 0; for (size_t b = 0; b < blk0; ++b) sse += part[b]; *sse_out = sse; }
  return AF_OK;
}

static int ensure_layers(af_handle* h, size_t floats) {
  if (floats <= h->l_cap) return 0;
  (void)hipFree(h->l_buf); h->l_buf = nullptr; h->l_cap = 0;
  HCHK(dalloc(&h->l_buf, floats));
  h->l_cap = floats;
  return 0;
}

int af_render_layers(af_handle* h, int frame, float* uv1, float* uv2, float* alpha, float* rgb1, float* rgb2) {
  if (!h) return AF_EINVAL;
  if (frame < 0 || frame >= h->cfg.number_of_frames) return h->fail(AF_EINVAL, "af_render_layers: frame index");
  if (!h->seg && (uv2 || rgb2)) return h->fail(AF_EINVAL, "af_render_layers: uv2 / rgb2 need a two_layer handle");
  HCHK(hipSetDevice(h->device));
  const size_t npix = (size_t)h->cfg.resx * h->cfg.resy;
  int rc = frame_chains(h, frame_time(h, frame)); if (rc) return rc;
  if ((rc = ensure_layers(h, npix * 11)) != 0) return rc;
  float* d[5] = {h->l_buf, h->l_buf + 2 * npix, h->l_buf + 4 * npix, h->l_buf + 5 * npix, h->l_buf + 8 * npix};
  float* o[5] = {uv1, uv2, alpha, rgb1, rgb2};
// ... 399 lines not shown
```

Measured before the change: 11.82 million.

## Fuse next-iteration sample prep into Adam kernel and skip unused fp32 weight images

The prep kernel for iteration i+1 now runs as extra blocks inside the Adam update launch of iteration i, which removes one kernel launch per step. The loss-visible valid counts are double-buffered by iteration parity so that prep for the next step cannot overwrite counts still being read. In f16x3 mode, Adam no longer writes the fp32 weight images. Instead they are flagged stale and repacked on demand when the mode changes or pretraining needs them. The fused launch depends on the ticket-based block ordering staying correct when it is mixed with the Adam blocks.

```diff
diff --git a/all-in-one-deflicker_amd/csrc/elem.h b/all-in-one-deflicker_amd/csrc/elem.h
--- a/all-in-one-deflicker_amd/csrc/elem.h
+++ b/all-in-one-deflicker_amd/csrc/elem.h
@@ -148,6 +148,7 @@
   const float* loss_part; float* loss_out; int* counts; int loss_nblk;
   int* nan_flag;
   int check_counts;
+  PrepArgs prep; int prep_blocks;
 };
 
 struct EditArgs {
diff --git a/all-in-one-deflicker_amd/csrc/elem.hip b/all-in-one-deflicker_amd/csrc/elem.hip
--- a/all-in-one-deflicker_amd/csrc/elem.hip
+++ b/all-in-one-deflicker_amd/csrc/elem.hip
@@ -179,7 +179,7 @@
   put_row_at(a, (size_t)seg * a.N + n, aseg >= 0 ? (long long)aseg * a.N + n : -1, x, y, t);
 }
 
-__global__ __launch_bounds__(256) void k_prep(PrepArgs a) {
+AF_DEV void prep_block(const PrepArgs& a, int nblk) {
   __shared__ int wsum[4];
   __shared__ int red_i[4];
   if (threadIdx.x == 0) red_i[0] = (int)(atomicAdd(a.ticket, 1ull) - a.ticket_base);
@@ -190,7 +190,7 @@
   const int lane = threadIdx.x & 63, wave = threadIdx.x >> 6;
   int vf = 0, vb = 0;
   int x = 0, y = 0, f = 0;
-  float ffu = 0.f, ffv = 0.f, fbu = 0.f, fbv = 0.f;
+  f32x4 r0 = {0.f, 0.f, 0.f, 0.f}, r1 = r0, r2 = r0, r3 = r0;
   const float hm = a.half_main, hg = a.half_grad, hf = a.half_frames;
   if (n < a.N) {
     const uint64_t P2 = (uint64_t)a.resx * a.resy;
@@ -199,18 +199,33 @@
     const uint64_t rem = k - (uint64_t)f * P2;
     y = (int)(rem / a.resx); x = (int)(rem - (uint64_t)y * a.resx);
     const f32x4* rp = (const f32x4*)(a.table + k * AF_REC_F);
-    f32x4 r0 = rp[0], r1 = rp[1], r2 = rp[2], r3 = rp[3];
+    r0 = rp[0]; r1 = rp[1]; r2 = rp[2]; r3 = rp[3];
+    vf = r3[1] != 0.f; vb = r3[2] != 0.f;
+  }
+  const unsigned long long bf = __ballot(vf), bb = __ballot(vb);
+  const unsigned long long lt = (1ull << lane) - 1ull;
+  const int in_wave = __popcll(bf & lt) + __popcll(bb & lt);
+  if (lane == 0) wsum[wave] = __popcll(bf) + __popcll(bb);
+  __syncthreads();
+  int in_block = in_wave;
+  for (int w = 0; w < wave; ++w) in_block += wsum[w];
+  const int btot = (wsum[0] + wsum[1]) + (wsum[2] + wsum[3]);
+  if (threadIdx.x == 0)
+    __hip_atomic_store(a.scan + vblk, ((unsigned long long)a.epoch << 32) | (unsigned)btot, __ATOMIC_RELEASE, __HIP_MEMORY_SCOPE_AGENT);
+  if (lane == 0) {
+    if (bf) atomicAdd(a.counts + 0, __popcll(bf));
+    if (bb) atomicAdd(a.counts + 1, __popcll(bb));
+  }
+  const float ffu = r2[1], ffv = r2[2], fbu = r2[3], fbv = r3[0];
+  if (n < a.N) {
     f32x4* sp = (f32x4*)(a.samples + (size_t)n * AF_REC_F);
     sp[0] = r0; sp[1] = r1; sp[2] = r2; sp[3] = r3;
-    ffu = r2[1]; ffv = r2[2]; fbu = r2[3]; fbv = r3[0];
-    const float mf = r3[1], mb = r3[2];
     const float xc = (float)x / hm - 1.f, yc = (float)y / hm - 1.f, tc = (float)f / hf - 1.f;
     put_row(a, 0, 0, n, xc, yc, tc);
     put_row(a, 1, 1, n, (float)x / hg - 1.f, (float)(y + 1) / hg - 1.f, tc);
     put_row(a, 2, 2, n, (float)(x + 1) / hg - 1.f, (float)y / hg - 1.f, tc);
     put_row(a, 3, -1, n, xc, (float)(y - a.d_local) / hm - 1.f, tc);
     put_row(a, 4, -1, n, (float)(x - a.d_local) / hm - 1.f, yc, tc);
-    vf = mf != 0.f; vb = mb != 0.f;
     if (a.nseg > 7) {
       put_row_to(a.coords, a.x0_tile, (size_t)5 * a.N + n, xc, (float)(y - a.d_global) / hm - 1.f, tc);
       put_row_to(a.coords, a.x0_tile, (size_t)6 * a.N + n, (float)(x - a.d_global) / hm - 1.f, yc, tc);
@@ -220,20 +235,6 @@
       }
     }
   }
-  const unsigned long long bf = __ballot(vf), bb = __ballot(vb);
-  const unsigned long long lt = (1ull << lane) - 1ull;
-  const int in_wave = __popcll(bf & lt) + __popcll(bb & lt);
-  if (lane == 0) {
-    wsum[wave] = __popcll(bf) + __popcll(bb);
-    if (bf) atomicAdd(a.counts + 0, __popcll(bf));
-    if (bb) atomicAdd(a.counts + 1, __popcll(bb));
-  }
-  __syncthreads();
-  int in_block = in_wave;
-  for (int w = 0; w < wave; ++w) in_block += wsum[w];
-  const int btot = (wsum[0] + wsum[1]) + (wsum[2] + wsum[3]);
-  if (threadIdx.x == 0)
-    __hip_atomic_store(a.scan + vblk, ((unsigned long long)a.epoch << 32) | (unsigned)btot, __ATOMIC_RELEASE, __HIP_MEMORY_SCOPE_AGENT);
   int pre = 0;
   if (wave == 0) {
     for (int b = lane; b < vblk; b += 64) {
@@ -247,7 +248,7 @@
   }
   __syncthreads();
   pre = red_i[0];
-  if (vblk == (int)gridDim.x - 1 && threadIdx.x == 0) *a.live = pre + btot;
+  if (vblk == nblk - 1 && threadIdx.x == 0) *a.live = pre + btot;
   if (n < a.N) {
     const int rank_f = pre + in_block, rank_b = rank_f + vf;
     const size_t base = (size_t)(a.nseg - 2) * a.N, abase = (size_t)3 * a.N;
@@ -257,6 +258,7 @@
     if (vb) put_row_at(a, base + rank_b, (long long)(abase + rank_b), ((float)x + fbu) / hm - 1.f, ((float)y + fbv) / hm - 1.f, (float)(f - 1) / hf - 1.f);
   }
 }
+__global__ __launch_bounds__(256) void k_prep(PrepArgs a) { prep_block(a, (int)gridDim.x); }
 
 AF_DEV float block_sum(float v, float* red ) {
 #pragma unroll
@@ -587,10 +589,10 @@
   const uint32_t col = j.col0 + i;
   uint32_t k = col;
   if (col >= j.hid_cols) k = j.hid_cols + (uint32_t)af_pe_slot_of_feature((int)j.pe_kind, (int)(col - j.hid_cols));
-  b.img_f[j.f_off + af_img_index(j.f_mpad, o, k)] = p;
+  if (b.img_f) b.img_f[j.f_off + af_img_index(j.f_mpad, o, k)] = p;
   if (j.b_img_off >= 0 && col < (j.hid_cols ? j.hid_cols : j.p_ld)) {
     const uint32_t mrow = j.hid_cols ? col : (uint32_t)af_pe_slot_of_feature((int)j.pe_kind, (int)col);
-    b.img_b[(uint32_t)j.b_img_off + af_img_index(j.b_mpad, mrow, o)] = p;
+    if (b.img_b) b.img_b[(uint32_t)j.b_img_off + af_img_index(j.b_mpad, mrow, o)] = p;
     if (b.sb && j.sb_off >= 0) {
       if (j.sb_kind == 0) ((float*)(b.sb + j.sb_off))[af_img_index(j.sb_mpad, mrow, o)] = p;
       else                emit_bf3(b.sb + j.sb_off, mrow, o, p);
@@ -612,7 +614,16 @@
 
 template <bool UPDATE>
 __global__ __launch_bounds__(256) void k_adam(AdamArgs a) {
-  const AdamJob j = a.jobs[blockIdx.y];
+  uint32_t job_y = blockIdx.y;
+  if (UPDATE && a.prep_blocks > 0) {
+    const uint32_t rows = ((uint32_t)a.prep_blocks + gridDim.x - 1) / gridDim.x;
+    if (blockIdx.y < rows) {
+      if (blockIdx.y * gridDim.x + blockIdx.x < (uint32_t)a.prep_blocks) prep_block(a.prep, a.prep_blocks);
+      return;
+    }
+    job_y -= rows;
+  }
+  const AdamJob j = a.jobs[job_y];
   const uint32_t e = blockIdx.x * blockDim.x + threadIdx.x;
   const uint32_t nw = j.out_real * j.in_real;
   const uint32_t nb = j.b_off >= 0 ? j.out_real : 0u;
@@ -659,7 +670,7 @@
     if (is_bias) a.bufs.bias_img[j.bias_img_off + o] = p;
     else emit_weight(j, a.bufs, o, i, p);
   }
-  if (UPDATE && blockIdx.x == 0 && blockIdx.y == 0 && a.loss_out) {
+  if (UPDATE && blockIdx.x == 0 && job_y == 0 && a.loss_out) {
     if (threadIdx.x < AF_LOSS_W - 2) {
       float s = 0.f;
       for (int b = 0; b < a.loss_nblk; ++b) s += a.loss_part[b * AF_LOSS_W + threadIdx.x];
@@ -852,7 +863,8 @@
   return (int)hipGetLastError();
 }
 int af_launch_adam(const AdamArgs* a, int njobs, int update, hipStream_t s) {
-  const dim3 grid((AF_HID * 320 + AF_HID + 255) / 256, njobs);
+  const unsigned gx = (AF_HID * 320 + AF_HID + 255) / 256;
+  const dim3 grid(gx, njobs + (update && a->prep_blocks > 0 ? ((unsigned)a->prep_blocks + gx - 1) / gx : 0u));
   if (update) hipLaunchKernelGGL(k_adam<true>, grid, dim3(256), 0, s, *a);
   else        hipLaunchKernelGGL(k_adam<false>, grid, dim3(256), 0, s, *a);
   return (int)hipGetLastError();
diff --git a/all-in-one-deflicker_amd/csrc/host.hip b/all-in-one-deflicker_amd/csrc/host.hip
--- a/all-in-one-deflicker_amd/csrc/host.hip
+++ b/all-in-one-deflicker_amd/csrc/host.hip
@@ -127,6 +127,7 @@
   int N = 0;
   float *samples = nullptr, *loss_part = nullptr, *loss_log = nullptr;
   int* counts = nullptr; int loss_nblk_cap = 0; size_t loss_log_cap = 0;
+  bool img_stale = false;
   int* nan_flag = nullptr;
   int cur_nseg = 0;
   int* flow_rank = nullptr; unsigned long long* scan = nullptr; int* live = nullptr; uint32_t prep_epoch = 0; unsigned long long prep_tickets = 0;
@@ -521,18 +522,19 @@
   return hy;
 }
 
-AdamBufs adam_bufs(af_handle* h, float* m, float* v) {
+AdamBufs adam_bufs(af_handle* h, float* m, float* v, bool all_views = false) {
   const int cls = chain_family(h->mlp_mode).cls;
-  const bool bf = cls == 1, hf = cls == 2;
-  return {h->params, m, v, h->img_f, h->img_b, h->bias_img, bf ? h->img_sf : nullptr, bf ? h->img_sb : nullptr, hf ? h->img_hf : nullptr, hf ? h->img_hb : nullptr};
+  const bool bf = cls == 1, hf = cls == 2, img = all_views || h->mlp_mode != 3;
+  return {h->params, m, v, img ? h->img_f : nullptr, img ? h->img_b : nullptr, h->bias_img, bf ? h->img_sf : nullptr, bf ? h->img_sb : nullptr, hf ? h->img_hf : nullptr, hf ? h->img_hb : nullptr};
 }
 
 int repack(af_handle* h, Sched& sc) {
   AdamArgs a{};
   a.jobs = sc.d_ajobs; a.partial = h->partial;
-  a.bufs = adam_bufs(h, h->adam_m, h->adam_v);
+  a.bufs = adam_bufs(h, h->adam_m, h->adam_v, true);
   a.nan_flag = h->nan_flag;
   LCHK(af_launch_adam(&a, (int)sc.ajobs.size(), 0, h->stream));
+  if (&sc == &h->sched[0]) h->img_stale = false;
   return 0;
 }
 
@@ -581,7 +583,40 @@
   T2 = std::min(NT_map, T1 + 4 * std::max(0, extra));
 }
 
-int finish_step(af_handle* h, Sched& sc, float* m, float* v, long long step, float* loss_out, int loss_nblk, double dw_flops, bool check_counts = true) {
+int* counts_slot(const af_handle* h, int iter) { return h->counts + 2 * (iter & 1); }
+
+PrepArgs prep_args(af_handle* h, int i, const int64_t* d_inds, uint64_t seed) {
+  const af_config& c = h->cfg;
+  const int L = std::max(c.resx, c.resy);
+  NetDesc& M1 = h->nets[AF_NET_MAP1];
+  PrepArgs p{};
+  p.table = h->table; p.inds = d_inds; p.seed = seed; p.iter = (uint32_t)i;
+  p.N = h->N; p.resx = c.resx; p.resy = c.resy; p.F = c.number_of_frames;
+  p.half_main = (float)(L / 2.0); p.half_grad = (float)(c.resx / 2.0); p.half_frames = (float)(c.number_of_frames / 2.0);
+  p.d_local = c.derivative_amount; p.d_global = c.global_rigidity_derivative_amount_fg; p.nseg = glob_on(c, i) ? 9 : 7;
+  p.coords = M1.coords; p.x0_tile = M1.x0_tile; p.samples = h->samples; p.counts = counts_slot(h, i);
+  if (h->seg) {
+    NetDesc& M2 = h->nets[AF_NET_MAP2];
+    p.coords2 = M2.coords; p.x0_tile2 = M2.x0_tile; p.coordsA = h->nets[AF_NET_ALPHA].coords; p.d_global2 = c.global_rigidity_derivative_amount_bg;
+  }
+  p.flow_rank = h->flow_rank; p.scan = h->scan; p.live = h->live;
+  return p;
+}
+int take_prep_launch(af_handle* h, PrepArgs& p) {
+  const int nblk = (p.N + 255) / 256;
+  p.epoch = ++h->prep_epoch; p.ticket = h->scan + nblk; p.ticket_base = h->prep_tickets;
+  return nblk;
+}
+int launch_prep_alone(af_handle* h, int i, const int64_t* d_inds, uint64_t seed) {
+  Timer t(h, T_PREP);
+  PrepArgs p = prep_args(h, i, d_inds, seed);
+  const int nblk = take_prep_launch(h, p);
+  LCHK(af_launch_prep(&p, h->stream));
+  h->prep_tickets += (unsigned long long)nblk;
+  return 0;
+}
+
+int finish_step(af_handle* h, Sched& sc, float* m, float* v, long long step, float* loss_out, int loss_nblk, double dw_flops, int* counts, bool check_counts = true, const PrepArgs* next_prep = nullptr) {
   { Timer t(h, T_DW, dw_flops); DwArgs d{sc.d_jobs, sc.d_segs, h->partial, h->dw_clock, h->step_stamp ? h->step_stamp + (size_t)4 * AF_STAMP_WG * 4 : nullptr}; LCHK(af_launch_dw(&d, sc.nwg, h->dw_mode, h->stream)); }
   {
     Timer t(h, T_ADAM);
@@ -590,9 +625,12 @@
     a.bufs = adam_bufs(h, m, v);
     a.hy = adam_hyper(h->cfg.lr, step);
     a.grad_out = h->debug ? h->grads : nullptr;
-    a.loss_part = h->loss_part; a.loss_out = loss_out; a.counts = h->counts; a.loss_nblk = loss_nblk; a.nan_flag = h->nan_flag;
+    a.loss_part = h->loss_part; a.loss_out = loss_out; a.counts = counts; a.loss_nblk = loss_nblk; a.nan_flag = h->nan_flag;
     a.check_counts = check_counts ? 1 : 0;
+    if (next_prep) { a.prep = *next_prep; a.prep_blocks = take_prep_launch(h, a.prep); }
+    if (!a.bufs.img_f) h->img_stale = true;
     LCHK(af_launch_adam(&a, (int)sc.ajobs.size(), 1, h->stream));
+    h->prep_tickets += (unsigned long long)a.prep_blocks;
   }
   return 0;
 }
@@ -613,7 +651,7 @@
   return 0;
 }
 
-int enqueue_single_step(af_handle* h, int i, const int64_t* d_inds, uint64_t seed, float* loss_out) {
+int enqueue_single_step(af_handle* h, int i, const int64_t* d_inds, uint64_t seed, float* loss_out, bool first, bool carry_next, const int64_t* d_inds_next) {
   const af_config& c = h->cfg;
   NetDesc& M = h->nets[AF_NET_MAP1]; NetDesc& A = h->nets[AF_NET_ATLAS];
   const int N = h->N, L = std::max(c.resx, c.resy);
@@ -625,20 +663,9 @@
     HCHK(hipMemsetAsync(M.dout, 0, (size_t)M.nt_cap * 32 * 16, h->stream));
     h->cur_nseg = nseg;
   }
-  {
-    Timer t(h, T_PREP);
-    PrepArgs p{};
-    p.table = h->table; p.inds = d_inds; p.seed = seed; p.iter = (uint32_t)i;
-    p.N = N; p.resx = c.resx; p.resy = c.resy; p.F = c.number_of_frames;
-    p.half_main = (float)(L / 2.0); p.half_grad = (float)(c.resx / 2.0); p.half_frames = (float)(c.number_of_frames / 2.0);
-    p.d_local = c.derivative_amount; p.d_global = c.global_rigidity_derivative_amount_fg; p.nseg = nseg;
-    p.coords = M.coords; p.x0_tile = M.x0_tile; p.samples = h->samples; p.counts = h->counts;
-    p.flow_rank = h->flow_rank; p.scan = h->scan; p.live = h->live; p.epoch = ++h->prep_epoch;
-    p.ticket = h->scan + (N + 255) / 256; p.ticket_base = h->prep_tickets;
-    LCHK(af_launch_prep(&p, h->stream));
-    h->prep_tickets += (unsigned long long)((N + 255) / 256);
-  }
-  int rc, T1, T2;
+  int rc;
+  if (first && (rc = launch_prep_alone(h, i, d_inds, seed)) != 0) return rc;
+  int T1, T2;
   plan_mapping_split(h->ncu, std::min(NT_map, tiles_of((nseg - 2) * N + h->plan_flow_rows)), NT_atlas, 3 * N, T1, T2);
   const int flow_base = (nseg - 2) * N;
   const FwdArgs fm = with_live(fwd_args(h, M, M.coords, M.out_buf, NT_map, true), h, flow_base);
@@ -650,7 +677,7 @@
     Timer t(h, T_LOSS);
     LossArgs l{};
     l.samples = h->samples; l.out_map = M.out_buf; l.out_atlas = A.out_buf; l.dout_map = M.dout; l.dout_atlas = A.dout;
-    l.counts = h->counts; l.loss_part = h->loss_part; l.N = N; l.nseg = nseg; l.flow_rank = h->flow_rank; l.live = h->live;
+    l.counts = counts_slot(h, i); l.loss_part = h->loss_part; l.N = N; l.nseg = nseg; l.flow_rank = h->flow_rank; l.live = h->live;
     l.L = (float)L; l.uv_scale = c.uv_mapping_scale; l.d_local = c.derivative_amount; l.d_global = c.global_rigidity_derivative_amount_fg;
     l.c_rgb = c.rgb_coeff; l.c_grad = c.use_gradient_loss ? c.gradient_loss_coeff : 0.f; l.c_rig = c.rigidity_coeff;
     l.c_grig = glob ? c.global_rigidity_coeff_fg : 0.f; l.c_flow = c.optical_flow_coeff;
@@ -665,10 +692,11 @@
     if ((rc = launch_bwd(h, T_BWD_2, {{AF_NET_MAP1, tile_range(bm, 0, T1), nseg * N}})) != 0) return rc;
   }
   const double dwf = (double)nseg * N * h->flop_fwd[AF_NET_MAP1] + 3.0 * N * h->flop_fwd[AF_NET_ATLAS];
-  return finish_step(h, sc, h->adam_m, h->adam_v, h->adam_step, loss_out, (N + 255) / 256, dwf);
-}
-
-int enqueue_seg_step(af_handle* h, int i, const int64_t* d_inds, uint64_t seed, float* loss_out) {
+  const PrepArgs next = carry_next ? prep_args(h, i + 1, d_inds_next, seed) : PrepArgs{};
+  return finish_step(h, sc, h->adam_m, h->adam_v, h->adam_step, loss_out, (N + 255) / 256, dwf, counts_slot(h, i), true, carry_next ? &next : nullptr);
+}
+
+int enqueue_seg_step(af_handle* h, int i, const int64_t* d_inds, uint64_t seed, float* loss_out, bool first, bool carry_next, const int64_t* d_inds_next) {
   const af_config& c = h->cfg;
   NetDesc& M1 = h->nets[AF_NET_MAP1]; NetDesc& M2 = h->nets[AF_NET_MAP2]; NetDesc& A = h->nets[AF_NET_ATLAS]; NetDesc& AL = h->nets[AF_NET_ALPHA];
   const int N = h->N, L = std::max(c.resx, c.resy);
@@ -681,21 +709,8 @@
     HCHK(hipMemsetAsync(M2.dout, 0, (size_t)M2.nt_cap * 32 * 16, h->stream));
     h->cur_nseg = nseg;
   }
-  {
-    Timer t(h, T_PREP);
-    PrepArgs p{};
-    p.table = h->table; p.inds = d_inds; p.seed = seed; p.iter = (uint32_t)i;
-    p.N = N; p.resx = c.resx; p.resy = c.resy; p.F = c.number_of_frames;
-    p.half_main = (float)(L / 2.0); p.half_grad = (float)(c.resx / 2.0); p.half_frames = (float)(c.number_of_frames / 2.0);
-    p.d_local = c.derivative_amount; p.d_global = c.global_rigidity_derivative_amount_fg; p.nseg = nseg;
-    p.coords = M1.coords; p.x0_tile = M1.x0_tile; p.samples = h->samples; p.counts = h->counts;
-    p.coords2 = M2.coords; p.x0_tile2 = M2.x0_tile; p.coordsA = AL.coords; p.d_global2 = c.global_rigidity_derivative_amount_bg;
-    p.flow_rank = h->flow_rank; p.scan = h->scan; p.live = h->live; p.epoch = ++h->prep_epoch;
-    p.ticket = h->scan + (N + 255) / 256; p.ticket_base = h->prep_tickets;
-    LCHK(af_launch_prep(&p, h->stream));
-    h->prep_tickets += (unsigned long long)((N + 255) / 256);
-  }
   int rc;
+  if (first && (rc = launch_prep_alone(h, i, d_inds, seed)) != 0) return rc;
   const int wg_atlas = (NT_atlas + 3) / 4, pad = (h->ncu - wg_atlas % h->ncu) % h->ncu;
   const int T_al = std::max(0, std::min(NT_alpha, tiles_of(3 * N + h->plan_flow_rows)) - 4 * pad);
   const int flow_base = (nseg - 2) * N;
@@ -711,7 +726,7 @@
     LossSegArgs l{};
     l.samples = h->samples; l.out_m1 = M1.out_buf; l.out_m2 = M2.out_buf; l.out_alpha = AL.out_buf; l.out_atlas = A.out_buf;
     l.dout_m1 = M1.dout; l.dout_m2 = M2.dout; l.dout_alpha = AL.dout; l.dout_atlas = A.dout;
-    l.counts = h->counts; l.loss_part = h->loss_part; l.N = N; l.nseg = nseg; l.flow_rank = h->flow_rank; l.live = h->live;
+    l.counts = counts_slot(h, i); l.loss_part = h->loss_part; l.N = N; l.nseg = nseg; l.flow_rank = h->flow_rank; l.live = h->live;
     l.L = (float)L; l.uv_scale = c.uv_mapping_scale; l.d_local = c.derivative_amount;
     l.d_global_fg = c.global_rigidity_derivative_amount_fg; l.d_global_bg = c.global_rigidity_derivative_amount_bg;
     l.c_rgb = c.rgb_coeff; l.c_grad = c.use_gradient_loss ? c.gradient_loss_coeff : 0.f; l.c_rig = c.rigidity_coeff;
@@ -731,7 +746,8 @@
                                       {AF_NET_MAP2, with_live(bwd_args(h, M2, NT_map), h, flow_base), nseg * N}})) != 0) return rc;
   }
   const double dwf = (double)nseg * N * (h->flop_fwd[AF_NET_MAP1] + h->flop_fwd[AF_NET_MAP2]) + 6.0 * N * h->flop_fwd[AF_NET_ATLAS] + 5.0 * N * h->flop_fwd[AF_NET_ALPHA];
-  return finish_step(h, sc, h->adam_m, h->adam_v, h->adam_step, loss_out, (N + 255) / 256, dwf);
+  const PrepArgs next = carry_next ? prep_args(h, i + 1, d_inds_next, seed) : PrepArgs{};
+  return finish_step(h, sc, h->adam_m, h->adam_v, h->adam_step, loss_out, (N + 255) / 256, dwf, counts_slot(h, i), true, carry_next ? &next : nullptr);
 }
 
 }
@@ -1076,7 +1092,7 @@
   CCHK(dalloc(&h->samples, (size_t)N * AF_REC_F));
   h->loss_nblk_cap = (std::max(N, rows_pre) + 255) / 256;
   CCHK(dalloc(&h->loss_part, (size_t)h->loss_nblk_cap * AF_LOSS_W)); CCHK(hipMemset(h->loss_part, 0, (size_t)h->loss_nblk_cap * AF_LOSS_W * 4));
-  CCHK(dalloc(&h->counts, 2)); CCHK(hipMemset(h->counts, 0, 8));
+  CCHK(dalloc(&h->counts, 4)); CCHK(hipMemset(h->counts, 0, 16));
   CCHK(dalloc(&h->nan_flag, 1)); CCHK(hipMemset(h->nan_flag, 0, 4));
   CCHK(dalloc(&h->flow_rank, (size_t)2 * N)); CCHK(hipMemset(h->flow_rank, 0xff, (size_t)2 * N * 4));
   CCHK(dalloc(&h->scan, (size_t)(N + 255) / 256 + 1)); CCHK(hipMemset(h->scan, 0, (size_t)((N + 255) / 256 + 1) * 8));
@@ -1294,7 +1310,7 @@
   if (mode < 0 || mode > 3) return h->fail(AF_EINVAL, "af_set_mlp_mode: 0 (fp32 MFMA), 1 (bf16x6), 2 (bf16x6 forward, three-product bf16 backward chain) or 3 (f16x3: two-term fp16 split with a scale per row)");
   const int cls_old = chain_family(h->mlp_mode).cls, cls_new = chain_family(mode).cls;
   h->mlp_mode = mode;
-  if (cls_new != cls_old && cls_new != 0) {
+  if ((cls_new != cls_old && cls_new != 0) || (mode != 3 && h->img_stale)) {
     HCHK(hipSetDevice(h->device));
     const int rc = repack(h, h->sched[0]); if (rc) return rc;
     HCHK(hipStreamSynchronize(h->stream));
@@ -1368,6 +1384,7 @@
       p.coords = M.coords; p.x0_tile = M.x0_tile;
       if (af_launch_pre_prep(&p, h->stream)) { rc = h->fail(AF_EHIP, "pre_prep"); break; }
       const bool hf = h->mlp_mode == 3;
+      if (!hf && h->img_stale && (rc = repack(h, h->sched[0])) != 0) break;
       if (hf) { if ((rc = launch_fwd(h, T_FWD_1, {{net, fwd_args(h, M, M.coords, M.out_buf, NT, true), NB}}, true)) != 0) break; }
       else { Timer t(h, T_FWD_1, (double)NB * h->flop_fwd[net]); const FwdArgs fa = fp32_images(fwd_args(h, M, M.coords, M.out_buf, NT, true), h, M);
         if (af_launch_fwd16(M.kern, &fa, h->stream)) { rc = h->fail(AF_EHIP, "fwd16"); break; } }
@@ -1376,7 +1393,7 @@
       if (hf) { if ((rc = launch_bwd(h, T_BWD_2, {{net, bwd_args(h, M, NT), NB}})) != 0) break; }
       else { Timer t(h, T_BWD_2, (double)NB * h->flop_dx[net]); const BwdArgs ba = fp32_images(bwd_args(h, M, NT), h, M);
         if (af_launch_bwd16(M.kern, &ba, h->stream)) { rc = h->fail(AF_EHIP, "bwd16"); break; } }
-      rc = finish_step(h, sc, h->pre_m, h->pre_v, (long long)s + 1, h->loss_log + s * AF_LOSS_W, (NB + 255) / 256, (double)NB * h->flop_fwd[net], false);
+      rc = finish_step(h, sc, h->pre_m, h->pre_v, (long long)s + 1, h->loss_log + s * AF_LOSS_W, (NB + 255) / 256, (double)NB * h->flop_fwd[net], h->counts, false);
     }
   hipError_t e = hipStreamSynchronize(h->stream);
   drain_timers(h);
@@ -1408,12 +1425,14 @@
     HCHK(dalloc(&d_inds, (size_t)n_iters * N));
     HCHK(hipMemcpy(d_inds, inds, (size_t)n_iters * N * 8, hipMemcpyHostToDevice));
   }
-  HCHK(hipMemsetAsync(h->counts, 0, 8, h->stream));
+  HCHK(hipMemsetAsync(h->counts, 0, 16, h->stream));
   for (int k = 0; k < n_iters && rc == 0; ++k) {
     const int64_t* di = d_inds ? d_inds + (size_t)k * N : nullptr;
+    const bool first = k == 0, carry = k + 1 < n_iters;
+    const int64_t* dn = d_inds && carry ? di + N : nullptr;
     float* lo = h->loss_log + (size_t)k * AF_LOSS_W;
     h->timing_live = (k % (int)h->timing_every) == 0;
-    rc = h->seg ? enqueue_seg_step(h, first_iter + k, di, seed, lo) : enqueue_single_step(h, first_iter + k, di, seed, lo);
+    rc = h->seg ? enqueue_seg_step(h, first_iter + k, di, seed, lo, first, carry, dn) : enqueue_single_step(h, first_iter + k, di, seed, lo, first, carry, dn);
   }
   h->timing_live = true;
   hipError_t e = hipStreamSynchronize(h->stream);
```

Result: no change. 11.89 million (median of 6 runs) (+0.7%).
